# zgojcic/3D_multiview_reg

Measured on AMD Instinct MI355X. Metric: point-cloud pairs/s (feat+match+filter+SVD), 3DMatch 20k-pt, 1/2/4/8 GPU, higher is better.
Workload: dtype f32 (bf16x3 MFMA operands); 1 GPU; one synthetic 3DMatch-scale scene per GPU (configs[2]): 30 fragments x ~20393 voxels (0.025 m) -> FCGF -> rand 5000 samples -> soft feature-NN for all 435 pairs -> OANet (128ch, 500 clusters, 2 blocks) -> weighted Procrustes -> all-gather of (R,t,conf); sampler=rand, fragments_per_gpu=30, pairs_per_gpu=435, samples=5000, voxels_mean=20393, math=f32eq, oanet_point_layout=chunk-major, spconv_presplit_planes=False, spatial_map_order=False, library=d32607a7c7e03829, parallelism=dp1 (one scene per rank, RCCL all-gather of records)

## Files before the change

### 3d_multiview_reg_amd/csrc/gemm.hip

```cpp
#include <atomic>
#include <type_traits>
#include <utility>

#include "common.hpp"
#include "knobs.hpp"
#include "gemm.hpp"
#include "mfma_bf16.hpp"
#include "prof.hpp"

#ifndef GEMM_EARLY
#define GEMM_EARLY 0
#endif

#ifndef GEMM_TRACE
#define GEMM_TRACE 0
#endif

namespace mvr {

#if GEMM_TRACE
__device__ unsigned long long g_gemm_trace[8];
#define TSTAMP(slot)                                                   \
  do {                                                                 \
    unsigned long long t_;                                             \
// ... 1017 lines not shown
#pragma unroll
      for (int j = 0; j < 2; ++j) {
        const int r = wn * 64 + j * 32 + l32;
        const int o = r * C2_BK + 8 * (cc ^ ((r >> 2) & 3));
        fb[j].h = *reinterpret_cast<const bf16x8*>(Bs + o);
        fb[j].m = *reinterpret_cast<const bf16x8*>(Bs + C2_BPL + o);
        fb[j].l = *reinterpret_cast<const bf16x8*>(Bs + 2 * C2_BPL + o);
      }
      if (st == 0) store_a(SET, gn, so);
#pragma unroll
      for (int ii = 0; ii < 2; ++ii)
#pragma unroll
        for (int j = 0; j < 2; ++j) acc[ii][j] = bx::mfma6(fa[ii], fb[j], acc[ii][j]);
      if (st == 0) {
        issue_a(SET, min(gs + 3, S - 1));
        __builtin_amdgcn_sched_group_barrier(0x100, 16, 0);
#pragma unroll
        for (int u = 0; u < 24; ++u) {
          __builtin_amdgcn_sched_group_barrier(0x008, 1, 0);
          __builtin_amdgcn_sched_group_barrier(0x002, 4, 0);
          if (u == C2_AISSUE) __builtin_amdgcn_sched_group_barrier(0x020, 2, 0);
          if (u == 20) __builtin_amdgcn_sched_group_barrier(0x200, 3, 0);
        }
        __builtin_amdgcn_sched_barrier(0);
        TSTAMP(3);
      }
    }
    TSTAMP(4);
    if (ks == nks - 1) {
      const int t = slot + (gs / nks) * G;
      const int b = t / ntn, tn = t % ntn;
      const int n0 = tn * C2_BN, nb0 = n0 + wn * 64;
      const int nw = min(max(N - nb0, 0), 64);
      const float rnw = nw > 0 ? 1.f / (float)nw : 0.f;
      bool cok[2][4], sok[2];
      float bn[2][4];
#pragma unroll
      for (int j = 0; j < 2; ++j) {
        const int gn = nb0 + j * 32 + 4 * p8;
        sok[j] = gn < N4;
#pragma unroll
        for (int u = 0; u < 4; ++u) {
          cok[j][u] = gn + u < N;
          bn[j][u] = cok[j][u] ? g.bias[gn + u] : 0.f;
        }
      }
      float* Cb = g.C + (int64_t)b * g.sCb;
      if (!C2_RPRE) {
        const float* Rb = g.R + (int64_t)b * g.sRb;
#pragma unroll
        for (int ii = 0; ii < 2; ++ii)
#pragma unroll
          for (int q = 0; q < 4; ++q) {
            const int gm = wm * 64 + ii * 32 + 8 * q + 4 * kh + t4;
#pragma unroll
            for (int j = 0; j < 2; ++j) {
              const int gnc = min(nb0 + j * 32 + 4 * p8, N4 - 4);
              w[ii][j][q] = *reinterpret_cast<const float4*>(Rb + (int64_t)gm * g.ldc + gnc);
            }
          }
      }
#pragma unroll
      for (int ii = 0; ii < 2; ++ii) {
#pragma unroll
        for (int q = 0; q < 4; ++q) {
          const int gm = wm * 64 + ii * 32 + 8 * q + 4 * kh + t4;
#pragma unroll
          for (int j = 0; j < 2; ++j) {
            float a0 = acc[ii][j][4 * q], a1 = acc[ii][j][4 * q + 1], a2 = acc[ii][j][4 * q + 2],
                  a3 = acc[ii][j][4 * q + 3];
            quad_transpose(a0, a1, a2, a3, h1, h2);
            const float4 x = make_float4(a0 + bn[j][0] + w[ii][j][q].x, a1 + bn[j][1] + w[ii][j][q].y,
                                         a2 + bn[j][2] + w[ii][j][q].z, a3 + bn[j][3] + w[ii][j][q].w);
            w[ii][j][q] = x;
            if (sok[j]) *reinterpret_cast<float4*>(Cb + (int64_t)gm * g.ldc + nb0 + j * 32 + 4 * p8) = x;
          }
        }
        float s1[4], s2[4];
#pragma unroll
        for (int q = 0; q < 4; ++q) {
          s1[q] = 0.f;
#pragma unroll
          for (int j = 0; j < 2; ++j)
#pragma unroll
            for (int u = 0; u < 4; ++u) s1[q] += cok[j][u] ? f4(w[ii][j][q], u) : 0.f;
          s1[q] = sum8_p8(s1[q]);
        }
#pragma unroll
        for (int q = 0; q < 4; ++q) {
          const float mu = s1[q] * rnw;
          s2[q] = 0.f;
#pragma unroll
          for (int j = 0; j < 2; ++j)
#pragma unroll
            for (int u = 0; u < 4; ++u) {
              const float d = cok[j][u] ? f4(w[ii][j][q], u) - mu : 0.f;
              s2[q] = fmaf(d, d, s2[q]);
            }
          s2[q] = sum8_p8(s2[q]);
        }
        if (p8 == 0) {
#pragma unroll
          for (int q = 0; q < 4; ++q)
            red[wn * 128 + wm * 64 + ii * 32 + 8 * q + 4 * kh + t4] = make_float2(s1[q], s2[q]);
        }
      }
      lds_barrier();
      if (tid < 256) {
        const int half = tid >> 7, row = tid & 127;
        const int n0h = n0 + 128 * half;
        if (n0h < N) {
          const float2 x = red[(2 * half) * 128 + row], c = red[(2 * half + 1) * 128 + row];
          const int na = min(N - n0h, 64), nb = min(max(N - n0h - 64, 0), 64);
          float2 o = x;
          if (nb > 0) {
            const float d = c.x / (float)nb - x.x / (float)na;
            o = make_float2(x.x + c.x, x.y + c.y + d * d * ((float)na * (float)nb / (float)(na + nb)));
          }
          g.stats[((int64_t)b * ntn128 + 2 * tn + half) * g.st_ld + g.st_off + row] = o;
        }
      }
#pragma unroll
      for (int ii = 0; ii < 2; ++ii)
#pragma unroll
        for (int j = 0; j < 2; ++j)
#pragma unroll
          for (int r = 0; r < 16; ++r) acc[ii][j][r] = 0.f;
    }
    TSTAMP(5);
    if (ks != nks - 1) asm volatile("s_waitcnt vmcnt(2)" ::: "memory");
    else asm volatile("s_waitcnt vmcnt(0)" ::: "memory");
  };
  for (int gs = 0; gs < S; gs += 2) {
    stage(I1{}, gs);
    if (gs + 1 < S) stage(I0{}, gs + 1);
  }
  asm volatile("s_waitcnt vmcnt(0)" ::: "memory");
#if GEMM_TRACE
  TSTAMP(7);
  if (lane == 0)
    for (int q = 0; q < 8; ++q) atomicAdd(&g_gemm_trace[q], tr[q]);
#endif
}


static bool oaf_conv2_covers(const GemmArgs& g) {
  return g.wimg && g.M == 128 && g.pro == PRO_A_K && g.bkc == 1 && g.sBb == 0 && g.bias_mode == BIAS_N &&
         g.stats_mode == ST_ROW && g.has_res && !g.no_store && !g.head_w && !g.xin && g.K % 4 == 0 &&
         g.K > C2_BK && g.K <= C2_KMAX &&
         g.wimg_bytes >= oaf_conv2_image_bytes(g.N, g.K) && (reinterpret_cast<uintptr_t>(g.wimg) & 15) == 0 &&
         (int64_t)c2_nks(g.K) * c2_npad(g.N) * C2_BK * 2 * 3 < ((int64_t)1 << 31);
}

static int launch_oaf_conv2(const GemmArgs& g, hipStream_t s) {
  const int Npad = c2_npad(g.N), nks = c2_nks(g.K);
  const int64_t nthr = (int64_t)nks * Npad * 4;
  hipLaunchKernelGGL(oaf_w_image_kernel, dim3((unsigned)((nthr + 255) / 256)), dim3(256), 0, s, g.B, g.N, g.K, g.ldb,
                     Npad, nks, g.wimg);
  MVR_CHECK_LAUNCH();
  const long long tiles = (long long)(Npad / C2_BN) * g.batch;
  const unsigned wgs = (unsigned)(tiles < GPU_CUS ? tiles : GPU_CUS);
  hipLaunchKernelGGL(oaf_conv2_kernel, dim3(wgs), dim3(C2_THREADS), 0, s, g, (const uint16_t*)g.wimg);
  MVR_CHECK_LAUNCH();
  return MVR_OK;
}

#ifndef GEMM_F16_DEFAULT
#define GEMM_F16_DEFAULT 0
#endif
int g_gemm_h = GEMM_F16_DEFAULT;

template <int PRO, int BKC, int BIAS, int STATS, int RES>
static void launch_t(const KArgs& ka0, long long tiles, hipStream_t s) {
  KArgs ka = ka0;
  const unsigned wgs = (unsigned)(tiles < ka.persist ? tiles : ka.persist);
  const GemmArgs& g = ka.g;
  const bool alias = g.C && (g.C == g.A || g.C == g.B || (g.has_res && g.C == g.R));
  if (g_gemm_h && g.flag && !alias) {
    ka.range = g.flag;
    ka.epoch = 1;
    hipLaunchKernelGGL((gemm_kernel<MATH_F16X2, PRO, BKC, BIAS, STATS, RES>), dim3(wgs), dim3(256), 0, s, ka);
    ka.guard = ka.range;
    ka.range = nullptr;
  }
  hipLaunchKernelGGL((gemm_kernel<MATH_BF16X3, PRO, BKC, BIAS, STATS, RES>), dim3(wgs), dim3(256), 0, s, ka);
}

static inline bool al16(const void* p) { return (reinterpret_cast<uintptr_t>(p) & 15) == 0; }

static int launch_gemm_impl(const GemmArgs& g, hipStream_t s, bool conv2) {
  if (g.M <= 0 || g.N <= 0 || g.batch <= 0) return MVR_OK;
  if (!g.A || !g.B || (!g.C && !g.no_store) || g.K <= 0) return MVR_EINVAL;
  if (g.no_store && !g.head_w && (g.stats_mode != ST_ROW || g.has_res)) return MVR_EINVAL;
  if (g.pro != PRO_NONE && !g.psc) return MVR_EINVAL;
  if ((g.pro == PRO_A_K || g.pro == PRO_B_K) && !g.psh) return MVR_EINVAL;
  if (g.stats_mode != ST_NONE && !g.stats) return MVR_EINVAL;
  if (g.bias_mode != BIAS_NONE && !g.bias) return MVR_EINVAL;
  if (g.has_res && !g.R) return MVR_EINVAL;
  if (g.math != MATH_BF16X3) return MVR_EINVAL;
  const int64_t K4 = round4(g.K), N4 = round4(g.N);
  const bool cm = g.bcs || g.ccs || (g.has_res && (g.rcs || (g.ldr && g.ldr != g.ldc)));
  const int64_t ldr = g.ldr ? g.ldr : g.ldc;
  bool ok = al16(g.A) && al16(g.B) && al16(g.C) && g.lda % 4 == 0 && g.ldb % 4 == 0 && g.ldc % 4 == 0 &&
            g.sAb % 4 == 0 && g.sBb % 4 == 0 && g.sCb % 4 == 0 && g.lda >= K4 && g.ldc >= (g.ccs ? 32 : N4) &&
            g.ldb >= (g.bkc ? K4 : (g.bcs ? 32 : N4));
  if (g.bcs) ok = ok && !g.bkc && g.ldb == 32 && g.bcs % 4 == 0 && g.bcs >= 32LL * g.K;
  if (g.ccs) ok = ok && g.ldc == 32 && g.ccs % 4 == 0 && g.ccs >= 32LL * g.M;
  if (g.has_res) {
    ok = ok && al16(g.R) && g.sRb % 4 == 0;
    if (g.xin != 2)
      ok = ok && ldr % 4 == 0 && (g.rcs ? ldr == 32 && g.rcs % 4 == 0 && g.rcs >= 32LL * g.M : ldr >= N4);
  }
  if (cm && !pconv_covers(g)) return MVR_EINVAL;
  if (g.pro == PRO_A_K || g.pro == PRO_B_K)
    ok = ok && al16(g.psc) && al16(g.psh) && g.sPb % 4 == 0 && g.K % 4 == 0 && g.K <= KV_MAX;
  if (g.pro == PRO_B_SMX) ok = ok && al16(g.psc) && g.sPb % 4 == 0 && g.pld % 4 == 0 && g.pld >= N4;
  if (!ok) return MVR_EINVAL;
  KArgs ka{};
  ka.g = g;
  ka.persist = 2 * GPU_CUS;
  ka.m_fast = (g.sAb == 0 && gemm_mtiles(g.M) > 1) ? 1 : 0;
  const long long tiles = (long long)gemm_ntiles(g.N) * gemm_mtiles(g.M) * g.batch;
  if (tiles > 0x7fffffffLL) return MVR_EINVAL;
  const double fl = 2.0 * g.M * g.N * (double)g.K * g.batch;
  double by = 4.0 * ((double)g.M * g.K * (g.sAb ? g.batch : 1) + (double)g.K * g.N * (g.sBb ? g.batch : 1) +
                     (double)g.M * g.N * g.batch * ((g.has_res ? 2 : 1) - (g.no_store ? 1 : 0)));
  if (g.xin) {
    if (!pconv_covers(g)) return MVR_EINVAL;
    by = 4.0 * ((double)g.M * g.K + (double)g.N * g.batch * (g.xin == 1 ? g.xci + g.M : g.K + g.xci + g.M));
  }
  ProfScope prof(g.prof_kind, fl, by, s);
  if (pconv_covers(g)) return launch_pconv(g, s);
  if (conv2 && oaf_conv2_covers(g)) return launch_oaf_conv2(g, s);
  if (g.head_w) return MVR_EINVAL;
#define MVR_CASE(P, BKC_, BI, ST, RS)                                                                     \
  if (g.pro == P && g.bkc == BKC_ && g.bias_mode == BI && g.stats_mode == ST && (g.has_res != 0) == RS) { \
    launch_t<P, BKC_, BI, ST, RS>(ka, tiles, s);                                                        \
    MVR_CHECK_LAUNCH();                                                                                  \
    return MVR_OK;                                                                                       \
  }
  MVR_CASE(PRO_NONE, 0, BIAS_M, ST_ROW, 0)
  MVR_CASE(PRO_NONE, 0, BIAS_M, ST_NONE, 0)
  MVR_CASE(PRO_B_K, 0, BIAS_M, ST_ROW, 0)
  MVR_CASE(PRO_B_K, 0, BIAS_M, ST_NONE, 0)
  MVR_CASE(PRO_B_K, 0, BIAS_M, ST_COL, 0)
  MVR_CASE(PRO_B_K, 0, BIAS_M, ST_ROW, 1)
  MVR_CASE(PRO_B_K, 0, BIAS_M, ST_ROWSMX, 0)
  MVR_CASE(PRO_B_K, 0, BIAS_M, ST_COLSMX, 0)
  MVR_CASE(PRO_B_SMX, 1, BIAS_NONE, ST_ROW, 0)
  MVR_CASE(PRO_B_SMX, 0, BIAS_NONE, ST_ROW, 0)
  MVR_CASE(PRO_A_K, 1, BIAS_N, ST_ROW, 1)
  MVR_CASE(PRO_NONE, 0, BIAS_NONE, ST_NONE, 0)
  MVR_CASE(PRO_NONE, 1, BIAS_NONE, ST_NONE, 0)
#undef MVR_CASE
  return MVR_EINVAL;
}

int launch_gemm(const GemmArgs& g, hipStream_t s) { return launch_gemm_impl(g, s, !g_force[FORCE_GENERIC_GEMM]); }

}

extern "C" int mvr_gemm_f32(int M, int N, int K, int batch, const float* A, int64_t sAb, int64_t lda, const float* B,
                            int64_t sBb, int64_t ldb, int b_kcontig, float* C, int64_t sCb, int64_t ldc,
                            const float* R, int64_t sRb, const float* bias, int bias_mode, const float* psc,
                            const float* psh, int64_t sPb, int64_t pld, int pro, float* stats, int64_t st_ld,
                            int st_off, int stats_mode, int math, int32_t* range_flag, hipStream_t stream) {
  mvr::GemmArgs g{};
  if (range_flag && math == mvr::MATH_BF16X3 && (mvr::g_gemm_h || mvr::g_pconv_h)) {
    if (hipMemsetAsync(range_flag, 0, sizeof(int32_t), stream) != hipSuccess) return MVR_ELAUNCH;
    g.flag = range_flag;
  }
  g.math = math;
  g.M = M; g.N = N; g.K = K; g.batch = batch;
  g.A = A; g.sAb = sAb; g.lda = lda;
  g.B = B; g.sBb = sBb; g.ldb = ldb; g.bkc = b_kcontig;
  g.C = C; g.sCb = sCb; g.ldc = ldc;
  g.R = R; g.sRb = sRb; g.has_res = R != nullptr;
  g.bias = bias; g.bias_mode = bias_mode;
  g.psc = psc; g.psh = psh; g.sPb = sPb; g.pld = pld; g.pro = pro;
  g.stats = reinterpret_cast<float2*>(stats); g.st_ld = st_ld; g.st_off = st_off; g.stats_mode = stats_mode;
  return mvr::launch_gemm(g, stream);
}

#if GEMM_TRACE
extern "C" int mvr_gemm_trace(unsigned long long* out, int reset) {
  if (hipMemcpyFromSymbol(out, HIP_SYMBOL(mvr::g_gemm_trace), sizeof(unsigned long long) * 8) != hipSuccess) return -1;
  if (reset) {
    unsigned long long z[8] = {0, 0, 0, 0, 0, 0, 0, 0};
    if (hipMemcpyToSymbol(HIP_SYMBOL(mvr::g_gemm_trace), z, sizeof(z)) != hipSuccess) return -1;
  }
  return 0;
}
#endif

extern "C" int mvr_oaf_conv2_f32(int M, int N, int K, int batch, const float* A, int64_t sAb, int64_t lda,
                                 const float* W, int64_t ldw, float* C, int64_t sCb, int64_t ldc, const float* R,
                                 int64_t sRb, const float* bias, const float* psc, const float* psh, int64_t sPb,
                                 float* stats, int64_t st_ld, void* img, int64_t img_bytes, hipStream_t stream) {
  mvr::GemmArgs g{};
  g.math = mvr::MATH_BF16X3;
  g.M = M; g.N = N; g.K = K; g.batch = batch;
  g.A = A; g.sAb = sAb; g.lda = lda;
  g.B = W; g.sBb = 0; g.ldb = ldw; g.bkc = 1;
  g.C = C; g.sCb = sCb; g.ldc = ldc;
  g.R = R; g.sRb = sRb; g.has_res = 1;
  g.bias = bias; g.bias_mode = mvr::BIAS_N;
  g.psc = psc; g.psh = psh; g.sPb = sPb; g.pro = mvr::PRO_A_K;
  g.stats = reinterpret_cast<float2*>(stats); g.st_ld = st_ld; g.stats_mode = mvr::ST_ROW;
  g.wimg = static_cast<uint16_t*>(img); g.wimg_bytes = img_bytes;
  if (M != 128 || K % 4 || N < 0 || batch < 0) return MVR_EINVAL;
  if (N == 0 || batch == 0) return MVR_OK;
  if (!R || !bias || !psc || !psh || !stats || !img) return MVR_EINVAL;
// ... 8 lines not shown
```

### 3d_multiview_reg_amd/csrc/gemm.hpp

```cpp
#pragma once
#include "knobs.hpp"
#include <hip/hip_runtime.h>
#include <stdint.h>

#include "mvreg.h"

namespace mvr {

enum Pro : int {
  PRO_NONE = 0,
  PRO_A_K = 1,
  PRO_B_K = 2,
  PRO_B_SMX = 3,
};
enum Bias : int { BIAS_NONE = 0, BIAS_M = 1, BIAS_N = 2 };
enum Stats : int {
  ST_NONE = 0,
  ST_ROW = 1,
  ST_ROWSMX = 2,
  ST_COLSMX = 3,
  ST_COL = 4,
};

enum Math : int { MATH_BF16X3 = 1, MATH_F16X2 = 2 };

constexpr int GEMM_BM = 128, GEMM_BN = 128, GEMM_BK = 32;

struct GemmArgs {
  int M, N, K, batch;
  const float* A; int64_t sAb; int64_t lda;
  const float* B; int64_t sBb; int64_t ldb; int bkc;
  float* C; int64_t sCb; int64_t ldc;
  const float* R; int64_t sRb;
  const float* bias;
  const float* psc; const float* psh; int64_t sPb;
  int64_t pld;
  float2* stats; int64_t st_ld; int st_off;
  int pro, bias_mode, stats_mode, has_res;
  int prof_kind;
  int math;
  int no_store;
  const float* head_w; const float* head_bp; float* logits; float* scores; int32_t* pos;
  int xin; int xci; const float* xw; const float* xb;
  int64_t xld;
  int* flag;
  int* fin_cnt; float fin_eps; mvr_bn_p fin_bn; float* fin_sc; float* fin_sh; int64_t fin_ld;
  float fin_eps2; mvr_bn_p fin_bn2; float* fin_sc2; float* fin_sh2;
  int fin_train; float2* fin_mv; int* fin_done;
  uint16_t* wimg; int64_t wimg_bytes;
  int64_t bcs, ccs, rcs, ldr;
};

int launch_gemm(const GemmArgs& g, hipStream_t stream);

bool pconv_covers(const GemmArgs& g);
int launch_pconv(const GemmArgs& g, hipStream_t stream);

int oan_diff_pool_cm(const float* x, int64_t x_pstride, int64_t x_ld, int64_t x_cs, const float* sc, const float* sh,
                     int64_t s_pstride, const float* weight, const float* bias, int P, int channels, int N, int clusters,
                     float* out, int64_t out_pstride, int64_t out_ld, float* stats, int64_t st_ld, int st_off,
                     void* workspace, size_t workspace_bytes, hipStream_t stream);
int oan_diff_unpool_cm(const float* x_up, int64_t x_pstride, int64_t x_ld, int64_t x_cs, const float* sc,
                       const float* sh, int64_t s_pstride, const float* weight, const float* bias, const float* x_down,
                       int64_t xd_pstride, int64_t xd_ld, int P, int channels, int N, int clusters, float* out,
                       int64_t out_pstride, int64_t out_ld, int64_t out_cs, float* stats, int64_t st_ld, int st_off,
                       void* workspace, size_t workspace_bytes, hipStream_t stream);

int64_t oaf_conv2_image_bytes(int N, int K);

inline int gemm_ntiles(int N){ return (N + GEMM_BN - 1) / GEMM_BN; }
inline int gemm_mtiles(int M) { return (M + GEMM_BM - 1) / GEMM_BM; }
inline int64_t round4(int64_t x) { return (x + 3) & ~(int64_t)3; }
inline int64_t round32(int64_t x) { return (x + 31) & ~(int64_t)31; }

}
```

### 3d_multiview_reg_amd/csrc/knobs.hip

```cpp
#include "common.hpp"
#include "knobs.hpp"
#include "mvreg.h"

namespace mvr {
int g_force[FORCE_COUNT] = {};
}

extern "C" int mvr_set_math(int mode) {
  using namespace mvr;
  const int prev = g_spconv_h ? 1 : 0;
  const int h = mode == 1 ? 1 : 0;
  g_gemm_h = g_pconv_h = g_attn_h = g_spconv_h = h;
  if (g_feat_nn_fast) g_feat_nn_fast = h ? 2 : 1;
  return prev;
}

extern "C" int mvr_debug_force(int what, int value) {
  using namespace mvr;
  if (what == FORCE_FEAT_NN_ONLINE) {
    const int prev = g_feat_nn_fast ? 0 : 1;
    g_feat_nn_fast = value ? 0 : (g_spconv_h ? 2 : 1);
    return prev;
  }
  if (what < 0 || what >= FORCE_COUNT) return MVR_EINVAL;
  const int prev = g_force[what];
  g_force[what] = value ? 1 : 0;
  return prev;
}
```

### 3d_multiview_reg_amd/csrc/knobs.hpp

```cpp
#pragma once

namespace mvr {

constexpr int GPU_CUS = 256;

extern int g_gemm_h;
extern int g_pconv_h;
extern int g_attn_h;
extern int g_spconv_h;
extern int g_feat_nn_fast;

enum ForcePath : int {
  FORCE_FEAT_NN_ONLINE = 0,
  FORCE_GENERIC_GEMM = 1,
  FORCE_UNFUSED_ATTN = 2,
  FORCE_NO_CONV1_FOLD = 3,
  FORCE_POOL_NOSPLIT = 4,
  FORCE_UNPOOL8 = 5,
  FORCE_ROW_LAYOUT = 6,
  FORCE_COUNT = 7
};
extern int g_force[FORCE_COUNT];

}
```

### 3d_multiview_reg_amd/csrc/oan_attn.hip

```cpp
#include <algorithm>
#include <functional>
#include <vector>

#include "common.hpp"
#include "gemm.hpp"
#include "knobs.hpp"
#include "mfma_bf16.hpp"
#include "prof.hpp"
#include "mvreg.h"

namespace mvr {

using namespace bx;

constexpr int AC = 128;
constexpr int AKB = 32;
constexpr int AQ = 256;
constexpr int ATHREADS = 512;
constexpr int ATL = AQ + 4;
constexpr int PLANE = AC * AKB * 2;
constexpr int IMG = 3 * PLANE;
constexpr int STAGE_B = 2 * IMG;
constexpr int MAX_CLUSTERS = 1024;
constexpr int WROW = 272;
// ... 982 lines not shown
static double pool_makespan(int64_t full, int64_t parts, int k, int cus) {
  std::vector<double> slot((size_t)cus, 0.0);
  std::make_heap(slot.begin(), slot.end(), std::greater<double>());
  auto put = [&](double d) {
    std::pop_heap(slot.begin(), slot.end(), std::greater<double>());
    slot.back() += d;
    std::push_heap(slot.begin(), slot.end(), std::greater<double>());
  };
  for (int64_t i = 0; i < full; ++i) put(1.0);
  for (int64_t i = 0; i < parts; ++i) put(1.0 / k);
  return *std::max_element(slot.begin(), slot.end());
}
static PoolSplit pool_splits(int P, int nqb, int N) {
  const int nkb = (N + AKB - 1) / AKB;
  if (!POOL_TAIL) return nkb >= 16 ? PoolSplit{2, 0} : PoolSplit{1, (P + 7) / 8};
  int dev = 0, cus = 0;
  if (hipGetDevice(&dev) != hipSuccess ||
      hipDeviceGetAttribute(&cus, hipDeviceAttributeMultiprocessorCount, dev) != hipSuccess || cus <= 0)
    cus = 256;
  const int G = (P + 7) / 8;
  const int64_t per = 8LL * nqb;
  PoolSplit best{1, G};
  double tbest = pool_makespan(per * G, 0, 1, cus);
  int64_t slabs_best = 0;
  for (int k = 2; k <= 4; k *= 2) {
    if (nkb < 8 * k) break;
    const int gfill = (int)(((per * G) / cus) * cus / per);
    const int cands[3] = {0, gfill, G};
    for (int g0 : cands) {
      if (g0 >= G) continue;
      const int64_t parts = per * k * (G - g0);
      const double t = pool_makespan(per * g0, parts, k, cus);
      if (t < tbest - 1e-9 || (t < tbest + 1e-9 && parts < slabs_best)) {
        tbest = t;
        best = PoolSplit{k, g0};
        slabs_best = parts;
      }
    }
  }
  return best;
}

static size_t pool_ws_bytes(int P, int clusters, int nks) {
  const size_t slots = (size_t)P * ((clusters + AQ - 1) / AQ);
  return (nks > 1 ? slots * ((size_t)nks * PSLAB * 4 + 4) : 0) + 512;
}


extern "C" size_t mvr_oan_diff_pool_workspace_bytes(int P, int channels, int clusters) {
  if (P <= 0 || channels != AC || clusters <= 0 || clusters > MAX_CLUSTERS) return 0;
  return pool_ws_bytes(P, clusters, 4);
}

extern "C" int mvr_oan_diff_pool_ws(const float* x, int64_t x_pstride, int64_t x_ld, const float* sc,
                                    const float* sh, int64_t s_pstride, const float* weight, const float* bias, int P,
                                    int channels, int N, int clusters, float* out, int64_t out_pstride, int64_t out_ld,
                                    float* stats, int64_t st_ld, int st_off, void* workspace, size_t workspace_bytes,
                                    hipStream_t stream);

extern "C" int mvr_oan_diff_pool(const float* x, int64_t x_pstride, int64_t x_ld, const float* sc, const float* sh,
                                 int64_t s_pstride, const float* weight, const float* bias, int P, int channels, int N,
                                 int clusters, float* out, int64_t out_pstride, int64_t out_ld, float* stats,
                                 int64_t st_ld, int st_off, hipStream_t stream) {
  return mvr_oan_diff_pool_ws(x, x_pstride, x_ld, sc, sh, s_pstride, weight, bias, P, channels, N, clusters, out,
                              out_pstride, out_ld, stats, st_ld, st_off, nullptr, 0, stream);
}

extern "C" int mvr_oan_diff_pool_ws(const float* x, int64_t x_pstride, int64_t x_ld, const float* sc,
                                    const float* sh, int64_t s_pstride, const float* weight, const float* bias, int P,
                                    int channels, int N, int clusters, float* out, int64_t out_pstride, int64_t out_ld,
                                    float* stats, int64_t st_ld, int st_off, void* workspace, size_t workspace_bytes,
                                    hipStream_t stream) {
  return mvr::oan_diff_pool_cm(x, x_pstride, x_ld, 32, sc, sh, s_pstride, weight, bias, P, channels, N, clusters, out,
                               out_pstride, out_ld, stats, st_ld, st_off, workspace, workspace_bytes, stream);
}

int mvr::oan_diff_pool_cm(const float* x, int64_t x_pstride, int64_t x_ld, int64_t x_cs, const float* sc,
                          const float* sh, int64_t s_pstride, const float* weight, const float* bias, int P,
                          int channels, int N, int clusters, float* out, int64_t out_pstride, int64_t out_ld,
                          float* stats, int64_t st_ld, int st_off, void* workspace, size_t workspace_bytes,
                          hipStream_t stream) {
  if (P < 0 || N <= 0 || channels != AC || clusters <= 0 || clusters > MAX_CLUSTERS) return MVR_EINVAL;
  if (P == 0) return MVR_OK;
  if (!x || !sc || !sh || !weight || !out) return MVR_EINVAL;
  const bool xcm = x_cs != 32;
  if ((xcm ? (x_ld != 32 || (x_cs & 3) || x_cs < 32 * AC) : x_ld < round_up4(N)) || (x_ld & 3) || (x_pstride & 3) ||
      !al16(x) || !al16(weight) || !al16(out) || out_ld < round_up4(clusters) || (out_ld & 3) || (out_pstride & 3) ||
      (stats && (st_ld < channels + st_off)))
    return MVR_EINVAL;
  if ((xcm ? (int64_t)((N + 31) / 32) * x_cs : (int64_t)AC * x_ld) * 4 >= ((int64_t)1 << 31)) return MVR_EINVAL;
  if (P == 0) return MVR_OK;
  PoolArgs a{};
  a.X = x; a.xps = x_pstride; a.xld = x_ld; a.xcs = x_cs;
  a.sc = sc; a.sh = sh; a.sps = s_pstride;
  a.W = weight; a.bias = bias;
  a.P = P; a.N = N; a.Kc = clusters; a.nqb = (clusters + AQ - 1) / AQ;
  a.out = out; a.ops = out_pstride; a.old = out_ld;
  a.stats = reinterpret_cast<float2*>(stats); a.st_ld = st_ld; a.st_off = st_off;
  a.nks = 1;
  const size_t slots = (size_t)P * a.nqb;
  int* range = nullptr;
  if (workspace) {
    if (!al16(workspace) || workspace_bytes < pool_ws_bytes(P, clusters, 4)) return MVR_EINVAL;
    const PoolSplit ps = pool_splits(P, a.nqb, N);
    const int k = ps.nks;
    if (k > 1) {
      a.nks = k;
      a.g0 = ps.g0;
      a.part = reinterpret_cast<float*>(workspace);
      a.cnt = reinterpret_cast<int*>(reinterpret_cast<char*>(workspace) + slots * (size_t)k * PSLAB * 4);
    }
    if (g_attn_h)
      range = reinterpret_cast<int*>(reinterpret_cast<char*>(workspace) +
                                     (a.nks > 1 ? slots * ((size_t)a.nks * PSLAB * 4 + 4) : 0));
  }
  if (a.nks > 1 || range) {
    void* z = a.nks > 1 ? (void*)a.cnt : (void*)range;
    const size_t zb = (a.nks > 1 ? slots * sizeof(int) : 0) + (range ? sizeof(int) : 0);
    if (hipMemsetAsync(z, 0, zb, stream) != hipSuccess) return MVR_ELAUNCH;
  }
  const double fl = 4.0 * AC * clusters * (double)N * P;
  const double by = 4.0 * AC * ((double)N + clusters) * P;
  ProfScope prof(PK_POOL, fl, by, stream);
  const int G = (P + 7) / 8;
  const int grid = a.nks > 1 ? 8 * a.nqb * (a.g0 + a.nks * (G - a.g0)) : G * 8 * a.nqb;
  if (range) {
    a.range = range;
    hipLaunchKernelGGL(oan_pool_kernel<1>, dim3(grid), dim3(ATHREADS), 0, stream, a);
    MVR_CHECK_LAUNCH();
    a.range = nullptr;
    a.guard = range;
  }
  hipLaunchKernelGGL(oan_pool_kernel<0>, dim3(grid), dim3(ATHREADS), 0, stream, a);
  MVR_CHECK_LAUNCH();
  return MVR_OK;
}

extern "C" int mvr_oan_diff_unpool(const float* x_up, int64_t x_pstride, int64_t x_ld, const float* sc,
                                   const float* sh, int64_t s_pstride, const float* weight, const float* bias,
                                   const float* x_down, int64_t xd_pstride, int64_t xd_ld, int P, int channels,
                                   int N, int clusters, float* out, int64_t out_pstride, int64_t out_ld, float* stats,
                                   int64_t st_ld, int st_off, void* workspace, size_t workspace_bytes,
                                   hipStream_t stream) {
  return mvr::oan_diff_unpool_cm(x_up, x_pstride, x_ld, 32, sc, sh, s_pstride, weight, bias, x_down, xd_pstride,
                                 xd_ld, P, channels, N, clusters, out, out_pstride, out_ld, 32, stats, st_ld, st_off,
                                 workspace, workspace_bytes, stream);
}

int mvr::oan_diff_unpool_cm(const float* x_up, int64_t x_pstride, int64_t x_ld, int64_t x_cs, const float* sc,
                            const float* sh, int64_t s_pstride, const float* weight, const float* bias,
                            const float* x_down, int64_t xd_pstride, int64_t xd_ld, int P, int channels, int N,
                            int clusters, float* out, int64_t out_pstride, int64_t out_ld, int64_t out_cs,
                            float* stats, int64_t st_ld, int st_off, void* workspace, size_t workspace_bytes,
                            hipStream_t stream) {
  if (P < 0 || N <= 0 || channels != AC || clusters <= 0 || clusters > MAX_CLUSTERS) return MVR_EINVAL;
  if (P == 0) return MVR_OK;
  if (!x_up || !sc || !sh || !weight || !x_down || !out || !workspace) return MVR_EINVAL;
  auto bad_layout = [&](int64_t ld, int64_t cs) {
    return cs != 32 ? (ld != 32 || (cs & 3) || cs < 32 * AC) : ld < round_up4(N);
  };
  if (bad_layout(x_ld, x_cs) || (x_ld & 3) || (x_pstride & 3) || xd_ld < clusters || bad_layout(out_ld, out_cs) ||
      (out_ld & 3) || (out_pstride & 3) || !al16(out) || !al16(workspace) || (stats && (st_ld < channels + st_off)))
    return MVR_EINVAL;
  if (P == 0) return MVR_OK;
  if (workspace_bytes < mvr_oan_diff_unpool_workspace_bytes(P, channels, clusters)) return MVR_EINVAL;
  const int nkb = (clusters + AKB - 1) / AKB;
  char* wimg = reinterpret_cast<char*>(workspace);
  char* dimg = wimg + (size_t)nkb * WIMG;
  float2* bs = reinterpret_cast<float2*>(dimg + (size_t)P * nkb * IMG);
  int* range = reinterpret_cast<int*>(bs + (size_t)nkb * AKB);
  const double fl = 4.0 * AC * clusters * (double)N * P;
  const double by = 4.0 * AC * (2.0 * N + clusters) * P;
  ProfScope prof(PK_UNPOOL, fl, by, stream);
  UnpoolArgs a{};
  a.X = x_up; a.xps = x_pstride; a.xld = x_ld; a.xcs = x_cs;
  a.sc = sc; a.sh = sh; a.sps = s_pstride;
  a.wimg = wimg; a.bias = bias; a.bs = bs; a.dimg = dimg;
  a.P = P; a.N = N; a.Kc = clusters; a.nkb = nkb; a.nqb = (N + AQ - 1) / AQ;
  a.out = out; a.ops = out_pstride; a.old = out_ld; a.ocs = out_cs;
  a.stats = reinterpret_cast<float2*>(stats); a.st_ld = st_ld; a.st_off = st_off;
  const int64_t nx = (int64_t)P * nkb * 1024;
  const dim3 gw((nkb * 512 + 255) / 256), gx((unsigned)((nx + 255) / 256));
  if (!g_force[FORCE_UNPOOL8] && clusters <= 512) {
    a.nqb = (N + U4Q - 1) / U4Q;
    const int grid = ((P + 7) / 8) * 8 * a.nqb;
    const int* guard = nullptr;
    if (g_attn_h) {
      if (hipMemsetAsync(range, 0, sizeof(int), stream) != hipSuccess) return MVR_ELAUNCH;
      hipLaunchKernelGGL(split_w_kernel<1>, gw, dim3(256), 0, stream, weight, bias, clusters, nkb, wimg, bs, range,
                         nullptr);
      MVR_CHECK_LAUNCH();
      hipLaunchKernelGGL(split_xd16_kernel, dim3((unsigned)(((int64_t)P * AC * 64 + 255) / 256)), dim3(256), 0, stream,
                         x_down, xd_pstride, xd_ld, P, clusters, nkb, dimg, range);
      MVR_CHECK_LAUNCH();
      a.range = range;
      hipLaunchKernelGGL(oan_unpool4_kernel<1>, dim3(grid), dim3(U4T), 0, stream, a);
      MVR_CHECK_LAUNCH();
      a.range = nullptr;
      a.guard = guard = range;
    }
    hipLaunchKernelGGL(split_w_kernel<0>, gw, dim3(256), 0, stream, weight, bias, clusters, nkb, wimg, bs, nullptr,
                       guard);
    MVR_CHECK_LAUNCH();
    hipLaunchKernelGGL(split_xd_kernel, gx, dim3(256), 0, stream, x_down, xd_pstride, xd_ld, P, clusters, nkb, dimg,
                       guard);
    MVR_CHECK_LAUNCH();
    hipLaunchKernelGGL(oan_unpool4_kernel<0>, dim3(grid), dim3(U4T), 0, stream, a);
  } else {
    hipLaunchKernelGGL(split_w_kernel<0>, gw, dim3(256), 0, stream, weight, bias, clusters, nkb, wimg, bs, nullptr,
                       nullptr);
    MVR_CHECK_LAUNCH();
    hipLaunchKernelGGL(split_xd_kernel, gx, dim3(256), 0, stream, x_down, xd_pstride, xd_ld, P, clusters, nkb, dimg,
                       nullptr);
    MVR_CHECK_LAUNCH();
    const int grid = ((P + 7) / 8) * 8 * a.nqb;
    hipLaunchKernelGGL(oan_unpool_kernel, dim3(grid), dim3(ATHREADS), 0, stream, a);
  }
  MVR_CHECK_LAUNCH();
  return MVR_OK;
}

extern "C" int mvr_attn_reruns(int reset) {
  int v = 0;
  if (hipDeviceSynchronize() != hipSuccess || hipMemcpyFromSymbol(&v, HIP_SYMBOL(g_attn_reruns), sizeof(int)) != hipSuccess)
    return -1;
  if (reset) {
    const int z = 0;
    if (hipMemcpyToSymbol(HIP_SYMBOL(g_attn_reruns), &z, sizeof(int)) != hipSuccess) return -1;
  }
  return v;
}
```

### 3d_multiview_reg_amd/csrc/oanet.hip

```cpp
#include <math.h>
#include <string.h>

#include <algorithm>

#include "common.hpp"
#include "gemm.hpp"
#include "prof.hpp"
#include "mvreg.h"

namespace mvr {

__global__ void in_finalize_kernel(const float2* __restrict__ st, int64_t st_ld, int st_off, int tw0, int csplit,
                                   int tw1, int C, int L, float eps_in, mvr_bn_p bn, int train, float* sc, float* sh,
                                   int64_t out_ld, float2* mv) {
  extern __shared__ double red[];
  const int G = blockDim.y, nb = blockDim.x, lt = threadIdx.x, tg = threadIdx.y;
  const int c = blockIdx.x * nb + lt;
  const int p = blockIdx.y;
  const bool ok = c < C;
  const int cc = ok ? c : 0;
  const int tw = cc < csplit ? tw0 : tw1;
  const int T = (L + tw - 1) / tw;
  const float2* sp = st + (int64_t)p * T * st_ld + st_off + cc;
  double tot = 0.0;
// ... 211 lines not shown

static unsigned long long* g_dbg = nullptr;
static int g_dbg_cap = 0, g_dbg_n = 0;

__global__ void dbg_hash_kernel(const float* __restrict__ p, int rows, int L, int64_t ps, int64_t ld, int64_t cs,
                                int64_t total, unsigned long long* out) {
  unsigned long long acc = 0;
  for (int64_t i = (int64_t)blockIdx.x * blockDim.x + threadIdx.x; i < total; i += (int64_t)gridDim.x * blockDim.x) {
    const int64_t n = i % L, r = (i / L) % rows, b = i / ((int64_t)L * rows);
    acc += (unsigned long long)__float_as_uint(p[b * ps + r * ld + (n >> 5) * cs + (n & 31)]) *
           (unsigned long long)(2 * i + 1);
  }
  for (int o = 32; o > 0; o >>= 1) acc += __shfl_xor(acc, o, 64);
  if ((threadIdx.x & 63) == 0) atomicAdd(out, acc);
}

static void dbg_hash(const float* p, int P, int rows, int L, int64_t ps, int64_t ld, hipStream_t s, int64_t cs = 0) {
  if (!g_dbg || g_dbg_n >= g_dbg_cap) return;
  hipLaunchKernelGGL(dbg_hash_kernel, dim3(1024), dim3(256), 0, s, p, rows, L, ps, ld, cs ? cs : 32,
                     (int64_t)P * rows * L, g_dbg + g_dbg_n++);
}

static void* g_dump = nullptr;
static size_t g_dump_bytes = 0;
static int g_dump_stage = -1;
static void dbg_dump(const void* p, size_t bytes, hipStream_t s) {
  if (g_dump && g_dbg && g_dbg_n - 1 == g_dump_stage)
    (void)hipMemcpyAsync(g_dump, p, bytes < g_dump_bytes ? bytes : g_dump_bytes, hipMemcpyDeviceToDevice, s);
}

static int g_last_layout = -1;
extern "C" int mvr_oan_last_layout(void) { return g_last_layout; }

extern "C" int mvr_debug_stage_dump(int stage, void* dst, size_t bytes) {
  g_dump = dst;
  g_dump_bytes = bytes;
  g_dump_stage = stage;
  return MVR_OK;
}

extern "C" int mvr_debug_stage_hash(unsigned long long* buf, int cap) {
  g_dbg = buf;
  g_dbg_cap = buf ? cap : 0;
  g_dbg_n = 0;
  return MVR_OK;
}

struct Act {
  float* p;
  int64_t ps;
  int64_t ld;
  int C, L;
  float2* st;
  int64_t st_ld;
  int st_off;
  int tw0 = 128;
  int csplit = 1 << 30;
  int tw1 = 128;
  int64_t cs = 0;
};

struct Ws {
  char* base;
  size_t off, cap;
  template <typename T>
  T* take(size_t n) {
    off = (off + 255) & ~(size_t)255;
    T* r = reinterpret_cast<T*>(base + off);
    off += n * sizeof(T);
    return r;
  }
};

struct Plan {
  int P, N, C, Kc, Cin;
  int64_t Np, Kp, Cinp;
  bool fused;
  bool cm = false;
  char* uimg;
  size_t uimg_bytes;
  size_t bytes;
  float *X11, *XA, *T1, *E, *XD, *O1, *O2, *sc, *sh, *scK, *shK, *fac, *W1, *W8;
  float *sc2, *sh2;
  float *scU, *shU;
  int* fcnt;
  float2 *st11, *stA, *stT, *stD, *stO, *smx, *mv, *stcol;
  int* flags;
  uint16_t* w2img;
  int64_t w2img_bytes;
};

constexpr int FLAG_SLOTS = 128;
constexpr int FIN_SLOTS = 32;

struct FoldReq {
  float eps;
  mvr_bn_p bn;
  float eps2 = 0.f;
  mvr_bn_p bn2{};
  float* sc2 = nullptr;
  float* sh2 = nullptr;
};

Plan plan(int C, int Kc, int Cin, int P, int N, void* base) {
  Plan pl{};
  pl.P = P; pl.N = N; pl.C = C; pl.Kc = Kc; pl.Cin = Cin;
  pl.Np = round32(N); pl.Kp = round32(Kc); pl.Cinp = round4(Cin);
  pl.fused = !g_force[FORCE_UNFUSED_ATTN] && mvr_oan_diff_unpool_workspace_bytes(P, C, Kc) > 0;
  const int TS = gemm_ntiles(N);
  Ws w{reinterpret_cast<char*>(base), 0, 0};
  const size_t PN = (size_t)P * pl.Np, PK = (size_t)P * pl.Kp;
  const int TN = gemm_ntiles(N), TK = gemm_ntiles(Kc), MK = gemm_mtiles(Kc), MC = gemm_mtiles(C);
  pl.X11 = w.take<float>(PN * 2 * C);
  pl.XA = w.take<float>(PN * C);
  pl.T1 = w.take<float>(PN * C);
  pl.E = pl.fused ? nullptr : w.take<float>(PN * Kc);
  pl.XD = w.take<float>(PK * C);
  pl.O1 = w.take<float>(PK * C);
  pl.O2 = w.take<float>(PK * C);
  pl.sc = w.take<float>((size_t)P * 2 * C);
  pl.sh = w.take<float>((size_t)P * 2 * C);
  pl.sc2 = w.take<float>((size_t)P * 2 * C);
  pl.sh2 = w.take<float>((size_t)P * 2 * C);
  pl.scU = w.take<float>((size_t)P * C);
  pl.shU = w.take<float>((size_t)P * C);
  pl.fcnt = w.take<int>((size_t)FIN_SLOTS * P);
  pl.scK = w.take<float>((size_t)P * pl.Kp);
  pl.shK = w.take<float>((size_t)P * pl.Kp);
  size_t nf = (size_t)P * TN * pl.Kp;
  if ((size_t)P * MK * pl.Np > nf) nf = (size_t)P * MK * pl.Np;
  pl.fac = pl.fused ? nullptr : w.take<float>(nf);
  pl.W1 = w.take<float>((size_t)C * pl.Cinp);
  pl.W8 = w.take<float>((size_t)C * 8);
  pl.st11 = w.take<float2>((size_t)P * TS * 2 * C);
  pl.stA = w.take<float2>((size_t)P * TS * C);
  pl.stT = w.take<float2>((size_t)P * TN * C);
  pl.stD = w.take<float2>((size_t)P * TK * C);
  pl.stO = w.take<float2>((size_t)P * TK * C);
  size_t smx = (size_t)P * TN * Kc;
  if ((size_t)P * MK * N > smx) smx = (size_t)P * MK * N;
  pl.smx = pl.fused ? nullptr : w.take<float2>(smx);
  pl.uimg_bytes = pl.fused ? std::max(mvr_oan_diff_unpool_workspace_bytes(P, C, Kc),
                                      mvr_oan_diff_pool_workspace_bytes(P, C, Kc)) : 0;
  pl.uimg = pl.fused ? w.take<char>(pl.uimg_bytes) : nullptr;
  pl.mv = w.take<float2>((size_t)P * 2 * C);
  pl.stcol = w.take<float2>((size_t)P * MC * Kc);
  pl.flags = w.take<int>(FLAG_SLOTS);
  pl.w2img_bytes = oaf_conv2_image_bytes(Kc, Kc);
  pl.w2img = w.take<uint16_t>((size_t)pl.w2img_bytes / 2);
  pl.bytes = w.off + 256;
  return pl;
}

struct Ctx {
  const Plan& pl;
  hipStream_t s;
  int train;
  int bn_group;
  int ngroups() const { return (pl.P + bn_group - 1) / bn_group; }
  bool f16;
  int err = 0;
  int nflag = 0;
  int nfin = 0;
  int fcur = 0;
  float* sc() const { return fcur ? pl.sc2 : pl.sc; }
  float* sh() const { return fcur ? pl.sh2 : pl.sh; }
  int* flag() { return f16 && nflag < FLAG_SLOTS ? pl.flags + nflag++ : nullptr; }
  void chk(int e) {
    if (e && !err) err = e;
  }
  void chk_launch() {
    if (hipGetLastError() != hipSuccess && !err) err = MVR_ELAUNCH;
  }

  Act pts(float* p, int C, int rows, float2* st, int64_t st_ld, int st_off = 0) const {
    Act a{p, (int64_t)rows * pl.Np, pl.cm ? 32 : pl.Np, C, pl.N, st, st_ld, st_off};
    a.cs = pl.cm ? 32LL * rows : 0;
    return a;
  }

  void finalize_in(const Act& a, float eps, const mvr_bn_p& bn, float* sc = nullptr, float* sh = nullptr) {
    if (!sc) { sc = this->sc(); sh = this->sh(); }
    const int bs = a.C >= 256 ? 256 : (a.C + 63) & ~63;
    const int G = 1024 / bs < 4 ? 1024 / bs : 4;
    dim3 grid((a.C + bs - 1) / bs, pl.P);
    hipLaunchKernelGGL(in_finalize_kernel, grid, dim3(bs, G), sizeof(double) * bs * G, s, a.st, a.st_ld, a.st_off,
                       a.tw0, a.csplit, a.tw1, a.C, a.L, eps, bn, train, sc, sh, (int64_t)a.C, pl.mv);
    chk_launch();
    if (train) {
      hipLaunchKernelGGL(in_bn_train_kernel, dim3((a.C + 255) / 256, ngroups()), dim3(256), 0, s, pl.mv, pl.P,
                         bn_group, a.C, eps, bn, sc, sh, (int64_t)a.C);
      chk_launch();
    }
  }

  const mvr_conv_p* head = nullptr;
  bool head_only = false;
  float* h_logits = nullptr;
  float* h_scores = nullptr;
  int32_t* h_pos = nullptr;

  void bn_train_from_mv(int C, float eps, const mvr_bn_p& bn, float* sc, float* sh) {
    hipLaunchKernelGGL(in_bn_train_kernel, dim3((C + 255) / 256, ngroups()), dim3(256), 0, s, pl.mv, pl.P, bn_group, C,
                       eps, bn, sc, sh, (int64_t)C);
    chk_launch();
  }

  bool conv(const mvr_conv_p& cv, const Act& in, bool pro, const Act& out, const Act* res, int stats_mode,
            const float* w_padded = nullptr, bool no_store = false, const FoldReq* fold = nullptr,
            const float* pro_sc = nullptr, const float* pro_sh = nullptr) {
    GemmArgs g{};
    int done = 0;
    if (fold) fuse(g, *fold, &done);
    if (head) {
      g.head_w = head->weight; g.head_bp = head->bias;
      g.logits = h_logits; g.scores = h_scores; g.pos = h_pos;
    }
    g.no_store = no_store ? 1 : 0;
    g.math = MATH_BF16X3;
    g.M = out.C; g.N = in.L; g.K = in.C; g.batch = pl.P;
    g.A = w_padded ? w_padded : cv.weight; g.sAb = 0; g.lda = w_padded ? round4(in.C) : in.C;
    g.B = in.p; g.sBb = in.ps; g.ldb = in.ld; g.bkc = 0; g.bcs = in.cs;
    g.C = out.p; g.sCb = out.ps; g.ldc = out.ld; g.ccs = out.cs;
    if (res) { g.R = res->p; g.sRb = res->ps; g.has_res = 1; g.ldr = res->ld; g.rcs = res->cs; }
    g.bias = cv.bias; g.bias_mode = cv.bias ? BIAS_M : BIAS_NONE;
    if (pro) { g.pro = PRO_B_K; g.psc = pro_sc ? pro_sc : sc(); g.psh = pro_sh ? pro_sh : sh(); g.sPb = in.C; }
    g.stats_mode = stats_mode;
    g.stats = out.st; g.st_ld = out.st_ld; g.st_off = out.st_off;
    g.prof_kind = (in.L == pl.Kc && out.L == pl.Kc) ? PK_OAFILTER : (out.C == pl.Kc ? PK_EMBED : PK_CONV_PTS);
    g.flag = flag();
    chk(launch_gemm(g, s));
    return fused(g, fold, done, out.C);
  }

  void fuse(GemmArgs& g, const FoldReq& f, int* done) {
    if (!OAN_FUSED_FIN || nfin >= FIN_SLOTS) return;
    g.fin_cnt = pl.fcnt + (size_t)nfin * pl.P;
    g.fin_eps = f.eps; g.fin_bn = f.bn;
    g.fin_sc = fcur ? pl.sc : pl.sc2; g.fin_sh = fcur ? pl.sh : pl.sh2; g.fin_ld = 128;
    g.fin_eps2 = f.eps2; g.fin_bn2 = f.bn2; g.fin_sc2 = f.sc2; g.fin_sh2 = f.sh2;
    g.fin_train = train; g.fin_mv = pl.mv;
    g.fin_done = done;
  }
  bool fused(const GemmArgs& g, const FoldReq* f, int done, int C) {
    if (!f || !g.fin_cnt) return false;
    ++nfin;
    if (!done) return false;
    fcur ^= 1;
    if (train) {
      bn_train_from_mv(C, f->eps, f->bn, sc(), sh());
      if (f->sc2) bn_train_from_mv(C, f->eps2, f->bn2, f->sc2, f->sh2);
    }
    return true;
  }

  bool pointcn(const mvr_pointcn_p& pc, const Act& x, Act& y, const FoldReq* next = nullptr, bool x_folded = false) {
    if (!x_folded) finalize_in(x, 1e-5f, pc.bn1);
    Act t = pts(pl.T1, y.C, y.C, pl.stT, y.C);
    const bool sc = pc.shortcut.weight != nullptr;
    y.tw0 = 128;
    y.csplit = 1 << 30;
    const mvr_conv_p* hd = head;
    head = nullptr;
    dbg_hash(this->sc(), pl.P, 1, x.C, x.C, 0, s);
    dbg_hash(this->sh(), pl.P, 1, x.C, x.C, 0, s);
    if (sc) conv(pc.shortcut, x, false, y, nullptr, ST_NONE);
    const FoldReq f5{1e-5f, pc.bn5};
    const bool tf = conv(pc.conv3, x, true, t, nullptr, ST_ROW, nullptr, false, &f5);
    const int TNn = (pl.N + 127) / 128;
    dbg_hash(reinterpret_cast<const float*>(pl.stT), pl.P, 1, TNn * y.C * 2, (int64_t)TNn * y.C * 2, 0, s);
    if (!tf) finalize_in(t, 1e-5f, pc.bn5);
    dbg_hash(this->sc(), pl.P, 1, y.C, y.C, 0, s);
    dbg_hash(this->sh(), pl.P, 1, y.C, y.C, 0, s);
    head = hd;
    const bool yf = conv(pc.conv7, t, true, y, sc ? &y : &x, hd ? ST_NONE : ST_ROW, nullptr, hd && head_only,
                         hd ? nullptr : next);
    head = nullptr;
    if (!hd) {
      dbg_hash(y.p, pl.P, y.C, pl.N, y.ps, y.ld, s, y.cs);
      dbg_hash(reinterpret_cast<const float*>(y.st + y.st_off), pl.P * TNn, 1, 2 * y.C, y.st_ld * 2, 0, s);
      dbg_dump(y.st, (size_t)pl.P * TNn * y.st_ld * sizeof(float2), s);
    }
    return yf;
  }

  bool oafilter(const mvr_oafilter_p& f, const Act& xd, const FoldReq* next = nullptr, bool x_folded = false) {
    const int C = pl.C, Kc = pl.Kc;
    const int64_t Kp = pl.Kp;
    if (!x_folded) finalize_in(xd, 1e-3f, f.bn1);
    Act o1{pl.O1, (int64_t)C * Kp, Kp, C, Kc, pl.stcol, Kc, 0};
    conv(f.conv1, xd, true, o1, nullptr, train ? ST_COL : ST_NONE);
    if (train) {
      hipLaunchKernelGGL(bn_col_train_kernel, dim3((Kc + 255) / 256, ngroups()), dim3(256), 0, s, pl.stcol, pl.P,
                         bn_group, gemm_mtiles(C), Kc, C, f.bn2, pl.scK, pl.shK, Kp);
    } else {
      hipLaunchKernelGGL(bn_fold_eval_kernel, dim3((Kc + 255) / 256), dim3(256), 0, s, f.bn2, Kc, pl.scK, pl.shK);
    }
    chk_launch();
    Act o2{pl.O2, (int64_t)C * Kp, Kp, C, Kc, pl.stO, C, 0};
    GemmArgs g{};
    g.math = MATH_BF16X3;
    g.M = C; g.N = Kc; g.K = Kc; g.batch = pl.P;
    g.A = pl.O1; g.sAb = (int64_t)C * Kp; g.lda = Kp;
    g.B = f.conv2.weight; g.sBb = 0; g.ldb = Kc; g.bkc = 1;
    g.C = o2.p; g.sCb = o2.ps; g.ldc = Kp;
    g.R = pl.O1; g.sRb = (int64_t)C * Kp; g.has_res = 1;
    g.bias = f.conv2.bias; g.bias_mode = BIAS_N;
    g.pro = PRO_A_K; g.psc = pl.scK; g.psh = pl.shK; g.sPb = train ? Kp : 0;
    g.stats_mode = ST_ROW; g.stats = o2.st; g.st_ld = C; g.st_off = 0;
    g.prof_kind = PK_OAFILTER;
    g.flag = flag();
    g.wimg = pl.w2img; g.wimg_bytes = pl.w2img_bytes;
    chk(launch_gemm(g, s));
    finalize_in(o2, 1e-3f, f.bn3);
    return conv(f.conv3, o2, true, xd, &xd, ST_ROW, nullptr, false, next);
  }

  void smx_factors(int T, int L, int64_t ld) {
    dim3 grid((unsigned)((ld + 255) / 256), pl.P);
    hipLaunchKernelGGL(smx_factor_kernel, grid, dim3(256), 0, s, pl.smx, T, L, ld, pl.fac);
    chk_launch();
  }
};

}
}

using namespace mvr;


extern "C" size_t mvr_oan_block_workspace_bytes(int channels, int clusters, int in_channels, int P, int N) {
  return plan(channels, clusters, in_channels, P, N, nullptr).bytes;
}

extern "C" int mvr_oan_block_forward(const mvr_oan_block_p* blk, const float* input, int64_t in_pstride, int64_t ld,
                                     const float* xs, int64_t xs_pstride, int64_t xs_nstride, int P, int N,
                                     int bn_train, float* logits, float* scores, float* R, float* t, float* res,
                                     float* latent, float* res_row, float* score_row, int64_t row_pstride,
                                     int32_t* guard_pos, int32_t* status, int guard_group, void* workspace,
                                     size_t workspace_bytes, hipStream_t s) {
  if (P < 0 || N < 0) return MVR_EINVAL;
  if (P == 0) return MVR_OK;
  if (!blk || !input || !xs || !logits || !scores || !R || !t || !res || !guard_pos || !workspace) return MVR_EINVAL;
  const int C = blk->channels, Kc = blk->clusters, H = blk->half_layers, Cin = blk->in_channels;
  if (P <= 0 || N <= 0 || C <= 0 || Kc <= 0 || H <= 0 || H > MVR_OAN_MAX_HALF || Cin <= 0) return MVR_EINVAL;
  if (C % 4 || ld < round4(N) || ld % 4 || in_pstride % 4 || (reinterpret_cast<uintptr_t>(input) & 15))
    return MVR_EINVAL;
  if (!blk->l1_2[0].shortcut.weight) return MVR_EINVAL;
  Plan pl = plan(C, Kc, Cin, P, N, workspace);
  if (workspace_bytes < pl.bytes) return MVR_EINVAL;
  Ctx cx{pl, s, bn_train ? 1 : 0, bn_train > 1 ? std::min(bn_train, P) : P, g_gemm_h || g_pconv_h};
  if (cx.f16 && hipMemsetAsync(pl.flags, 0, sizeof(int) * FLAG_SLOTS, s) != hipSuccess) return MVR_ELAUNCH;
  if (OAN_FUSED_FIN && hipMemsetAsync(pl.fcnt, 0, sizeof(int) * FIN_SLOTS * P, s) != hipSuccess)
    return MVR_ELAUNCH;
  const int64_t Np = pl.Np, Kp = pl.Kp;
  const int64_t CN = (int64_t)C * Np;
  const int TN = gemm_ntiles(N);

  const float* w1 = nullptr;
  if (Cin % 4) {
    const int n = (int)(C * pl.Cinp);
    hipLaunchKernelGGL(pad_cols_kernel, dim3((n + 255) / 256), dim3(256), 0, s, blk->conv1.weight, C, Cin,
                       (int)pl.Cinp, pl.W1);
    cx.chk_launch();
    w1 = pl.W1;
  }
  Act in{const_cast<float*>(input), in_pstride, ld, Cin, N, nullptr, 0, 0};
  GemmArgs f3{};
  f3.math = MATH_BF16X3; f3.M = C; f3.N = N; f3.K = C; f3.batch = P;
  f3.A = blk->l1_1[0].conv3.weight; f3.lda = C;
  f3.B = input; f3.sBb = in_pstride; f3.ldb = ld;
  f3.C = pl.T1; f3.sCb = CN; f3.ldc = Np;
  f3.bias = blk->l1_1[0].conv3.bias; f3.bias_mode = f3.bias ? BIAS_M : BIAS_NONE;
  f3.pro = PRO_B_K; f3.sPb = C;
  f3.stats_mode = ST_ROW; f3.stats = pl.stT; f3.st_ld = C; f3.st_off = 0;
  f3.xin = 1; f3.xci = Cin; f3.xw = pl.W8; f3.xb = blk->conv1.bias; f3.xld = ld;
  f3.prof_kind = PK_CONV_PTS;
  const bool fold1 = !g_force[FORCE_NO_CONV1_FOLD] && Cin <= 8 && C == 128 && !blk->l1_1[0].shortcut.weight &&
                     pconv_covers(f3);
  auto pconv_takes = [&](int K, int pro, int res, int st) {
    GemmArgs q{};
    q.math = MATH_BF16X3; q.M = C; q.N = N; q.K = K; q.batch = P; q.bias_mode = BIAS_M;
    q.pro = pro ? PRO_B_K : PRO_NONE; q.has_res = res; q.stats_mode = st ? ST_ROW : ST_NONE;
    return pconv_covers(q);
  };
  pl.cm = OAN_CHUNK_MAJOR && fold1 && pl.fused && !g_force[FORCE_ROW_LAYOUT] && pconv_takes(C, 1, 1, 1) && pconv_takes(C, 1, 0, 1) &&
          pconv_takes(2 * C, 1, 0, 1) && pconv_takes(2 * C, 0, 0, 0);
  g_last_layout = pl.cm ? 1 : 0;
  Act xa = cx.pts(pl.XA, C, C, pl.stA, C);
  Act x11top = cx.pts(pl.X11, C, 2 * C, pl.st11, 2 * C);
  const int64_t x11cs = x11top.cs ? x11top.cs : 32;
  f3.ldc = xa.ld; f3.ccs = xa.cs;
  FoldReq fx11{1e-3f, blk->down_bn};
  fx11.eps2 = 1e-3f; fx11.bn2 = blk->up_bn; fx11.sc2 = pl.scU; fx11.sh2 = pl.shU;
  const FoldReq fnext1{1e-5f, H > 1 ? blk->l1_1[1].bn1 : mvr_bn_p{}};
  bool yfold = false;
  if (fold1) {
    const int n8 = C * 8;
    hipLaunchKernelGGL(pad_cols_kernel, dim3((n8 + 255) / 256), dim3(256), 0, s, blk->conv1.weight, C, Cin, 8, pl.W8);
    hipLaunchKernelGGL(xin_stats_kernel, dim3((TN + 3) / 4, P), dim3(256), 0, s, input, in_pstride, ld, Cin, N, TN,
                       pl.W8, blk->conv1.bias, pl.stA);
    cx.chk_launch();
    dbg_hash(reinterpret_cast<const float*>(pl.stA), P, 1, TN * C * 2, (int64_t)TN * C * 2, 0, s);
    cx.finalize_in(xa, 1e-5f, blk->l1_1[0].bn1);
    dbg_hash(cx.sc(), P, 1, C, C, 0, s);
    dbg_hash(cx.sh(), P, 1, C, C, 0, s);
    f3.psc = cx.sc(); f3.psh = cx.sh();
    f3.flag = cx.flag();
    const FoldReq f5{1e-5f, blk->l1_1[0].bn5};
    int f3done = 0;
    cx.fuse(f3, f5, &f3done);
    cx.chk(launch_gemm(f3, s));
    Act t = cx.pts(pl.T1, C, C, pl.stT, C);
    dbg_hash(reinterpret_cast<const float*>(pl.stT), P, 1, TN * C * 2, (int64_t)TN * C * 2, 0, s);
    if (!cx.fused(f3, &f5, f3done, C)) cx.finalize_in(t, 1e-5f, blk->l1_1[0].bn5);
    dbg_hash(cx.sc(), P, 1, C, C, 0, s);
    dbg_hash(cx.sh(), P, 1, C, C, 0, s);
    Act& y = (H == 1) ? x11top : xa;
    GemmArgs f7{};
    f7.math = MATH_BF16X3; f7.M = C; f7.N = N; f7.K = C; f7.batch = P;
    f7.A = blk->l1_1[0].conv7.weight; f7.lda = C;
    f7.B = pl.T1; f7.sBb = CN; f7.ldb = t.ld; f7.bcs = t.cs;
    f7.C = y.p; f7.sCb = y.ps; f7.ldc = y.ld; f7.ccs = y.cs;
    f7.R = input; f7.sRb = in_pstride; f7.has_res = 1;
    f7.bias = blk->l1_1[0].conv7.bias; f7.bias_mode = f7.bias ? BIAS_M : BIAS_NONE;
    f7.pro = PRO_B_K; f7.psc = cx.sc(); f7.psh = cx.sh(); f7.sPb = C;
    f7.stats_mode = ST_ROW; f7.stats = y.st; f7.st_ld = y.st_ld; f7.st_off = y.st_off;
    f7.xin = 2; f7.xci = Cin; f7.xw = pl.W8; f7.xb = blk->conv1.bias; f7.xld = ld;
    f7.prof_kind = PK_CONV_PTS;
    f7.flag = cx.flag();
    int f7done = 0;
    const FoldReq* n7 = (H == 1) ? &fx11 : &fnext1;
    cx.fuse(f7, *n7, &f7done);
    cx.chk(launch_gemm(f7, s));
    yfold = cx.fused(f7, n7, f7done, C);
    dbg_hash(pl.T1, P, C, N, CN, t.ld, s, t.cs);
    dbg_hash(y.p, P, C, N, y.ps, y.ld, s, y.cs);
  } else {
    cx.conv(blk->conv1, in, false, xa, nullptr, ST_ROW, w1);
  }
  for (int i = fold1 ? 1 : 0; i < H; ++i) {
    Act& yo = (i == H - 1) ? x11top : xa;
    const FoldReq fn{1e-5f, i + 1 < H ? blk->l1_1[i + 1].bn1 : mvr_bn_p{}};
    yfold = cx.pointcn(blk->l1_1[i], xa, yo, i == H - 1 ? &fx11 : &fn, yfold);
    dbg_hash(pl.T1, P, C, N, CN, xa.ld, s, xa.cs);
    dbg_hash(yo.p, P, C, N, yo.ps, yo.ld, s, yo.cs);
  }
  const bool up_folded = yfold;

  if (!yfold) cx.finalize_in(x11top, 1e-3f, blk->down_bn);
  Act xd{pl.XD, (int64_t)C * Kp, Kp, C, Kc, pl.stD, C, 0};
  if (pl.fused) {
    cx.chk(oan_diff_pool_cm(pl.X11, 2 * CN, x11top.ld, x11cs, cx.sc(), cx.sh(), C, blk->down_conv.weight,
                            blk->down_conv.bias, P, C, N, Kc, pl.XD, (int64_t)C * Kp, Kp, reinterpret_cast<float*>(pl.stD),
                            C, 0, !g_force[FORCE_POOL_NOSPLIT] ? pl.uimg : nullptr, pl.uimg_bytes, s));
  } else {
    Act e{pl.E, (int64_t)Kc * Np, Np, Kc, N, pl.smx, Kc, 0};
    cx.conv(blk->down_conv, x11top, true, e, nullptr, ST_ROWSMX);
    cx.smx_factors(TN, Kc, Kp);
    GemmArgs g{};
    g.math = MATH_BF16X3;
    g.M = C; g.N = Kc; g.K = N; g.batch = P;
    g.A = pl.X11; g.sAb = 2 * CN; g.lda = Np;
    g.B = pl.E; g.sBb = (int64_t)Kc * Np; g.ldb = Np; g.bkc = 1;
    g.C = pl.XD; g.sCb = (int64_t)C * Kp; g.ldc = Kp;
    g.pro = PRO_B_SMX; g.psc = pl.fac; g.sPb = (int64_t)TN * Kp; g.pld = Kp;
    g.stats_mode = ST_ROW; g.stats = pl.stD; g.st_ld = C; g.st_off = 0;
    g.prof_kind = PK_POOL;
    g.flag = cx.flag();
    cx.chk(launch_gemm(g, s));
  }
  dbg_hash(pl.XD, P, C, Kc, (int64_t)C * Kp, Kp, s);
  bool xdfold = false;
  for (int i = 0; i < H; ++i) {
    const FoldReq fn{1e-3f, i + 1 < H ? blk->l2[i + 1].bn1 : mvr_bn_p{}};
    xdfold = cx.oafilter(blk->l2[i], xd, i + 1 < H ? &fn : nullptr, xdfold);
    dbg_hash(pl.XD, P, C, Kc, (int64_t)C * Kp, Kp, s);
  }

  if (!up_folded) cx.finalize_in(x11top, 1e-3f, blk->up_bn, pl.scU, pl.shU);
  if (pl.fused) {
    cx.chk(oan_diff_unpool_cm(pl.X11, 2 * CN, x11top.ld, x11cs, pl.scU, pl.shU, C, blk->up_conv.weight,
                              blk->up_conv.bias, pl.XD, (int64_t)C * Kp, Kp, P, C, N, Kc, pl.X11 + C * x11top.ld, 2 * CN,
                              x11top.ld, x11cs, reinterpret_cast<float*>(pl.st11), 2 * C, C, pl.uimg, pl.uimg_bytes, s));
  } else {
    Act e2{pl.E, (int64_t)Kc * Np, Np, Kc, N, pl.smx, N, 0};
    cx.conv(blk->up_conv, x11top, true, e2, nullptr, ST_COLSMX, nullptr, false, nullptr, pl.scU, pl.shU);
    const int MK = gemm_mtiles(Kc);
    cx.smx_factors(MK, N, Np);
    GemmArgs g{};
    g.math = MATH_BF16X3;
    g.M = C; g.N = N; g.K = Kc; g.batch = P;
    g.A = pl.XD; g.sAb = (int64_t)C * Kp; g.lda = Kp;
    g.B = pl.E; g.sBb = (int64_t)Kc * Np; g.ldb = Np; g.bkc = 0;
    g.C = pl.X11 + CN; g.sCb = 2 * CN; g.ldc = Np;
    g.pro = PRO_B_SMX; g.psc = pl.fac; g.sPb = (int64_t)MK * Np; g.pld = Np;
    g.stats_mode = ST_ROW; g.stats = pl.st11; g.st_ld = 2 * C; g.st_off = C;
    g.prof_kind = PK_UNPOOL;
    g.flag = cx.flag();
    cx.chk(launch_gemm(g, s));
  }
  dbg_hash(pl.X11 + C * x11top.ld, P, C, N, 2 * CN, x11top.ld, s, x11top.cs);
  Act x11 = cx.pts(pl.X11, 2 * C, 2 * C, pl.st11, 2 * C);
  x11.tw0 = x11top.tw0;
  x11.csplit = C;
  x11.tw1 = 128;
  Act outI = cx.pts(pl.XA, C, C, pl.stA, C);
  Act outL{latent, (int64_t)C * ld, ld, C, N, pl.stA, C, 0};
  if (hipMemsetAsync(guard_pos, 0, sizeof(int32_t) * P, s) != hipSuccess) return MVR_ELAUNCH;
  GemmArgs probe{};
  probe.math = MATH_BF16X3; probe.M = C; probe.N = N; probe.K = C; probe.batch = P; probe.pro = PRO_B_K;
  probe.has_res = 1; probe.bias_mode = BIAS_M; probe.head_w = blk->output.weight;
  probe.no_store = latent ? 0 : 1;
  const bool fuse_head = pconv_covers(probe);
  bool ofold = false;
  for (int i = 0; i < H; ++i) {
    if (fuse_head && i == H - 1) {
      cx.head = &blk->output;
      cx.head_only = latent == nullptr;
      cx.h_logits = logits; cx.h_scores = scores; cx.h_pos = guard_pos;
    }
    const FoldReq fn{1e-5f, i + 1 < H ? blk->l1_2[i + 1].bn1 : mvr_bn_p{}};
    Act& yo = (latent && i == H - 1) ? outL : outI;
    ofold = cx.pointcn(blk->l1_2[i], i == 0 ? x11 : outI, yo, i + 1 < H ? &fn : nullptr, i > 0 && ofold);
    dbg_hash(pl.T1, P, C, N, CN, outI.ld, s, outI.cs);
    if (latent || i < H - 1) dbg_hash(yo.p, P, C, N, yo.ps, yo.ld, s, yo.cs);
  }
  const Act& out = latent ? outL : outI;
  dbg_hash(logits, P, 1, N, N, N, s);
  if (!fuse_head) {
    hipLaunchKernelGGL(head_kernel, dim3((N + 255) / 256, P), dim3(256), 0, s, out.p, out.ps, out.ld,
                       out.cs ? out.cs : (int64_t)32, C, N,
                       blk->output.weight, blk->output.bias, logits, scores, guard_pos);
    cx.chk_launch();
  }
  if (cx.err) return cx.err;
  if (guard_group < 0) return hipGetLastError() == hipSuccess ? MVR_OK : MVR_ELAUNCH;
  int e3 = mvr_procrustes(xs, xs + 3, xs_pstride, xs_nstride, scores, N, guard_pos, nullptr, 0, P, N, 1, 1e-7f, R,
                          t, res, N, res_row, row_pstride, status, guard_group, s);
  if (e3) return e3;
  if (score_row) {
    if (hipMemcpy2DAsync(score_row, row_pstride * sizeof(float), scores, N * sizeof(float), N * sizeof(float), P,
                         hipMemcpyDeviceToDevice, s) != hipSuccess)
      return MVR_ELAUNCH;
  }
  return hipGetLastError() == hipSuccess ? MVR_OK : MVR_ELAUNCH;
}
```

### 3d_multiview_reg_amd/csrc/sparse.hip

```cpp

#include <algorithm>

#include "common.hpp"
#include "mfma_bf16.hpp"
#include "prof.hpp"
#include "radix.hpp"
#include "sparse.hpp"

namespace mvr {

__device__ __forceinline__ uint64_t mix64(uint64_t x) {
  x ^= x >> 33;
  x *= 0xff51afd7ed558ccdULL;
  x ^= x >> 33;
  x *= 0xc4ceb9fe1a85ec53ULL;
  x ^= x >> 33;
  return x;
}

__device__ __forceinline__ uint64_t pack_key(int b, int x, int y, int z) {
  return ((uint64_t)(uint32_t)b << 51) | ((uint64_t)((uint32_t)(x + KEY_BIAS) & KEY_MASK) << 34) |
         ((uint64_t)((uint32_t)(y + KEY_BIAS) & KEY_MASK) << 17) | (uint64_t)((uint32_t)(z + KEY_BIAS) & KEY_MASK);
}

// ... 335 lines not shown
    return;
  }
  const int t = h.hdr[0];
  if (t < -1 || t > 15) return;
  const int dx = k % 3 - 1, dy = (k / 3) % 3 - 1, dz = k / 9 - 1;
  const int4 c = oc[o];
  const int qx = c.y + dx * step, qy = c.z + dy * step, qz = c.w + dz * step;
  if (t >= 0 && ((qx | qy | qz) & ((1 << t) - 1)) != 0) return;
  const int64_t i = hash_find(h, pack_key(c.x, qx, qy, qz), t);
  if (i < 0) return;
  nbr[o * 27 + k] = (int32_t)i;
  nbr[i * 27 + (26 - k)] = (int32_t)o;
}

__global__ void kernel_map_transpose_kernel(const int32_t* __restrict__ src, int64_t Ms, int K, int32_t* __restrict__ dst,
                                            int64_t Md) {
  const int64_t e = (int64_t)blockIdx.x * blockDim.x + threadIdx.x;
  if (e >= Ms * K) return;
  const int32_t i = src[e];
  if (i < 0 || i >= Md) return;
  const int64_t o = e / K;
  const int k = (int)(e - o * K);
  dst[(int64_t)i * K + k] = (int32_t)o;
}

struct BrickView {
  HashView h;
  int32_t* count;
  int32_t* rows;
  int4* bcoord;
};

__device__ __forceinline__ int brick_cell(int x, int y, int z) { return (x & 3) | ((y & 3) << 2) | ((z & 3) << 4); }

__global__ void brick_insert_kernel(const int4* __restrict__ c, int64_t M, HashView h, int t) {
  const int64_t i = (int64_t)blockIdx.x * blockDim.x + threadIdx.x;
  if (i < M) {
    const int4 v = c[i];
    hash_insert_min(h, pack_key(v.x, v.y >> (t + 2), v.z >> (t + 2), v.w >> (t + 2)), (int32_t)i);
  }
}

__global__ __launch_bounds__(256) void brick_ids_kernel(const int4* __restrict__ c, int64_t M, HashView h,
                                                        int32_t* count, int32_t* slot_of, int4* bcoord, int t) {
  __shared__ int wcnt[4];
  __shared__ int wbase;
  const int64_t i = (int64_t)blockIdx.x * blockDim.x + threadIdx.x;
  int64_t sl = -1;
  bool rep = false;
  int4 v = make_int4(0, 0, 0, 0);
  if (i < M) {
    v = c[i];
    sl = hash_slot(h, pack_key(v.x, v.y >> (t + 2), v.z >> (t + 2), v.w >> (t + 2)));
    rep = sl >= 0 && h.vals[sl] == (int32_t)i;
    slot_of[i] = (int32_t)sl;
  }
  const unsigned long long m = __ballot(rep);
  const int lane = threadIdx.x & 63, wv = threadIdx.x >> 6;
  if (lane == 0) wcnt[wv] = __popcll(m);
  __syncthreads();
  if (threadIdx.x == 0) {
    const int tot = wcnt[0] + wcnt[1] + wcnt[2] + wcnt[3];
    wbase = tot ? atomicAdd(count, tot) : 0;
  }
  __syncthreads();
  int base = wbase;
  for (int w = 0; w < wv; ++w) base += wcnt[w];
  if (rep) {
    const int id = base + __popcll(m & ((1ULL << lane) - 1));
    h.vals[sl] = id;
    bcoord[id] = make_int4(v.x, v.y >> (t + 2), v.z >> (t + 2), v.w >> (t + 2));
  }
}

__global__ void brick_rows_init_kernel(int32_t* rows, const int32_t* __restrict__ count) {
  const int64_t n = (int64_t)count[0] * 16;
  int4* r = reinterpret_cast<int4*>(rows);
  for (int64_t i = (int64_t)blockIdx.x * blockDim.x + threadIdx.x; i < n; i += (int64_t)gridDim.x * blockDim.x)
    r[i] = make_int4(-1, -1, -1, -1);
}

__global__ void brick_fill_kernel(const int4* __restrict__ c, int64_t M, HashView h, const int32_t* __restrict__ slot_of,
                                  int32_t* rows, int t) {
  const int64_t i = (int64_t)blockIdx.x * blockDim.x + threadIdx.x;
  if (i >= M) return;
  const int4 v = c[i];
  const int sl = slot_of[i];
  if (sl < 0) return;
  rows[(int64_t)h.vals[sl] * 64 + brick_cell(v.y >> t, v.z >> t, v.w >> t)] = (int32_t)i;
}

template <int CO>
__global__ __launch_bounds__(256) void spconv_c1_kernel(const int4* __restrict__ oc, int64_t Mo, BrickView bv,
                                                        const float* __restrict__ feat, int ks, int step,
                                                        const float* __restrict__ W, mvr_bn_p bn, float bn_eps,
                                                        int relu, float* __restrict__ out, int64_t ldout) {
  extern __shared__ float sW[];
  constexpr int WLD = CO + 1;
  const int K = ks * ks * ks;
  for (int e = threadIdx.x; e < K * CO; e += blockDim.x) sW[(e / CO) * WLD + e % CO] = W[e];
  __syncthreads();
  const int64_t o = (int64_t)blockIdx.x * blockDim.x + threadIdx.x;
  if (o >= Mo) return;
  float acc[CO];
#pragma unroll
  for (int c = 0; c < CO; ++c) acc[c] = 0.f;
  const int4 cc = oc[o];
  const int r = ks / 2;
  const int x = cc.y / step, y = cc.z / step, z = cc.w / step;
  for (int bz = (z - r) >> 2; bz <= (z + r) >> 2; ++bz)
    for (int by = (y - r) >> 2; by <= (y + r) >> 2; ++by)
      for (int bx = (x - r) >> 2; bx <= (x + r) >> 2; ++bx) {
        const int64_t sl = hash_slot(bv.h, pack_key(cc.x, bx, by, bz));
        if (sl < 0) continue;
        const int32_t* br = bv.rows + (int64_t)bv.h.vals[sl] * 64;
        const int x0 = max(x - r, 4 * bx), x1 = min(x + r, 4 * bx + 3);
        const int y0 = max(y - r, 4 * by), y1 = min(y + r, 4 * by + 3);
        const int z0 = max(z - r, 4 * bz), z1 = min(z + r, 4 * bz + 3);
        for (int cz = z0; cz <= z1; ++cz)
          for (int cy = y0; cy <= y1; ++cy)
            for (int cx = x0; cx <= x1; ++cx) {
              const int row = br[brick_cell(cx, cy, cz)];
              if (row < 0) continue;
              const float f = feat[row];
              const float* w = sW + ((cx - x + r) + ks * (cy - y + r) + ks * ks * (cz - z + r)) * WLD;
#pragma unroll
              for (int c = 0; c < CO; ++c) acc[c] = fmaf(f, w[c], acc[c]);
            }
      }
#pragma unroll
  for (int c = 0; c < CO; ++c) {
    float v = acc[c];
    if (bn.gamma) {
      const float sc = bn.gamma[c] / sqrtf(bn.var[c] + bn_eps);
      v = (v - bn.mean[c]) * sc + bn.beta[c];
    }
    if (relu) v = fmaxf(v, 0.f);
    out[o * ldout + c] = v;
  }
}

constexpr int C1_KSZ = 7, C1_K = 343, C1_NS = 22;
constexpr int C1_G = 10;
constexpr int C1_WAVES = 8;
constexpr int C1_GRID = 1024;

struct C1Smem {
  bx::bf16x8 wf[C1_NS][3][64];
  short off[C1_NS * 16];
  float grid[C1_WAVES][C1_GRID];
  float sc[32], sh[32];
};

__global__ __launch_bounds__(512) void spconv_c1_brick_kernel(BrickView bv, const float* __restrict__ feat,
                                                              const float* __restrict__ W, mvr_bn_p bn,
                                                              float bn_eps, int relu, float* __restrict__ out,
                                                              int64_t ldout, uint16_t* __restrict__ outp) {
  using namespace bx;
  __shared__ __attribute__((aligned(16))) C1Smem sm;
  const int tid = threadIdx.x, lane = tid & 63, l32 = lane & 31, hh = lane >> 5;
  const int w = tid >> 6;
  for (int e = tid; e < C1_NS * 64; e += blockDim.x) {
    const int s = e >> 6, ln = e & 63, k0 = 16 * s + 8 * (ln >> 5), c = ln & 31;
    float v[8];
#pragma unroll
    for (int i = 0; i < 8; ++i) v[i] = k0 + i < C1_K ? W[(k0 + i) * 32 + c] : 0.f;
    Frag f;
    split8(v, f.h, f.m, f.l);
    sm.wf[s][0][ln] = f.h;
    sm.wf[s][1][ln] = f.m;
    sm.wf[s][2][ln] = f.l;
  }
  for (int k = tid; k < C1_NS * 16; k += blockDim.x)
    sm.off[k] = (short)(k < C1_K ? k % C1_KSZ + C1_G * ((k / C1_KSZ) % C1_KSZ) + C1_G * C1_G * (k / (C1_KSZ * C1_KSZ))
                                 : 0);
  if (tid < 32) {
    float sc = 1.f, sh = 0.f;
    if (bn.gamma) {
      sc = bn.gamma[tid] / sqrtf(bn.var[tid] + bn_eps);
      sh = bn.beta[tid] - bn.mean[tid] * sc;
    }
    sm.sc[tid] = sc;
    sm.sh[tid] = sh;
  }
  __syncthreads();
  const float csc = sm.sc[l32], csh = sm.sh[l32];
  const int base0 = (l32 & 3) + C1_G * ((l32 >> 2) & 3) + C1_G * C1_G * (l32 >> 4);
  const int base1 = base0 + 2 * C1_G * C1_G;
  float* g = sm.grid[w];
  const int nb = *bv.count;
  typedef short s16x8 __attribute__((ext_vector_type(8)));
  for (int b = blockIdx.x * C1_WAVES + w; b < nb; b += gridDim.x * C1_WAVES) {
    const int4 bc = bv.bcoord[b];
    int nid = -1;
    if (lane < 27) {
      const int64_t sl =
          hash_slot(bv.h, pack_key(bc.x, bc.y + lane % 3 - 1, bc.z + (lane / 3) % 3 - 1, bc.w + lane / 9 - 1));
      nid = sl >= 0 ? bv.h.vals[sl] : -1;
    }
    int rw[16];
#pragma unroll
    for (int i = 0; i < 16; ++i) {
      const int gi = lane + 64 * i;
      const int ux = gi % C1_G + 1, uy = (gi / C1_G) % C1_G + 1, uz = gi / (C1_G * C1_G) + 1;
      const int id = __shfl(nid, (ux >> 2) + 3 * (uy >> 2) + 9 * min(uz >> 2, 2), 64);
      rw[i] = (gi < C1_G * C1_G * C1_G && id >= 0) ? bv.rows[(int64_t)id * 64 + brick_cell(ux, uy, uz)] : -1;
    }
    float fv[16];
#pragma unroll
    for (int i = 0; i < 16; ++i) fv[i] = rw[i] >= 0 ? feat[rw[i]] : 0.f;
    const int myrow = bv.rows[(int64_t)b * 64 + lane];
    asm volatile("s_waitcnt lgkmcnt(0)" ::: "memory");
#pragma unroll
    for (int i = 0; i < 16; ++i) g[lane + 64 * i] = fv[i];
    asm volatile("s_waitcnt lgkmcnt(0)" ::: "memory");
    floatx16 acc0, acc1;
#pragma unroll
    for (int r = 0; r < 16; ++r) acc0[r] = acc1[r] = 0.f;
#pragma unroll 2
    for (int s = 0; s < C1_NS; ++s) {
      const s16x8 o = *reinterpret_cast<const s16x8*>(&sm.off[16 * s + 8 * hh]);
      Frag wf;
      wf.h = sm.wf[s][0][lane];
      wf.m = sm.wf[s][1][lane];
      wf.l = sm.wf[s][2][lane];
      float v0[8], v1[8];
#pragma unroll
      for (int i = 0; i < 8; ++i) {
        v0[i] = g[base0 + o[i]];
        v1[i] = g[base1 + o[i]];
      }
      Frag a0, a1;
      split8(v0, a0.h, a0.m, a0.l);
      split8(v1, a1.h, a1.m, a1.l);
      acc0 = mfma6(a0, wf, acc0);
      acc1 = mfma6(a1, wf, acc1);
    }
#pragma unroll
    for (int q = 0; q < 16; ++q) {
      const int r = (q & 3) + 8 * (q >> 2) + 4 * hh;
      const int r0 = __shfl(myrow, r, 64), r1 = __shfl(myrow, 32 + r, 64);
      float v0 = fmaf(acc0[q], csc, csh), v1 = fmaf(acc1[q], csc, csh);
      if (relu) {
        v0 = fmaxf(v0, 0.f);
        v1 = fmaxf(v1, 0.f);
      }
      if (r0 >= 0) out[(int64_t)r0 * ldout + l32] = v0;
      if (r1 >= 0) out[(int64_t)r1 * ldout + l32] = v1;
      if (outp) {
        if (r0 >= 0) store_planes(outp + (int64_t)r0 * 3 * ldout + l32, ldout, v0);
        if (r1 >= 0) store_planes(outp + (int64_t)r1 * 3 * ldout + l32, ldout, v1);
      }
    }
  }
}

__global__ void l2norm_rows_kernel(float* x, int64_t M, int C, int64_t ld) {
  const int64_t o = (int64_t)blockIdx.x * blockDim.x + threadIdx.x;
  if (o >= M) return;
  float* r = x + o * ld;
  float s = 0.f;
  for (int c = 0; c < C; ++c) s = fmaf(r[c], r[c], s);
  const float inv = 1.f / sqrtf(s);
  for (int c = 0; c < C; ++c) r[c] *= inv;
}

__global__ void l2norm_rows32_kernel(float* x, int64_t M, int64_t ld) {
  const int64_t o = ((int64_t)blockIdx.x * blockDim.x + threadIdx.x) >> 3;
  const int part = threadIdx.x & 7;
  const bool ok = o < M;
  float4* r = reinterpret_cast<float4*>(x + (ok ? o : 0) * ld) + part;
  float4 v = ok ? *r : make_float4(0.f, 0.f, 0.f, 0.f);
  float s = v.x * v.x + v.y * v.y + v.z * v.z + v.w * v.w;
  s += __shfl_xor(s, 1, 64);
  s += __shfl_xor(s, 2, 64);
  s += __shfl_xor(s, 4, 64);
  const float inv = 1.f / sqrtf(s);
  if (ok) *r = make_float4(v.x * inv, v.y * inv, v.z * inv, v.w * inv);
}

static inline uint64_t next_pow2(uint64_t v) {
  uint64_t p = 1024;
  while (p < v) p <<= 1;
  return p;
}

size_t hash_table_bytes(int64_t M) { return 16 + next_pow2((uint64_t)(2 * (M > 0 ? M : 1))) * 12; }

HashView hash_view(void* table, size_t bytes) {
  HashView h{};
  if (bytes < 16 + 1024 * 12) return h;
  uint64_t cap = 1024;
  while (16 + cap * 2 * 12 <= bytes) cap <<= 1;
  char* base = reinterpret_cast<char*>(table);
  h.cap = cap;
  h.keys = reinterpret_cast<uint64_t*>(base + 16);
  h.vals = reinterpret_cast<int32_t*>(base + 16 + cap * 8);
  h.hdr = reinterpret_cast<int32_t*>(base);
  return h;
}

static inline unsigned nblk(int64_t n, int b = 256) { return (unsigned)((n + b - 1) / b); }

struct DedupWs {
  uint64_t* keys; int4* cc; int32_t* flags; int32_t* pos; int32_t* bsum; void* table; size_t table_bytes;
};

static size_t dedup_scan_bytes(int64_t n) { return scan_ws_bytes(n > 0 ? n : 1); }
static size_t dedup_ws_bytes(int64_t n, int64_t keys = -1) {
  return (size_t)n * (8 + 16 + 4 + 4) + dedup_scan_bytes(n) + hash_table_bytes(keys < 0 ? n : keys) + 8 * 256;
}

static DedupWs dedup_ws(void* ws, int64_t n, int64_t keys = -1) {
  char* p = reinterpret_cast<char*>(ws);
  auto take = [&](size_t b) { p = reinterpret_cast<char*>(((uintptr_t)p + 255) & ~(uintptr_t)255); char* r = p; p += b; return r; };
  DedupWs d{};
  d.keys = reinterpret_cast<uint64_t*>(take((size_t)n * 8));
  d.cc = reinterpret_cast<int4*>(take((size_t)n * 16));
  d.flags = reinterpret_cast<int32_t*>(take((size_t)n * 4));
  d.pos = reinterpret_cast<int32_t*>(take((size_t)n * 4));
  d.bsum = reinterpret_cast<int32_t*>(take(dedup_scan_bytes(n)));
  d.table_bytes = hash_table_bytes(keys < 0 ? n : keys);
  d.table = take(d.table_bytes);
  return d;
}

static int dedup_run(const DedupWs& d, int64_t n, int4* coords_out, int64_t* sel_out, int64_t* counts, int B,
                     hipStream_t s, int* overflow = nullptr) {
  HashView h = hash_view(d.table, d.table_bytes);
  hipLaunchKernelGGL(hash_clear_kernel, dim3(nblk((int64_t)h.cap)), dim3(256), 0, s, h);
  if (overflow)
    hipLaunchKernelGGL(insert_min_bounded_kernel, dim3(nblk(n)), dim3(256), 0, s, d.keys, n, h, overflow);
  else
    hipLaunchKernelGGL(insert_min_kernel, dim3(nblk(n)), dim3(256), 0, s, d.keys, n, h);
  if (hipMemsetAsync(d.flags, 0, sizeof(int32_t) * (size_t)n, s) != hipSuccess) return MVR_ELAUNCH;
  hipLaunchKernelGGL(slot_flag_kernel, dim3(nblk((int64_t)h.cap)), dim3(256), 0, s, h, d.flags);
  if (hipMemsetAsync(counts, 0, sizeof(int64_t) * (1 + B), s) != hipSuccess) return MVR_ELAUNCH;
  const int rc = excl_scan_i32(d.flags, d.pos, n, d.bsum, dedup_scan_bytes(n), s);
  if (rc != MVR_OK) return rc;
  hipLaunchKernelGGL(compact_kernel, dim3(nblk(n)), dim3(256), 0, s, d.flags, d.pos, n, d.cc, coords_out, sel_out,
                     counts);
  const int cb = (int)std::min<int64_t>(nblk(n), 512);
  hipLaunchKernelGGL(batch_count_kernel, dim3(cb), dim3(256), sizeof(int) * B, s, coords_out, B, counts);
  MVR_CHECK_LAUNCH();
  return MVR_OK;
}

__device__ __forceinline__ uint32_t spread3(uint32_t v) {
  v &= 255u;
  v = (v | (v << 16)) & 0x030000FFu;
  v = (v | (v << 8)) & 0x0300F00Fu;
  v = (v | (v << 4)) & 0x030C30C3u;
  v = (v | (v << 2)) & 0x09249249u;
  return v;
}

constexpr int ORDER_MAX_MAPS = 16;
struct OrderMaps {
  const int32_t* nbr[ORDER_MAX_MAPS];
  const int4* coords[ORDER_MAX_MAPS];
  int step[ORDER_MAX_MAPS];
  int64_t start[ORDER_MAX_MAPS + 1];
  int n, K;
  int jshift;
};
__global__ __launch_bounds__(256) void order_keys_kernel(OrderMaps m, uint64_t* __restrict__ keys,
                                                         int32_t* __restrict__ vals) {
  __shared__ int32_t snb[4][64 * 27];
  const int64_t i = (int64_t)blockIdx.x * blockDim.x + threadIdx.x;
  const int lane = threadIdx.x & 63, w = threadIdx.x >> 6;
  const int64_t total = m.start[m.n];
  const int64_t iw = i - lane;
  int j = 0;
  const int64_t ic = i < total ? i : total - 1;
  while (ic >= m.start[j + 1]) ++j;
  const int jf = __shfl(j, 0, 64), jl = __shfl(j, (int)min<int64_t>(63, total - 1 - iw), 64);
  const bool staged = iw < total && jf == jl && m.nbr[jf] != nullptr;
  if (staged) {
    const int64_t nrow = min<int64_t>(64, total - iw);
    const int32_t* src = m.nbr[jf] + (iw - m.start[jf]) * m.K;
    for (int e = lane; e < nrow * m.K; e += 64) snb[w][e] = src[e];
  }
  __syncthreads();
  if (i >= total) return;
  const int64_t o = i - m.start[j];
  uint32_t mask = 0;
  if (m.nbr[j]) {
    const int32_t* row = staged ? &snb[w][lane * m.K] : m.nbr[j] + o * m.K;
    for (int k = 0; k < m.K; ++k) mask |= (row[k] >= 0 ? 1u : 0u) << k;
  }
  uint32_t lo = 0;
  if (m.coords[j]) {
    const int4 c = m.coords[j][o];
    const int st = m.step[j];
    lo = ((uint32_t)c.x & 127u) << 25 | spread3((uint32_t)(c.y / st)) << 2 | spread3((uint32_t)(c.z / st)) << 1 |
         spread3((uint32_t)(c.w / st));
  }
  keys[i] = (uint64_t)j << m.jshift | (uint64_t)mask << 32 | lo;
  vals[i] = (int32_t)o;
}

}

using namespace mvr;

extern "C" size_t mvr_hash_table_bytes(int64_t M) { return hash_table_bytes(M); }

// ... 61 lines not shown
}

extern "C" size_t mvr_coords_downsample_workspace_bytes(int64_t M) { return dedup_ws_bytes(M); }

extern "C" int mvr_coords_downsample(const int32_t* coords, int64_t M, int B, int stride_out, void* ws,
                                     size_t ws_bytes, int32_t* coords_out, int64_t* counts_out, hipStream_t s) {
  if (M < 0 || B <= 0 || B > MAX_BATCH || stride_out <= 0 || !counts_out) return MVR_EINVAL;
  if (M == 0) return hipMemsetAsync(counts_out, 0, sizeof(int64_t) * (1 + B), s) == hipSuccess ? MVR_OK : MVR_ELAUNCH;
  if (!coords || !ws || !coords_out || ws_bytes < dedup_ws_bytes(M)) return MVR_EINVAL;
  ProfScope prof(PK_SPARSE_MISC, 0.0, (double)M * 40.0, s);
  DedupWs d = dedup_ws(ws, M);
  hipLaunchKernelGGL(coarse_keys_kernel, dim3(nblk(M)), dim3(256), 0, s, reinterpret_cast<const int4*>(coords), M,
                     stride_out, d.keys, d.cc);
  return dedup_run(d, M, reinterpret_cast<int4*>(coords_out), nullptr, counts_out, B, s);
}

static int hash_build(const int32_t* coords, int64_t M, int t, void* table, size_t table_bytes, hipStream_t s) {
  if (M < 0 || !table || (M > 0 && !coords)) return MVR_EINVAL;
  if (table_bytes < hash_table_bytes(M)) return MVR_EINVAL;
  HashView h = hash_view(table, table_bytes);
  ProfScope prof(PK_SPARSE_MISC, 0.0, (double)h.cap * 12 + M * 28.0, s);
  hipLaunchKernelGGL(hash_clear_kernel, dim3(nblk((int64_t)h.cap)), dim3(256), 0, s, h, t);
  if (M > 0)
    hipLaunchKernelGGL(build_table_kernel, dim3(nblk(M)), dim3(256), 0, s, reinterpret_cast<const int4*>(coords), M,
                       h, t);
  MVR_CHECK_LAUNCH();
  return MVR_OK;
}

extern "C" int mvr_hash_build(const int32_t* coords, int64_t M, void* table, size_t table_bytes, hipStream_t s) {
  return hash_build(coords, M, -1, table, table_bytes, s);
}

extern "C" int mvr_hash_build_lattice(const int32_t* coords, int64_t M, int stride, void* table, size_t table_bytes,
                                      hipStream_t s) {
  if (stride <= 0 || (stride & (stride - 1)) || stride > (1 << 15)) return MVR_EINVAL;
  return hash_build(coords, M, __builtin_ctz((unsigned)stride), table, table_bytes, s);
}

extern "C" int mvr_kernel_map_x(const int32_t* out_coords, int64_t Mout, const void* in_table, size_t in_table_bytes,
                                int ksize, int step, int transposed, int32_t* nbr, const int32_t* row_order,
                                hipStream_t s) {
  if (Mout < 0 || ksize <= 0 || (ksize & 1) == 0 || step <= 0) return MVR_EINVAL;
  if (Mout == 0) return MVR_OK;
  if (!out_coords || !in_table || !nbr) return MVR_EINVAL;
  HashView h = hash_view(const_cast<void*>(in_table), in_table_bytes);
  if (!h.cap) return MVR_EINVAL;
  const int64_t tot = Mout * (int64_t)ksize * ksize * ksize;
  ProfScope prof(PK_SPARSE_MISC, 0.0, (double)tot * 4.0, s);
  hipLaunchKernelGGL(kernel_map_kernel, dim3(nblk(tot)), dim3(256), 0, s, reinterpret_cast<const int4*>(out_coords),
                     Mout, h, ksize, step, transposed ? -1 : 1, nbr, row_order);
  MVR_CHECK_LAUNCH();
  return MVR_OK;
}

extern "C" int mvr_kernel_map_sym(const int32_t* coords, int64_t M, const void* table, size_t table_bytes, int step,
                                  int32_t* nbr, hipStream_t s) {
  if (M < 0 || step <= 0) return MVR_EINVAL;
  if (M == 0) return MVR_OK;
  if (!coords || !table || !nbr) return MVR_EINVAL;
  HashView h = hash_view(const_cast<void*>(table), table_bytes);
  if (!h.cap) return MVR_EINVAL;
  ProfScope prof(PK_SPARSE_MISC, 0.0, (double)M * 27 * 4.0, s);
  if (hipMemsetAsync(nbr, 0xFF, sizeof(int32_t) * 27 * (size_t)M, s) != hipSuccess) return MVR_ELAUNCH;
  hipLaunchKernelGGL(kernel_map_sym_kernel, dim3(nblk(M * 14)), dim3(256), 0, s, reinterpret_cast<const int4*>(coords), M,
                     h, step, nbr);
  MVR_CHECK_LAUNCH();
  return MVR_OK;
}

extern "C" int mvr_kernel_map_transpose(const int32_t* src, int64_t Ms, int K, int32_t* dst, int64_t Md, hipStream_t s) {
  if (Ms < 0 || Md < 0 || K <= 0 || K > 343) return MVR_EINVAL;
  if (Md == 0) return MVR_OK;
  if (!dst || (Ms > 0 && !src)) return MVR_EINVAL;
  ProfScope prof(PK_SPARSE_MISC, 0.0, (double)(Ms + Md) * K * 4.0, s);
  if (hipMemsetAsync(dst, 0xFF, sizeof(int32_t) * (size_t)K * (size_t)Md, s) != hipSuccess) return MVR_ELAUNCH;
  if (Ms > 0)
    hipLaunchKernelGGL(kernel_map_transpose_kernel, dim3(nblk(Ms * K)), dim3(256), 0, s, src, Ms, K, dst, Md);
  MVR_CHECK_LAUNCH();
  return MVR_OK;
}

extern "C" int mvr_kernel_map(const int32_t* out_coords, int64_t Mout, const void* in_table, size_t in_table_bytes,
                              int ksize, int step, int transposed, int32_t* nbr, hipStream_t s) {
  return mvr_kernel_map_x(out_coords, Mout, in_table, in_table_bytes, ksize, step, transposed, nbr, nullptr, s);
}

static size_t brick_slot_of_bytes(int64_t M) { return ((size_t)(M > 0 ? M : 1) * 4 + 15) & ~(size_t)15; }
static size_t brick_map_bytes(int64_t M) {
  const uint64_t cap = next_pow2((uint64_t)(2 * (M > 0 ? M : 1)));
  const size_t m = (size_t)(M > 0 ? M : 1);
  return 16 + cap * 12 + m * 64 * 4 + brick_slot_of_bytes(M) + m * 16;
}
static BrickView brick_view(void* ws, int64_t M) {
  BrickView v{};
  const uint64_t cap = next_pow2((uint64_t)(2 * (M > 0 ? M : 1)));
  const size_t m = (size_t)(M > 0 ? M : 1);
  char* base = reinterpret_cast<char*>(ws);
  v.count = reinterpret_cast<int32_t*>(base);
  v.h.cap = cap;
  v.h.keys = reinterpret_cast<uint64_t*>(base + 16);
  v.h.vals = reinterpret_cast<int32_t*>(base + 16 + cap * 8);
  v.rows = reinterpret_cast<int32_t*>(base + 16 + cap * 12);
  v.bcoord = reinterpret_cast<int4*>(base + 16 + cap * 12 + m * 64 * 4 + brick_slot_of_bytes(M));
  return v;
}

extern "C" size_t mvr_brick_map_bytes(int64_t M) { return brick_map_bytes(M); }

extern "C" int mvr_brick_map_build_stride(const int32_t* coords, int64_t M, int stride, void* ws, size_t ws_bytes,
                                          hipStream_t s) {
  if (M < 0 || !ws || ws_bytes < brick_map_bytes(M) || stride <= 0 || (stride & (stride - 1)) || stride > (1 << 12) ||
      (M > 0 && !coords))
    return MVR_EINVAL;
  const int t = __builtin_ctz((unsigned)stride);
  BrickView v = brick_view(ws, M);
  int32_t* slot_of = v.rows + (M > 0 ? M : 1) * 64;
  ProfScope prof(PK_SPARSE_MISC, 0.0, (double)v.h.cap * 12 + M * 40.0, s);
  if (hipMemsetAsync(v.count, 0, 16, s) != hipSuccess) return MVR_ELAUNCH;
  hipLaunchKernelGGL(hash_clear_kernel, dim3(nblk((int64_t)v.h.cap)), dim3(256), 0, s, v.h, -1);
  if (M > 0) {
    const int4* c = reinterpret_cast<const int4*>(coords);
    hipLaunchKernelGGL(brick_insert_kernel, dim3(nblk(M)), dim3(256), 0, s, c, M, v.h, t);
    hipLaunchKernelGGL(brick_ids_kernel, dim3(nblk(M)), dim3(256), 0, s, c, M, v.h, v.count, slot_of, v.bcoord, t);
    hipLaunchKernelGGL(brick_rows_init_kernel, dim3((unsigned)std::min<int64_t>(1024, nblk(M * 16))), dim3(256), 0, s,
                       v.rows, v.count);
    hipLaunchKernelGGL(brick_fill_kernel, dim3(nblk(M)), dim3(256), 0, s, c, M, v.h, slot_of, v.rows, t);
  }
  MVR_CHECK_LAUNCH();
  return MVR_OK;
}

extern "C" int mvr_brick_map_build(const int32_t* coords, int64_t M, void* ws, size_t ws_bytes, hipStream_t s) {
  return mvr_brick_map_build_stride(coords, M, 1, ws, ws_bytes, s);
}

extern "C" int mvr_spconv_c1_x(const int32_t* out_coords, int64_t Mout, const void* in_bricks, int64_t Min,
                               size_t in_bricks_bytes, const float* feat, int ksize, int step, const float* W, int Cout,
                               mvr_bn_p bn, float bn_eps, int relu, float* out, int64_t ldout, uint16_t* out_planes,
                               hipStream_t s) {
  if (Mout < 0 || (ksize & 1) == 0 || step <= 0 || Min < 0) return MVR_EINVAL;
  if (Mout == 0 && (out_coords || Min == 0)) return MVR_OK;
  if (!in_bricks || !feat || !W || !out) return MVR_EINVAL;
  if (out_planes && (out_coords || (reinterpret_cast<uintptr_t>(out_planes) & 1))) return MVR_EINVAL;
  if (Cout != 32) return MVR_EINVAL;
  if (in_bricks_bytes < brick_map_bytes(Min)) return MVR_EINVAL;
  if (!out_coords) {
    if (Mout != Min || step != 1 || ksize != C1_KSZ || ldout < 32) return MVR_EINVAL;
    if (Mout == 0) return MVR_OK;
    BrickView v = brick_view(const_cast<void*>(in_bricks), Min);
    ProfScope prof(PK_SPCONV, 2.0 * Mout * C1_K * Cout, (double)Mout * (16 + Cout * 4), s);
    const int grid = (int)std::min<int64_t>(256, (Mout + 63) / 64);
    hipLaunchKernelGGL(spconv_c1_brick_kernel, dim3(grid), dim3(512), 0, s, v, feat, W, bn, bn_eps, relu, out,
                       ldout, out_planes);
    MVR_CHECK_LAUNCH();
    return MVR_OK;
  }
  if (Mout == 0) return MVR_OK;
  BrickView v = brick_view(const_cast<void*>(in_bricks), Min);
  const int K = ksize * ksize * ksize;
  const size_t lds = (size_t)K * (Cout + 1) * sizeof(float);
  if (lds > 160 * 1024) return MVR_EINVAL;
  ProfScope prof(PK_SPCONV, 2.0 * Mout * K * Cout, (double)Mout * (16 + Cout * 4), s);
  hipLaunchKernelGGL(spconv_c1_kernel<32>, dim3(nblk(Mout)), dim3(256), lds, s,
                     reinterpret_cast<const int4*>(out_coords), Mout, v, feat, ksize, step, W, bn, bn_eps, relu, out,
                     ldout);
  MVR_CHECK_LAUNCH();
  return MVR_OK;
}

extern "C" int mvr_spconv_c1(const int32_t* out_coords, int64_t Mout, const void* in_bricks, int64_t Min,
                             size_t in_bricks_bytes, const float* feat, int ksize, int step, const float* W, int Cout,
                             mvr_bn_p bn, float bn_eps, int relu, float* out, int64_t ldout, hipStream_t s) {
  return mvr_spconv_c1_x(out_coords, Mout, in_bricks, Min, in_bricks_bytes, feat, ksize, step, W, Cout, bn, bn_eps,
                         relu, out, ldout, nullptr, s);
}

extern "C" int mvr_l2norm_rows(float* x, int64_t M, int C, int64_t ld, hipStream_t s) {
  if (M < 0 || C <= 0 || ld < C) return MVR_EINVAL;
  if (M == 0) return MVR_OK;
  if (!x) return MVR_EINVAL;
  if (C == 32 && ld % 4 == 0 && (reinterpret_cast<uintptr_t>(x) & 15) == 0)
    hipLaunchKernelGGL(l2norm_rows32_kernel, dim3((unsigned)((M * 8 + 255) / 256)), dim3(256), 0, s, x, M, ld);
  else
    hipLaunchKernelGGL(l2norm_rows_kernel, dim3(nblk(M)), dim3(256), 0, s, x, M, C, ld);
  MVR_CHECK_LAUNCH();
  return MVR_OK;
}

extern "C" size_t mvr_kernel_map_orders_bytes(int64_t total) { return radix_ws_bytes(total); }

extern "C" int mvr_kernel_map_orders(int n_maps, const int32_t* const* nbr, const int32_t* const* out_coords,
                                     const int* steps, const int64_t* Mo, int K, int32_t* perm_out, void* ws,
                                     size_t ws_bytes, hipStream_t s) {
  if (n_maps <= 0 || n_maps > ORDER_MAX_MAPS || !Mo || K < 0 || K > 27) return MVR_EINVAL;
  if ((!nbr) != (K == 0) || (!nbr && !out_coords)) return MVR_EINVAL;
  OrderMaps m{};
  m.n = n_maps;
  m.K = K;
  m.jshift = nbr ? 59 : 32;
  m.start[0] = 0;
  for (int j = 0; j < n_maps; ++j) {
    const int32_t* c = out_coords ? out_coords[j] : nullptr;
    if (Mo[j] < 0 || (Mo[j] > 0 && nbr && !nbr[j]) || (c && (!steps || steps[j] <= 0)) || (!nbr && Mo[j] > 0 && !c))
      return MVR_EINVAL;
    m.nbr[j] = nbr ? nbr[j] : nullptr;
    m.coords[j] = reinterpret_cast<const int4*>(c);
    m.step[j] = c ? steps[j] : 1;
    m.start[j + 1] = m.start[j] + Mo[j];
  }
  const int64_t total = m.start[n_maps];
  if (total > (int64_t)(1 << 30) - 1) return MVR_EINVAL;
  if (total == 0) return MVR_OK;
  if (!perm_out || !ws || ws_bytes < radix_ws_bytes(total)) return MVR_EINVAL;
  ProfScope prof(PK_SPARSE_MISC, 0.0, (double)total * (4.0 * K + 16 + 8 * 24 + 4), s);
  RadixWs w = radix_ws(ws, total);
  hipLaunchKernelGGL(order_keys_kernel, dim3(nblk(total)), dim3(256), 0, s, m, w.ka, w.va);
  int bits = 32 + K;
  if (n_maps > 1) bits = m.jshift + (32 - __builtin_clz((unsigned)(n_maps - 1)));
  return radix_sort(w, bits, perm_out, s);
}

extern "C" size_t mvr_kernel_map_order_bytes(int64_t Mo) { return radix_ws_bytes(Mo); }

extern "C" int mvr_kernel_map_order(const int32_t* nbr, const int32_t* out_coords, int step, int64_t Mo, int K,
                                    int32_t* perm, void* ws, size_t ws_bytes, hipStream_t s) {
  if (Mo < 0 || K <= 0 || K > 27 || (out_coords && step <= 0)) return MVR_EINVAL;
  if (Mo == 0) return MVR_OK;
  if (!nbr || !perm) return MVR_EINVAL;
  return mvr_kernel_map_orders(1, &nbr, &out_coords, &step, &Mo, K, perm, ws, ws_bytes, s);
}
```

### 3d_multiview_reg_amd/lib/_native.py

```python
import ctypes
import os

import torch

_PKG = os.path.dirname(os.path.dirname(os.path.abspath(__file__)))
LIB_PATH = os.environ.get("MVR_LIB") or os.path.join(_PKG, "libmvreg_hip.so")
_lib = None

c_i64 = ctypes.c_int64
c_int = ctypes.c_int
c_float = ctypes.c_float
c_vp = ctypes.c_void_p
c_size = ctypes.c_size_t


class ConvP(ctypes.Structure):
    _fields_ = [("weight", c_vp), ("bias", c_vp)]


class BnP(ctypes.Structure):
    _fields_ = [("gamma", c_vp), ("beta", c_vp), ("mean", c_vp), ("var", c_vp)]


class PointCNP(ctypes.Structure):
    _fields_ = [("bn1", BnP), ("conv3", ConvP), ("bn5", BnP), ("conv7", ConvP), ("shortcut", ConvP)]


class OAFilterP(ctypes.Structure):
    _fields_ = [("bn1", BnP), ("conv1", ConvP), ("bn2", BnP), ("conv2", ConvP), ("bn3", BnP), ("conv3", ConvP)]


MAX_HALF = 8


class OanBlockP(ctypes.Structure):
    _fields_ = [("in_channels", c_int), ("channels", c_int), ("clusters", c_int), ("half_layers", c_int),
                ("conv1", ConvP), ("l1_1", PointCNP * MAX_HALF), ("down_bn", BnP), ("down_conv", ConvP),
                ("l2", OAFilterP * MAX_HALF), ("up_bn", BnP), ("up_conv", ConvP), ("l1_2", PointCNP * MAX_HALF),
                ("output", ConvP)]


_SIGS = {
    "mvr_procrustes": (c_int, [c_vp, c_vp, c_i64, c_i64, c_vp, c_i64, c_vp, c_vp, c_i64, c_int, c_int, c_int, c_float,
                               c_vp, c_vp, c_vp, c_i64, c_vp, c_i64, c_vp, c_int, c_vp]),
    "mvr_procrustes_f64": (c_int, [c_vp, c_vp, c_i64, c_i64, c_vp, c_i64, c_vp, c_vp, c_i64, c_int, c_int, c_int,
                                   ctypes.c_double, c_vp, c_vp, c_vp, c_i64, c_vp, c_i64, c_vp, c_int, c_vp]),
    "mvr_ransac_workspace_bytes": (c_size, [c_int, c_int]),
    "mvr_ransac": (c_int, [c_vp, c_vp, c_i64, c_vp, c_int, c_int, c_int, ctypes.c_double, ctypes.c_uint64, c_vp, c_vp,
                           c_vp, c_vp, c_vp, c_vp, c_size, c_vp]),
    "mvr_sync_workspace_bytes": (c_size, [c_int, c_int, c_int]),
    "mvr_sync_poses": (c_int, [c_vp, c_vp, c_vp, c_vp, c_i64, c_vp, c_vp, c_int, c_int, c_int, c_int, c_int,
                               ctypes.c_double, ctypes.c_double, c_vp, c_vp, c_i64, c_vp, c_vp, c_vp, c_vp, c_vp, c_vp,
                               c_size, c_vp]),
    "mvr_gemm_f32": (c_int, [c_int, c_int, c_int, c_int, c_vp, c_i64, c_i64, c_vp, c_i64, c_i64, c_int, c_vp, c_i64,
                             c_i64, c_vp, c_i64, c_vp, c_int, c_vp, c_vp, c_i64, c_i64, c_int, c_vp, c_i64, c_int,
                             c_int, c_int, c_vp, c_vp]),
    "mvr_oaf_conv2_f32": (c_int, [c_int, c_int, c_int, c_int, c_vp, c_i64, c_i64, c_vp, c_i64, c_vp, c_i64, c_i64,
                                  c_vp, c_i64, c_vp, c_vp, c_vp, c_i64, c_vp, c_i64, c_vp, c_i64, c_vp]),
    "mvr_oaf_conv2_image_bytes": (c_size, [c_int, c_int]),
    "mvr_oan_block_workspace_bytes": (c_size, [c_int, c_int, c_int, c_int, c_int]),
    "mvr_set_math": (c_int, [c_int]),
    "mvr_debug_force": (c_int, [c_int, c_int]),
    "mvr_attn_reruns": (c_int, [c_int]),
    "mvr_debug_stage_hash": (c_int, [c_vp, c_int]),
    "mvr_debug_stage_dump": (c_int, [c_int, c_vp, c_size]),
    "mvr_oan_diff_pool": (c_int, [c_vp, c_i64, c_i64, c_vp, c_vp, c_i64, c_vp, c_vp, c_int, c_int, c_int, c_int,
                                  c_vp, c_i64, c_i64, c_vp, c_i64, c_int, c_vp]),
    "mvr_oan_diff_pool_ws": (c_int, [c_vp, c_i64, c_i64, c_vp, c_vp, c_i64, c_vp, c_vp, c_int, c_int, c_int, c_int,
                                  c_vp, c_i64, c_i64, c_vp, c_i64, c_int, c_vp, c_size, c_vp]),
    "mvr_oan_diff_pool_workspace_bytes": (c_size, [c_int, c_int, c_int]),
    "mvr_oan_diff_unpool_workspace_bytes": (c_size, [c_int, c_int, c_int]),
    "mvr_oan_diff_unpool": (c_int, [c_vp, c_i64, c_i64, c_vp, c_vp, c_i64, c_vp, c_vp, c_vp, c_i64, c_i64, c_int,
                                    c_int, c_int, c_int, c_vp, c_i64, c_i64, c_vp, c_i64, c_int, c_vp, c_size, c_vp]),
    "mvr_oan_block_forward": (c_int, [ctypes.POINTER(OanBlockP), c_vp, c_i64, c_i64, c_vp, c_i64, c_i64, c_int, c_int, c_int,
                                      c_vp, c_vp, c_vp, c_vp, c_vp, c_vp, c_vp, c_vp, c_i64, c_vp, c_vp, c_int, c_vp,
                                      c_size, c_vp]),
    "mvr_feat_nn": (c_int, [c_vp, c_i64, c_vp, c_i64, c_vp, c_i64, c_vp, c_i64, c_vp, c_int, c_int, c_int, c_int,
                            c_float, c_int, c_vp, c_i64, c_i64, c_vp, c_vp]),
    "mvr_feat_nn_gumbel": (c_int, [c_vp, c_i64, c_vp, c_i64, c_vp, c_i64, c_vp, c_i64, c_vp, c_int, c_int, c_int,
                                   c_int, c_float, c_int, ctypes.c_uint64, c_vp, c_i64, c_i64, c_vp, c_vp]),
    "mvr_feat_nn_workspace_bytes": (c_size, [c_int, c_int]),
    "mvr_feat_nn_ws": (c_int, [c_vp, c_i64, c_vp, c_i64, c_vp, c_i64, c_vp, c_i64, c_vp, c_int, c_int, c_int, c_int,
                               c_float, c_int, c_vp, c_i64, c_i64, c_vp, c_int, c_vp, c_size, c_vp]),
    "mvr_gather_rows": (c_int, [c_vp, c_int, c_vp, c_int, c_vp, c_vp]),
    "mvr_sample_rand_mt19937": (c_int, [c_vp, c_vp, c_vp, c_int, c_int, c_vp, c_vp]),
    "mvr_feat_knn2": (c_int, [c_vp, c_i64, c_vp, c_i64, c_vp, c_int, c_int, c_int, c_int, c_vp, c_vp, c_vp]),
    "mvr_fps": (c_int, [c_vp, c_vp, c_vp, c_int, c_int, c_vp, c_vp]),
    "mvr_knn1": (c_int, [c_vp, c_i64, c_i64, c_vp, c_i64, c_i64, c_int, c_int, c_int, c_vp, c_vp, c_vp]),
    "mvr_mutuals": (c_int, [c_vp, c_i64, c_i64, c_vp, c_i64, c_i64, c_vp, c_i64, c_i64, c_vp, c_i64, c_i64, c_int,
                            c_int, c_float, c_vp, c_vp, c_vp]),
    "mvr_voxel_centroids_workspace_bytes": (c_size, [c_i64]),
    "mvr_voxel_centroids": (c_int, [c_vp, c_vp, c_int, c_i64, ctypes.c_double, c_vp, c_size, c_vp, c_vp, c_vp]),
    "mvr_radius_index_bytes": (c_size, [c_i64]),
    "mvr_radius_index_build": (c_int, [c_vp, c_vp, c_int, c_i64, ctypes.c_double, c_vp, c_size, c_vp]),
    "mvr_radius_overlap_count": (c_int, [c_vp, c_size, c_vp, c_vp, c_int, c_i64, c_vp, c_vp, c_int, c_i64,
                                         ctypes.c_double, c_vp, c_vp]),
    "mvr_icp_refine": (c_int, [c_vp, c_size, c_vp, c_vp, c_int, c_i64, ctypes.c_double, c_vp, c_vp, c_int,
                               ctypes.c_double, c_int, ctypes.c_double, ctypes.c_double, c_vp, c_vp, c_vp, c_vp, c_vp,
                               c_vp, c_vp, c_vp]),
    "mvr_estimate_normals": (c_int, [c_vp, c_size, c_vp, c_vp, c_int, c_i64, ctypes.c_double, ctypes.c_double, c_vp,
                                     c_vp, c_vp, c_vp]),
    "mvr_icp_refine_plane": (c_int, [c_vp, c_size, c_vp, c_vp, c_vp, c_int, c_i64, ctypes.c_double, c_vp, c_vp, c_int,
                                     ctypes.c_double, c_int, ctypes.c_double, ctypes.c_double, c_vp, c_vp, c_vp, c_vp,
                                     c_vp, c_vp, c_vp, c_vp]),
    "mvr_icp_refine_generalized": (c_int, [c_vp, c_size, c_vp, c_vp, c_vp, c_int, c_i64, ctypes.c_double, c_vp, c_vp,
                                           c_int, ctypes.c_double, ctypes.c_double, c_int, ctypes.c_double,
                                           ctypes.c_double, c_vp, c_vp, c_vp, c_vp, c_vp, c_vp, c_vp, c_vp]),
    "mvr_pair_information": (c_int, [c_vp, c_size, c_vp, c_vp, c_int, c_i64, ctypes.c_double, c_vp, c_vp, c_int,
                                     ctypes.c_double, c_vp, c_vp, c_vp, c_vp, c_vp]),
    "mvr_compute_fpfh_workspace_bytes": (c_size, [c_i64]),
    "mvr_compute_fpfh": (c_int, [c_vp, c_size, c_vp, c_vp, c_vp, c_int, c_i64, ctypes.c_double, ctypes.c_double, c_vp,
                                 c_vp, c_vp, c_size, c_vp]),
    "mvr_feat_match": (c_int, [c_vp, c_int, c_vp, c_int, c_i64, c_vp, c_vp, c_int, c_i64, c_i64, c_vp, c_vp, c_vp]),
    "mvr_posegraph_workspace_bytes": (c_size, [c_int, c_int, c_int]),
    "mvr_posegraph_optimize": (c_int, [c_vp, c_vp, c_vp, c_vp, c_vp, c_i64, c_vp, c_vp, c_int, c_int, c_int, c_int,
                                       c_vp, c_vp, c_int, ctypes.c_double, ctypes.c_double, ctypes.c_double, c_vp,
                                       c_vp, c_i64, c_vp, c_vp, c_vp, c_vp, c_vp, c_vp, c_size, c_vp]),
    "mvr_fuse_scene_workspace_bytes": (c_size, [c_i64]),
    "mvr_fuse_scene": (c_int, [c_vp, c_vp, c_vp, c_int, c_i64, c_vp, c_vp, ctypes.c_double, c_vp, c_size, c_vp, c_vp,
                               c_vp, c_vp, c_vp, c_vp]),
    "mvr_hash_table_bytes": (c_size, [c_i64]),
    "mvr_voxelize_workspace_bytes": (c_size, [c_i64]),
    "mvr_voxelize_hint_workspace_bytes": (c_size, [c_i64, c_i64]),
    "mvr_voxelize_hint": (c_int, [c_vp, c_vp, c_int, c_i64, ctypes.c_double, c_i64, c_vp, c_size, c_vp, c_vp, c_vp,
                                  c_vp]),
    "mvr_voxelize": (c_int, [c_vp, c_vp, c_int, c_i64, ctypes.c_double, c_vp, c_size, c_vp, c_vp, c_vp, c_vp]),
    "mvr_voxelize_f64": (c_int, [c_vp, c_vp, c_int, c_i64, ctypes.c_double, c_vp, c_size, c_vp, c_vp, c_vp, c_vp]),
    "mvr_coords_downsample_workspace_bytes": (c_size, [c_i64]),
    "mvr_coords_downsample": (c_int, [c_vp, c_i64, c_int, c_int, c_vp, c_size, c_vp, c_vp, c_vp]),
    "mvr_hash_build": (c_int, [c_vp, c_i64, c_vp, c_size, c_vp]),
    "mvr_hash_build_lattice": (c_int, [c_vp, c_i64, c_int, c_vp, c_size, c_vp]),
    "mvr_kernel_map": (c_int, [c_vp, c_i64, c_vp, c_size, c_int, c_int, c_int, c_vp, c_vp]),
    "mvr_kernel_map_x": (c_int, [c_vp, c_i64, c_vp, c_size, c_int, c_int, c_int, c_vp, c_vp, c_vp]),
    "mvr_kernel_map_sym": (c_int, [c_vp, c_i64, c_vp, c_size, c_int, c_vp, c_vp]),
    "mvr_kernel_map_transpose": (c_int, [c_vp, c_i64, c_int, c_vp, c_i64, c_vp]),
    "mvr_kernel_map_order_bytes": (c_size, [c_i64]),
    "mvr_kernel_map_order": (c_int, [c_vp, c_vp, c_int, c_i64, c_int, c_vp, c_vp, c_size, c_vp]),
    "mvr_kernel_map_orders_bytes": (c_size, [c_i64]),
    "mvr_kernel_map_orders": (c_int, [c_int, c_vp, c_vp, c_vp, c_vp, c_int, c_vp, c_vp, c_size, c_vp]),
    "mvr_radix_sort_pairs_bytes": (c_size, [c_i64]),
    "mvr_radix_sort_pairs": (c_int, [c_vp, c_vp, c_i64, c_int, c_vp, c_vp, c_size, c_vp]),
    "mvr_spconv": (c_int, [c_vp, c_i64, c_int, c_vp, c_vp, c_int, c_i64, c_vp, c_int, c_vp, BnP, c_float, c_vp, c_i64,
                           c_int, c_vp, c_i64, c_vp, c_vp, c_vp]),
    "mvr_spconv_x": (c_int, [c_vp, c_i64, c_int, c_vp, c_vp, c_int, c_i64, c_vp, c_int, c_vp, BnP, c_float, c_vp,
                             c_i64, c_int, c_vp, c_i64, c_vp, c_vp, c_vp, c_vp, c_vp]),
    "mvr_spconv_c1_x": (c_int, [c_vp, c_i64, c_vp, c_i64, c_size, c_vp, c_int, c_int, c_vp, c_int, BnP, c_float,
                                c_int, c_vp, c_i64, c_vp, c_vp]),
    "mvr_spconv_wimage_bytes": (c_size, [c_int, c_int, c_int]),
    "mvr_spconv_wimage": (c_int, [c_vp, c_int, c_int, c_int, c_vp, c_size, c_vp]),
    "mvr_brick_map_bytes": (c_size, [c_i64]),
    "mvr_brick_map_build": (c_int, [c_vp, c_i64, c_vp, c_size, c_vp]),
    "mvr_brick_map_build_stride": (c_int, [c_vp, c_i64, c_int, c_vp, c_size, c_vp]),
    "mvr_spconv_c1": (c_int, [c_vp, c_i64, c_vp, c_i64, c_size, c_vp, c_int, c_int, c_vp, c_int, BnP, c_float, c_int,
                              c_vp, c_i64, c_vp]),
    "mvr_l2norm_rows": (c_int, [c_vp, c_i64, c_int, c_i64, c_vp]),
    "mvr_prof_set": (c_int, [c_int]),
    "mvr_prof_mask": (c_int, [ctypes.c_uint]),
    "mvr_prof_seq": (c_int, [c_vp, c_vp, c_int]),
    "mvr_prof_get": (c_int, [c_int, ctypes.POINTER(ctypes.c_double), ctypes.POINTER(ctypes.c_longlong),
                             ctypes.POINTER(ctypes.c_double), ctypes.POINTER(ctypes.c_double)]),
    "mvr_oan_last_layout": (c_int, []),
    "mvr_source_hash": (c_int, [ctypes.c_char_p, c_size]),
    "mvr_xs_to_channels": (c_int, [c_vp, c_i64, c_i64, c_int, c_int, c_int, c_vp, c_i64, c_i64, c_vp]),
}

EXPORTS = tuple(_SIGS)


def lib():
    global _lib
    if _lib is None:
        if not os.path.exists(LIB_PATH):
            raise RuntimeError("libmvreg_hip.so not found at %s — run __graft_entry__.build() "
                               "(there is no CPU fallback for the HIP path)" % LIB_PATH)
        L = ctypes.CDLL(LIB_PATH)
        for name, (res, args) in _SIGS.items():
            f = getattr(L, name)
            f.restype = res
            f.argtypes = args
        _lib = L
    return _lib


_hip_ok = False


def require_hip(t=None):
    global _hip_ok
    if not _hip_ok:
        if not torch.cuda.is_available():
            raise RuntimeError("mvreg HIP path: no HIP device available (no CPU fallback)")
        _hip_ok = True
    if t is not None and t.device.type != "cuda":
        raise RuntimeError("mvreg HIP path: tensor on %s, expected a HIP device" % t.device)


def stream():
    return c_vp(torch.cuda.current_stream().cuda_stream)


def ptr(t):
    if t is None:
        return None
    return c_vp(t.data_ptr())


def check(rc, name):
    if rc != 0:
        raise RuntimeError("%s failed with code %d" % (name, rc))


def source_hash():
    buf = ctypes.create_string_buffer(128)
    check(lib().mvr_source_hash(buf, len(buf)), "mvr_source_hash")
    return buf.value.decode()


PROF_KINDS = {"conv_pts": 0, "embed": 1, "pool": 2, "unpool": 3, "oafilter": 4, "small": 5, "procrustes": 6,
              "feat_nn": 7, "spconv": 8, "sparse_misc": 9, "pointcn": 10}


def prof_set(on):
    check(lib().mvr_prof_set(int(on)), "mvr_prof_set")


def prof_mask(kinds=None):
    m = 0xFFFFFFFF if kinds is None else sum(1 << (PROF_KINDS[k] if isinstance(k, str) else int(k)) for k in kinds)
    check(lib().mvr_prof_mask(m), "mvr_prof_mask")


def prof_seq():
    import numpy as np
    L = lib()
    n = L.mvr_prof_seq(None, None, 0)
    k = np.zeros(max(n, 1), np.int32)
    b = np.zeros(max(n, 1), np.float64)
    L.mvr_prof_seq(k.ctypes.data, b.ctypes.data, n)
    names = {v: s for s, v in PROF_KINDS.items()}
    return [(names.get(int(k[i]), str(int(k[i]))), float(b[i])) for i in range(n)]


def prof_get(kind):
    ms, n, fl, by = ctypes.c_double(), ctypes.c_longlong(), ctypes.c_double(), ctypes.c_double()
    k = PROF_KINDS[kind] if isinstance(kind, str) else int(kind)
    check(lib().mvr_prof_get(k, ctypes.byref(ms), ctypes.byref(n), ctypes.byref(fl), ctypes.byref(by)),
          "mvr_prof_get")
    return ms.value, n.value, fl.value, by.value


MATH_KERNELS = "pconv_math,attn_math,spconv_math,gemm_f16,feat_nn"
FORCE = {"feat_nn_online": 0, "generic_gemm": 1, "unfused_attn": 2, "no_conv1_fold": 3, "pool_nosplit": 4,
         "unpool8": 5, "row_layout": 6}


def math_state():
    L = lib()
    m = L.mvr_set_math(0)
    L.mvr_set_math(m)
    return m


def set_math(mode):
    L = lib()
    L.mvr_set_math({"f32eq": 0, "split16": 1}[mode])
    m = math_state()
    dtype = "f32 (bf16x3 MFMA operands)" if not m else "mixed: split-fp16 (22-bit) operands in " + MATH_KERNELS
    return {"mode": "split16" if m else "f32eq", "dtype": dtype, "knobs": {"split16": m}}


class force:

    def __init__(self, what, value=1):
        self.what, self.value = FORCE[what], int(value)

    def __enter__(self):
        self.prev = lib().mvr_debug_force(self.what, self.value)
        return self

    def __exit__(self, *a):
        lib().mvr_debug_force(self.what, self.prev)


_ws_cache = {}
_flag_cache = {}


def flag_word(device=None):
    idx = (device.index if device is not None and device.index is not None else torch.cuda.current_device())
    key = (idx, torch.cuda.current_stream(idx).cuda_stream)
    buf = _flag_cache.get(key)
    if buf is None:
        buf = torch.zeros(64, dtype=torch.int32, device=torch.device("cuda", idx))
        _flag_cache[key] = buf
    return buf


def workspace(nbytes, device):
    idx = device.index if device.index is not None else torch.cuda.current_device()
    key = (idx, torch.cuda.current_stream(idx).cuda_stream)
    buf = _ws_cache.get(key)
    if buf is None or buf.numel() < nbytes:
        buf = torch.empty(max(int(nbytes), 1), dtype=torch.uint8, device=device)
        _ws_cache[key] = buf
    if _WS_POISON:
        buf[:int(nbytes)].fill_(0x7F)
    return buf


_WS_POISON = os.environ.get("MVR_WS_POISON") == "1"
```

### 3d_multiview_reg_amd/lib/descriptor/fcgf.py

```python
import os

import torch
import torch.nn as nn

from lib import _native as N
from lib.sparse import SparseTensor


CONV1_BRICKS = os.environ.get("MVR_CONV1_BRICKS", "1") == "1"
PRESPLIT = os.environ.get("MVR_SPCONV_PRESPLIT", "0") == "1"


def _planes(M, ld, dev):
    return torch.empty(M, 3, ld, dtype=torch.int16, device=dev) if PRESPLIT else None


class _MEConv(nn.Module):

    def __init__(self, cin, cout, ksize, has_bias=False):
        super().__init__()
        self.kernel_size = ksize
        self.kernel = nn.Parameter(torch.empty(ksize ** 3, cin, cout))
        nn.init.kaiming_normal_(self.kernel.data.view(-1, cout), nonlinearity="relu")
        self.bias = nn.Parameter(torch.zeros(1, cout)) if has_bias else None
# ... 9 lines not shown
            self._wimg = torch.empty(nb, dtype=torch.uint8, device=k.device)
            N.check(N.lib().mvr_spconv_wimage(N.ptr(k.data), K, cin, cout, N.ptr(self._wimg), nb, N.stream()),
                    "mvr_spconv_wimage")
            self._wimg_key = key
        return self._wimg


class _MENorm(nn.Module):

    def __init__(self, c, momentum=0.05):
        super().__init__()
        self.bn = nn.BatchNorm1d(c, momentum=momentum)


class BasicBlockBN(nn.Module):

    def __init__(self, inplanes, planes, bn_momentum=0.1):
        super().__init__()
        self.conv1 = _MEConv(inplanes, planes, 3)
        self.norm1 = _MENorm(planes, bn_momentum)
        self.conv2 = _MEConv(planes, planes, 3)
        self.norm2 = _MENorm(planes, bn_momentum)


def _bn(norm):
    if norm is None:
        return N.BnP(None, None, None, None), 1e-5
    b = norm.bn
    return N.BnP(b.weight.data_ptr(), b.bias.data_ptr(), b.running_mean.data_ptr(), b.running_var.data_ptr()), b.eps


class FCGFNet(nn.Module):
    NORM_TYPE = "BN"
    BLOCK_NORM_TYPE = "BN"
    CHANNELS = [None, 32, 64, 128, 256]
    TR_CHANNELS = [None, 64, 64, 64, 128]

    def __init__(self, in_channels=1, out_channels=32, bn_momentum=0.05, normalize_feature=True,
                 conv1_kernel_size=7, D=3):
        super().__init__()
        C, T = self.CHANNELS, self.TR_CHANNELS
        self.D = D
        self.normalize_feature = normalize_feature
        self.conv1_kernel_size = conv1_kernel_size
        self.conv1 = _MEConv(in_channels, C[1], conv1_kernel_size)
        self.norm1 = _MENorm(C[1], bn_momentum)
        self.block1 = BasicBlockBN(C[1], C[1], bn_momentum)
        self.conv2 = _MEConv(C[1], C[2], 3)
        self.norm2 = _MENorm(C[2], bn_momentum)
        self.block2 = BasicBlockBN(C[2], C[2], bn_momentum)
        self.conv3 = _MEConv(C[2], C[3], 3)
        self.norm3 = _MENorm(C[3], bn_momentum)
        self.block3 = BasicBlockBN(C[3], C[3], bn_momentum)
        self.conv4 = _MEConv(C[3], C[4], 3)
        self.norm4 = _MENorm(C[4], bn_momentum)
        self.block4 = BasicBlockBN(C[4], C[4], bn_momentum)
        self.conv4_tr = _MEConv(C[4], T[4], 3)
        self.norm4_tr = _MENorm(T[4], bn_momentum)
        self.block4_tr = BasicBlockBN(T[4], T[4], bn_momentum)
        self.conv3_tr = _MEConv(C[3] + T[4], T[3], 3)
        self.norm3_tr = _MENorm(T[3], bn_momentum)
        self.block3_tr = BasicBlockBN(T[3], T[3], bn_momentum)
        self.conv2_tr = _MEConv(C[2] + T[3], T[2], 3)
        self.norm2_tr = _MENorm(T[2], bn_momentum)
        self.block2_tr = BasicBlockBN(T[2], T[2], bn_momentum)
        self.conv1_tr = _MEConv(C[1] + T[2], T[1], 1)
        self.final = _MEConv(T[1], out_channels, 1, has_bias=True)

    def _conv(self, x, ldx, conv, km, M, out, ldout, norm=None, res=None, ldres=0, relu=False, bias=None, xp=None,
              outp=None):
        bnp, eps = _bn(norm)
        K, cin, cout = conv.kernel.shape
        nbr, perm = km if km is not None else (None, None)
        wimg = conv.wimage()
        N.check(N.lib().mvr_spconv_x(N.ptr(x), ldx, cin, N.ptr(nbr), N.ptr(perm), K, M, N.ptr(conv.kernel), cout,
                                     N.ptr(bias), bnp, eps, N.ptr(res), ldres, int(relu), N.ptr(out), ldout,
                                     N.ptr(wimg), N.ptr(N.flag_word(x.device)), N.ptr(xp), N.ptr(outp), N.stream()),
                "mvr_spconv_x")
        return out

    def _block(self, blk, x, ldx, km, M, out, ldout, xp=None, outp=None):
        c = blk.conv1.kernel.shape[2]
        t = torch.empty(M, c, device=x.device)
        tp = _planes(M, c, x.device)
        self._conv(x, ldx, blk.conv1, km, M, t, c, blk.norm1, relu=True, xp=xp, outp=tp)
        self._conv(t, c, blk.conv2, km, M, out, ldout, blk.norm2, res=x, ldres=ldx, relu=True, xp=tp, outp=outp)
        return out

    def forward(self, x):
        N.require_hip()
        f32 = torch.float32
        if not all(t.is_cuda and t.dtype is f32 and t.is_contiguous()
                   for t in (*self.parameters(), *self.buffers()) if t.dtype.is_floating_point):
            raise RuntimeError("FCGFNet parameters must be contiguous float32 on a HIP device")
        if self.training:
            raise NotImplementedError("FCGFNet on the HIP path runs in eval mode (BatchNorm running statistics)")
        cm = x.coords_man
        cm.prepare_orders()

        def km(kind, s):
            return cm.kernel_map(kind, s), cm.kernel_map_order(kind, s)
        dev = x.F.device
        C, T = self.CHANNELS, self.TR_CHANNELS
        M = [cm.coords_at(s).shape[0] for s in (1, 2, 4, 8)]
        L = N.lib()
        feat = x.F.float().contiguous()
        if feat.shape[1] != 1:
            raise NotImplementedError("conv1 kernel supports in_channels=1 (all reference configs)")
        s1 = torch.empty(M[0], C[1], device=dev)
        bnp, eps = _bn(self.norm1)
        bricks = cm.brick_map(1)
        oc = None if (self.conv1_kernel_size == 7 and CONV1_BRICKS) else N.ptr(cm.coords_at(1))
        s1p = _planes(M[0], C[1], dev) if oc is None else None
        N.check(L.mvr_spconv_c1_x(oc, M[0], N.ptr(bricks), M[0], bricks.numel(), N.ptr(feat),
                                  self.conv1_kernel_size, 1, N.ptr(self.conv1.kernel), C[1], bnp, eps, 0, N.ptr(s1),
                                  C[1], N.ptr(s1p), N.stream()), "mvr_spconv_c1_x")
        cat1 = torch.empty(M[0], T[2] + C[1], device=dev)
        cat2 = torch.empty(M[1], T[3] + C[2], device=dev)
        cat3 = torch.empty(M[2], T[4] + C[3], device=dev)
        w1, w2, w3 = cat1.shape[1], cat2.shape[1], cat3.shape[1]
        cat1p, cat2p, cat3p = (_planes(M[i], w, dev) for i, w in ((0, w1), (1, w2), (2, w3)))
        skip1, skip2, skip3 = cat1[:, T[2]:], cat2[:, T[3]:], cat3[:, T[4]:]

        def sl(p, c0):
            return p[:, :, c0:] if p is not None else None
        skip1p, skip2p, skip3p = sl(cat1p, T[2]), sl(cat2p, T[3]), sl(cat3p, T[4])
        self._block(self.block1, s1, C[1], km("s1", 1), M[0], skip1, w1, s1p, skip1p)
        t2 = torch.empty(M[1], C[2], device=dev)
        t2p = _planes(M[1], C[2], dev)
        self._conv(skip1, w1, self.conv2, km("down", 1), M[1], t2, C[2], self.norm2, xp=skip1p, outp=t2p)
        self._block(self.block2, t2, C[2], km("s1", 2), M[1], skip2, w2, t2p, skip2p)
        t3 = torch.empty(M[2], C[3], device=dev)
        t3p = _planes(M[2], C[3], dev)
        self._conv(skip2, w2, self.conv3, km("down", 2), M[2], t3, C[3], self.norm3, xp=skip2p, outp=t3p)
        self._block(self.block3, t3, C[3], km("s1", 4), M[2], skip3, w3, t3p, skip3p)
        t4 = torch.empty(M[3], C[4], device=dev)
        t4p = _planes(M[3], C[4], dev)
        self._conv(skip3, w3, self.conv4, km("down", 4), M[3], t4, C[4], self.norm4, xp=skip3p, outp=t4p)
        s8 = torch.empty(M[3], C[4], device=dev)
        s8p = _planes(M[3], C[4], dev)
        self._block(self.block4, t4, C[4], km("s1", 8), M[3], s8, C[4], t4p, s8p)
        u = torch.empty(M[2], T[4], device=dev)
        up = _planes(M[2], T[4], dev)
        self._conv(s8, C[4], self.conv4_tr, km("up", 4), M[2], u, T[4], self.norm4_tr, xp=s8p, outp=up)
        self._block(self.block4_tr, u, T[4], km("s1", 4), M[2], cat3, w3, up, cat3p)
        u = torch.empty(M[1], T[3], device=dev)
        up = _planes(M[1], T[3], dev)
        self._conv(cat3, w3, self.conv3_tr, km("up", 2), M[1], u, T[3], self.norm3_tr, xp=cat3p, outp=up)
        self._block(self.block3_tr, u, T[3], km("s1", 2), M[1], cat2, w2, up, cat2p)
        u = torch.empty(M[0], T[2], device=dev)
        up = _planes(M[0], T[2], dev)
        self._conv(cat2, w2, self.conv2_tr, km("up", 1), M[0], u, T[2], self.norm2_tr, xp=cat2p, outp=up)
        self._block(self.block2_tr, u, T[2], km("s1", 1), M[0], cat1, w1, up, cat1p)
        h = torch.empty(M[0], T[1], device=dev)
        hp = _planes(M[0], T[1], dev)
        self._conv(cat1, w1, self.conv1_tr, None, M[0], h, T[1], relu=True, xp=cat1p, outp=hp)
        cout = self.final.kernel.shape[2]
        out = torch.empty(M[0], cout, device=dev)
        self._conv(h, T[1], self.final, None, M[0], out, cout, bias=self.final.bias, xp=hp)
        if self.normalize_feature:
            N.check(L.mvr_l2norm_rows(N.ptr(out), M[0], cout, cout, N.stream()), "mvr_l2norm_rows")
        return SparseTensor(out, coords_key=1, coords_manager=cm)
```

### 3d_multiview_reg_amd/lib/filtering/oanet.py

```python
import ctypes
import logging

import torch
import torch.nn as nn

from lib import _native as N


class _Slots(nn.Module):

    def __init__(self, slots):
        super().__init__()
        for k in sorted(slots, key=int):
            self.add_module(str(k), slots[k])

    def __getitem__(self, i):
        return self._modules[str(i)]

    def __len__(self):
        return len(self._modules)


class DeviceFlag:
    __slots__ = ("_t", "_v")

    def __init__(self, t):
        self._t, self._v = t, None

    @property
    def tensor(self):
        return self._t

    def __bool__(self):
        if self._v is None:
            self._v = bool(self._t.item())
        return self._v

    def __eq__(self, other):
        return bool(self) == other

    def __hash__(self):
        return hash(bool(self))

    def __repr__(self):
        return repr(bool(self))


def _bn(c):
    return nn.BatchNorm2d(c)


def _conv(cin, cout):
    return nn.Conv2d(cin, cout, kernel_size=1)


class PointCN(nn.Module):

    def __init__(self, channels, out_channels=None):
        super().__init__()
        out_channels = out_channels or channels
        self.shot_cut = _conv(channels, out_channels) if out_channels != channels else None
        self.conv = _Slots({1: _bn(channels), 3: _conv(channels, out_channels), 5: _bn(out_channels),
                            7: _conv(out_channels, out_channels)})


class OAFilter(nn.Module):

    def __init__(self, channels, points):
        super().__init__()
        self.conv1 = _Slots({1: _bn(channels), 3: _conv(channels, channels)})
        self.conv2 = _Slots({0: _bn(points), 2: _conv(points, points)})
        self.conv3 = _Slots({2: _bn(channels), 4: _conv(channels, channels)})


class _Pool(nn.Module):

    def __init__(self, channels, clusters):
        super().__init__()
        self.output_points = clusters
        self.conv = _Slots({1: _bn(channels), 3: _conv(channels, clusters)})


class OANBlock(nn.Module):

    def __init__(self, net_channels, input_channel, depth, clusters, normalize_w=True):
        super().__init__()
        self.layer_num = depth
        self.in_channels = input_channel
        self.channels = net_channels
        self.clusters = clusters
        half = depth // 2
        if half > N.MAX_HALF:
            raise ValueError("net_depth too large for the native block (max %d layers per stage)" % (2 * N.MAX_HALF))
        logging.info("OANET: channels:%d, layer_num:%d", net_channels, depth)
        self.conv1 = _conv(input_channel, net_channels)
        self.l1_1 = _Slots({i: PointCN(net_channels) for i in range(half)})
        self.down1 = _Pool(net_channels, clusters)
        self.l2 = _Slots({i: OAFilter(net_channels, clusters) for i in range(half)})
        self.up1 = _Pool(net_channels, clusters)
        self.l1_2 = _Slots({i: (PointCN(2 * net_channels, net_channels) if i == 0 else PointCN(net_channels))
                            for i in range(half)})
        self.output = _conv(net_channels, 1)

    @staticmethod
    def _cp(conv):
        if conv is None:
            return N.ConvP(None, None)
        return N.ConvP(conv.weight.data_ptr(), conv.bias.data_ptr() if conv.bias is not None else None)

    @staticmethod
    def _bp(bn):
        return N.BnP(bn.weight.data_ptr(), bn.bias.data_ptr(), bn.running_mean.data_ptr(), bn.running_var.data_ptr())

    def _pcn(self, m):
        c = m.conv
        return N.PointCNP(self._bp(c[1]), self._cp(c[3]), self._bp(c[5]), self._cp(c[7]), self._cp(m.shot_cut))

    def native_params(self):
        for t in list(self.parameters()) + list(self.buffers()):
            if t.dtype.is_floating_point:
                if t.dtype != torch.float32 or not t.is_contiguous() or t.device.type != "cuda":
                    raise RuntimeError("OANBlock parameters must be contiguous float32 on a HIP device")
        p = N.OanBlockP()
        p.in_channels, p.channels, p.clusters, p.half_layers = (self.in_channels, self.channels, self.clusters,
                                                                self.layer_num // 2)
        p.conv1 = self._cp(self.conv1)
        for i in range(self.layer_num // 2):
            p.l1_1[i] = self._pcn(self.l1_1[i])
            f = self.l2[i]
            p.l2[i] = N.OAFilterP(self._bp(f.conv1[1]), self._cp(f.conv1[3]), self._bp(f.conv2[0]),
                                  self._cp(f.conv2[2]), self._bp(f.conv3[2]), self._cp(f.conv3[4]))
            p.l1_2[i] = self._pcn(self.l1_2[i])
        p.down_bn, p.down_conv = self._bp(self.down1.conv[1]), self._cp(self.down1.conv[3])
        p.up_bn, p.up_conv = self._bp(self.up1.conv[1]), self._cp(self.up1.conv[3])
        p.output = self._cp(self.output)
        return p


class OANet(nn.Module):

    def __init__(self, cfg):
        super().__init__()
        self.iter_num = cfg["misc"]["iter_num"]
        depth_each_stage = cfg["misc"]["net_depth"] // (cfg["misc"]["iter_num"] + 1)
        self.side_channel = (cfg["data"]["use_mutuals"] == 2)
        C, K = cfg["misc"]["net_channel"], cfg["misc"]["clusters"]
        nrm = cfg["misc"]["normalize_weights"]
        self.reg_init = OANBlock(C, 6 + self.side_channel, depth_each_stage, K, nrm)
        self.reg_iter = _Slots({i: OANBlock(C, 8 + self.side_channel, depth_each_stage, K, nrm)
                                for i in range(self.iter_num)})
        self.device = torch.device("cuda" if (torch.cuda.is_available() and cfg["misc"]["use_gpu"]) else "cpu")
        self.guard_group = 0
        self.guard_sync = None
        self.bn_group = 0

    def forward(self, data):
        xs_in = data["xs"]
        assert xs_in.dim() == 4 and xs_in.shape[1] == 1
        N.require_hip()
        dev = self.reg_init.conv1.weight.device
        N.require_hip(self.reg_init.conv1.weight)
        xs = xs_in.to(dev, torch.float32)[:, 0].contiguous()
        P, Npts, Cxs = xs.shape
        ld = (Npts + 31) // 32 * 32
        if Cxs < 6:
            raise ValueError("xs must have at least 6 channels (x1 | x2)")
        L = N.lib()
        st = N.stream()
        rows = Cxs + 2
        inp = torch.zeros(P, rows, ld, device=dev, dtype=torch.float32)
        N.check(L.mvr_xs_to_channels(N.ptr(xs), Npts * Cxs, Cxs, Cxs, P, Npts, N.ptr(inp), rows * ld, ld, st),
                "mvr_xs_to_channels")
        blocks = [self.reg_init] + [self.reg_iter[i] for i in range(self.iter_num)]
        C = self.reg_init.channels
        ws_bytes = max(L.mvr_oan_block_workspace_bytes(C, self.reg_init.clusters, b.in_channels, P, Npts)
                       for b in blocks)
        ws = N.workspace(ws_bytes, dev)
        guard = torch.empty(P, dtype=torch.int32, device=dev)
        status = torch.zeros(len(blocks), P, dtype=torch.int32, device=dev)
        latent = torch.empty(P, C, ld, device=dev, dtype=torch.float32)
        out = {"logits": [], "scores": [], "rot_est": [], "trans_est": []}
        for bi, blk in enumerate(blocks):
            params = blk.native_params()
            logits = torch.empty(P, Npts, device=dev)
            scores = torch.empty(P, Npts, device=dev)
            R = torch.empty(P, 3, 3, device=dev)
            t = torch.empty(P, 3, 1, device=dev)
            res = torch.empty(P, Npts, device=dev)
            if N._WS_POISON:
                for x in (logits, scores, R, t, res, latent):
                    x.fill_(3.0e38)
            last = bi == len(blocks) - 1
            ext = self.guard_sync is not None
            res_row = None if last else N.ptr(inp[:, Cxs])
            score_row = None if last else N.ptr(inp[:, Cxs + 1])
            rc = L.mvr_oan_block_forward(
                ctypes.byref(params), N.ptr(inp), rows * ld, ld, N.ptr(xs), Npts * Cxs, Cxs, P, Npts,
                (int(self.bn_group) if self.bn_group > 1 else 1) if self.training else 0,
                N.ptr(logits), N.ptr(scores), N.ptr(R), N.ptr(t), N.ptr(res), N.ptr(latent) if last else None,
                res_row, score_row, rows * ld, N.ptr(guard), N.ptr(status[bi]), -1 if ext else int(self.guard_group),
                N.ptr(ws), ws.numel(), st)
            N.check(rc, "mvr_oan_block_forward")
            if ext:
                gp = self.guard_sync(guard)
                N.check(L.mvr_procrustes(N.ptr(xs), N.ptr(xs[..., 3:]), Npts * Cxs, Cxs, N.ptr(scores), Npts, N.ptr(gp),
                                         None, 0, P, Npts, 1, 1e-7, N.ptr(R), N.ptr(t), N.ptr(res), Npts,
                                         res_row, rows * ld, N.ptr(status[bi]), 0, st), "mvr_procrustes")
                if not last:
                    inp[:, Cxs + 1, :Npts].copy_(scores)
            if bi == 0 and not last:
                blk_in_ch = blocks[1].in_channels
                if blk_in_ch != rows:
                    raise ValueError("reg_iter input channels %d != %d" % (blk_in_ch, rows))
            for k, v in zip(("logits", "scores", "rot_est", "trans_est"), (logits, scores, R, t)):
                out[k].append(v)
        out["latent features"] = latent[:, :, :Npts].unsqueeze(3)
        out["gradient_flag"] = DeviceFlag(status.any())
        return out
```

### include/mvreg.h

```cpp
#ifndef MVREG_H
#define MVREG_H
#include <stddef.h>
#include <stdint.h>

#ifdef __cplusplus
extern "C" {
#endif

typedef struct ihipStream_t* mvr_stream_t;

#define MVR_OK 0
#define MVR_EINVAL -1
#define MVR_ELAUNCH -2

int mvr_procrustes(const float* x1, const float* x2, int64_t x_pstride, int64_t x_nstride, float* w,
                   int64_t w_pstride, const int32_t* guard_pos, float* w_copy, int64_t wc_pstride, int P, int N,
                   int normalize, float eps, float* R, float* t, float* res, int64_t res_pstride, float* res_copy,
                   int64_t rc_pstride, int32_t* status, int guard_group, mvr_stream_t stream);
int mvr_procrustes_f64(const double* x1, const double* x2, int64_t x_pstride, int64_t x_nstride, double* w,
                       int64_t w_pstride, const int32_t* guard_pos, double* w_copy, int64_t wc_pstride, int P, int N,
                       int normalize, double eps, double* R, double* t, double* res, int64_t res_pstride,
                       double* res_copy, int64_t rc_pstride, int32_t* status, int guard_group,
                       mvr_stream_t stream);

size_t mvr_ransac_workspace_bytes(int P, int iters);
int mvr_ransac(const double* x1, const double* x2, int64_t x_pstride, const int32_t* n, int P, int ransac_n,
               int iters, double max_dist, uint64_t seed, double* T, double* fitness, double* rmse,
               int32_t* best_iter, double* hyp_out, void* workspace, size_t workspace_bytes, mvr_stream_t stream);

#define MVR_SYNC_MAX_FRAGS 128
size_t mvr_sync_workspace_bytes(int S, int max_frags, int max_edges);
int mvr_sync_poses(const double* R_pair, const double* t_pair, const int32_t* ij, const double* w, int64_t e_sstride,
                   const int32_t* n_edges, const int32_t* n_frags, int S, int max_frags, int max_edges, int anchor,
                   int irls_iters, double c_rot, double c_trans, double* R, double* t, int64_t f_sstride,
                   int32_t* member, double* w_out, double* res_rot, double* res_trans, int32_t* status,
                   void* workspace, size_t workspace_bytes, mvr_stream_t stream);

int mvr_set_math(int mode);
int mvr_debug_force(int what, int value);

int mvr_gemm_f32(int M, int N, int K, int batch, const float* A, int64_t sAb, int64_t lda, const float* B,
                 int64_t sBb, int64_t ldb, int b_kcontig, float* C, int64_t sCb, int64_t ldc, const float* R,
                 int64_t sRb, const float* bias, int bias_mode, const float* psc, const float* psh, int64_t sPb,
                 int64_t pld, int pro, float* stats, int64_t st_ld, int st_off, int stats_mode, int math,
                 int32_t* range_flag, mvr_stream_t stream);
int mvr_oaf_conv2_f32(int M, int N, int K, int batch, const float* A, int64_t sAb, int64_t lda, const float* W,
                      int64_t ldw, float* C, int64_t sCb, int64_t ldc, const float* R, int64_t sRb, const float* bias,
                      const float* psc, const float* psh, int64_t sPb, float* stats, int64_t st_ld, void* img,
                      int64_t img_bytes, mvr_stream_t stream);
size_t mvr_oaf_conv2_image_bytes(int N, int K);

typedef struct { const float* weight; const float* bias; } mvr_conv_p;
typedef struct { const float* gamma; const float* beta; const float* mean; const float* var; } mvr_bn_p;
typedef struct { mvr_bn_p bn1; mvr_conv_p conv3; mvr_bn_p bn5; mvr_conv_p conv7; mvr_conv_p shortcut; } mvr_pointcn_p;
typedef struct {
  mvr_bn_p bn1; mvr_conv_p conv1;
  mvr_bn_p bn2; mvr_conv_p conv2;
  mvr_bn_p bn3; mvr_conv_p conv3;
} mvr_oafilter_p;

#define MVR_OAN_MAX_HALF 8
typedef struct {
  int in_channels;
  int channels;
  int clusters;
  int half_layers;
  mvr_conv_p conv1;
  mvr_pointcn_p l1_1[MVR_OAN_MAX_HALF];
  mvr_bn_p down_bn; mvr_conv_p down_conv;
  mvr_oafilter_p l2[MVR_OAN_MAX_HALF];
  mvr_bn_p up_bn; mvr_conv_p up_conv;
  mvr_pointcn_p l1_2[MVR_OAN_MAX_HALF];
  mvr_conv_p output;
} mvr_oan_block_p;

size_t mvr_oan_block_workspace_bytes(int channels, int clusters, int in_channels, int P, int N);

int mvr_attn_reruns(int reset);
int mvr_debug_stage_hash(unsigned long long* buf, int cap);
int mvr_debug_stage_dump(int stage, void* dst, size_t bytes);
int mvr_oan_last_layout(void);
int mvr_oan_block_forward(const mvr_oan_block_p* blk, const float* input, int64_t in_pstride, int64_t ld,
                          const float* xs, int64_t xs_pstride, int64_t xs_nstride, int P, int N, int bn_train,
                          float* logits,
                          float* scores, float* R, float* t, float* res, float* latent, float* res_row,
                          float* score_row, int64_t row_pstride, int32_t* guard_pos, int32_t* status, int guard_group,
                          void* workspace,
                          size_t workspace_bytes, mvr_stream_t stream);

int mvr_oan_diff_pool(const float* x, int64_t x_pstride, int64_t x_ld, const float* sc, const float* sh,
                      int64_t s_pstride, const float* weight, const float* bias, int P, int channels, int N,
                      int clusters, float* out, int64_t out_pstride, int64_t out_ld, float* stats, int64_t st_ld,
                      int st_off, mvr_stream_t stream);
size_t mvr_oan_diff_pool_workspace_bytes(int P, int channels, int clusters);
int mvr_oan_diff_pool_ws(const float* x, int64_t x_pstride, int64_t x_ld, const float* sc, const float* sh,
                         int64_t s_pstride, const float* weight, const float* bias, int P, int channels, int N,
                         int clusters, float* out, int64_t out_pstride, int64_t out_ld, float* stats, int64_t st_ld,
                         int st_off, void* workspace, size_t workspace_bytes, mvr_stream_t stream);

size_t mvr_oan_diff_unpool_workspace_bytes(int P, int channels, int clusters);
int mvr_oan_diff_unpool(const float* x_up, int64_t x_pstride, int64_t x_ld, const float* sc, const float* sh,
                        int64_t s_pstride, const float* weight, const float* bias, const float* x_down,
                        int64_t xd_pstride, int64_t xd_ld, int P, int channels, int N, int clusters, float* out,
                        int64_t out_pstride, int64_t out_ld, float* stats, int64_t st_ld, int st_off,
                        void* workspace, size_t workspace_bytes, mvr_stream_t stream);

int mvr_xs_to_channels(const float* xs, int64_t xs_pstride, int64_t xs_nstride, int C, int P, int N, float* out,
                       int64_t out_pstride, int64_t out_ld, mvr_stream_t stream);

size_t mvr_voxel_centroids_workspace_bytes(int64_t n);
int mvr_voxel_centroids(const float* xyz, const int64_t* frag_off, int B, int64_t n, double voxel, void* workspace,
                        size_t workspace_bytes, double* out_xyz, int64_t* out_off, mvr_stream_t stream);
size_t mvr_radius_index_bytes(int64_t M);
int mvr_radius_index_build(const double* xyz, const int64_t* off, int B, int64_t M, double r, void* index,
                           size_t bytes, mvr_stream_t stream);
int mvr_radius_overlap_count(const void* index, size_t bytes, const double* xyz, const int64_t* off, int B,
                             int64_t M, const int64_t* pairs, const double* T, int P, int64_t max_points, double r,
                             int32_t* counts, mvr_stream_t stream);

int mvr_icp_refine(const void* index, size_t index_bytes, const double* xyz, const int64_t* off, int B, int64_t M,
                   double r_index, const int64_t* pairs, const double* T0, int P, double max_dist, int max_iters,
                   double tol_fitness, double tol_rmse, double* T, double* fitness, double* rmse, int32_t* n_corr,
                   int32_t* iters, int32_t* status, double* trace, mvr_stream_t stream);

int mvr_estimate_normals(const void* index, size_t index_bytes, const double* xyz, const int64_t* off, int B,
                         int64_t M, double r_index, double radius, const double* viewpoints, double* normals,
                         int32_t* n_nbr, mvr_stream_t stream);

int mvr_icp_refine_plane(const void* index, size_t index_bytes, const double* xyz, const double* normals,
                         const int64_t* off, int B, int64_t M, double r_index, const int64_t* pairs, const double* T0,
                         int P, double max_dist, int max_iters, double tol_fitness, double tol_rmse, double* T,
                         double* fitness, double* rmse, int32_t* n_corr, int32_t* iters, int32_t* status,
                         double* trace, mvr_stream_t stream);

int mvr_icp_refine_generalized(const void* index, size_t index_bytes, const double* xyz, const double* normals,
                               const int64_t* off, int B, int64_t M, double r_index, const int64_t* pairs,
                               const double* T0, int P, double max_dist, double epsilon, int max_iters,
                               double tol_fitness, double tol_rmse, double* T, double* fitness, double* rmse,
                               int32_t* n_corr, int32_t* iters, int32_t* status, double* trace, mvr_stream_t stream);

int mvr_pair_information(const void* index, size_t index_bytes, const double* xyz, const int64_t* off, int B,
                         int64_t M, double r_index, const int64_t* pairs, const double* T, int P, double max_dist,
                         double* info, int32_t* n_corr, double* rmse, int32_t* status, mvr_stream_t stream);

size_t mvr_compute_fpfh_workspace_bytes(int64_t M);
int mvr_compute_fpfh(const void* index, size_t index_bytes, const double* xyz, const double* normals,
                     const int64_t* off, int B, int64_t M, double r_index, double radius, float* fpfh,
                     float* spfh_out, void* workspace, size_t workspace_bytes, mvr_stream_t stream);

int mvr_feat_match(const float* F, int C, const int64_t* off, int B, int64_t M, const int64_t* pairs,
                   const int64_t* qoff, int P, int64_t n_queries, int64_t max_q, int32_t* idx, float* dist2,
                   mvr_stream_t stream);

size_t mvr_posegraph_workspace_bytes(int S, int max_frags, int max_edges);
int mvr_posegraph_optimize(const double* R_pair, const double* t_pair, const int32_t* ij, const double* w,
                           const double* info, int64_t e_sstride, const int32_t* n_edges, const int32_t* n_frags,
                           int S, int max_frags, int max_edges, int anchor, const double* R0, const double* t0,
                           int max_iters, double lambda0, double tol_cost, double tol_step, double* R, double* t,
                           int64_t f_sstride, int32_t* member, double* cost, int32_t* iters, int32_t* status,
                           double* trace, void* workspace, size_t workspace_bytes, mvr_stream_t stream);

size_t mvr_fuse_scene_workspace_bytes(int64_t M);
int mvr_fuse_scene(const double* xyz, const double* normals, const int64_t* off, int B, int64_t M,
                   const double* poses, const uint8_t* member, double voxel, void* workspace, size_t workspace_bytes,
                   double* out_xyz, double* out_normals, int32_t* out_n_points, int32_t* out_n_frags,
                   int64_t* out_count, mvr_stream_t stream);

int mvr_fps(const float* xyz, const int64_t* offsets, const int64_t* offsets_host, int B, int m, int64_t* idx_out,
            mvr_stream_t stream);

int mvr_knn1(const float* pos1, int64_t p1_bstride, int64_t p1_rstride, const float* pos2, int64_t p2_bstride,
             int64_t p2_rstride, int B, int N, int M, float* dist_out, int64_t* idx_out, mvr_stream_t stream);

int mvr_mutuals(const float* x1, int64_t x1_bstride, int64_t x1_rstride, const float* x2, int64_t x2_bstride,
                int64_t x2_rstride, const float* x1m, int64_t x1m_bstride, int64_t x1m_rstride, const float* x2m,
                int64_t x2m_bstride, int64_t x2m_rstride, int B, int N, float thr2, float* flag_out, int64_t* idx_out,
                mvr_stream_t stream);

int mvr_feat_nn(const float* Fq, int64_t fq_fstride, const float* Ft, int64_t ft_fstride, const float* Xq,
                int64_t xq_fstride, const float* Xt, int64_t xt_fstride, const int64_t* pairs, int P, int Nq, int Mt,
                int C, float inv_tau2, int mode, float* out, int64_t out_pstride, int64_t out_nstride,
                int32_t* idx_out, mvr_stream_t stream);
size_t mvr_feat_nn_workspace_bytes(int n_frag, int Mt);
int mvr_feat_nn_ws(const float* Fq, int64_t fq_fstride, const float* Ft, int64_t ft_fstride, const float* Xq,
                   int64_t xq_fstride, const float* Xt, int64_t xt_fstride, const int64_t* pairs, int P, int Nq,
                   int Mt, int C, float inv_tau2, int mode, float* out, int64_t out_pstride, int64_t out_nstride,
                   int32_t* idx_out, int n_frag, void* workspace, size_t workspace_bytes, mvr_stream_t stream);

int mvr_feat_nn_gumbel(const float* Fq, int64_t fq_fstride, const float* Ft, int64_t ft_fstride, const float* Xq,
                       int64_t xq_fstride, const float* Xt, int64_t xt_fstride, const int64_t* pairs, int P, int Nq,
                       int Mt, int C, float inv_tau, int hard, uint64_t seed, float* out, int64_t out_pstride,
                       int64_t out_nstride, int32_t* idx_out, mvr_stream_t stream);

int mvr_feat_knn2(const float* Fq, int64_t fq_fstride, const float* Ft, int64_t ft_fstride, const int64_t* pairs,
                  int P, int Nq, int Mt, int C, int32_t* idx2_out, double* dist2_out, mvr_stream_t stream);

int mvr_gather_rows(const float* src, int C, const int64_t* idx, int n, float* dst, mvr_stream_t stream);

size_t mvr_hash_table_bytes(int64_t M);
size_t mvr_voxelize_workspace_bytes(int64_t n);
int mvr_voxelize(const float* xyz, const int64_t* frag_off, int B, int64_t n, double voxel, void* workspace,
                 size_t workspace_bytes, int32_t* coords_out, int64_t* sel_out, int64_t* counts_out,
                 mvr_stream_t stream);
int mvr_voxelize_f64(const double* xyz, const int64_t* frag_off, int B, int64_t n, double voxel, void* workspace,
                     size_t workspace_bytes, int32_t* coords_out, int64_t* sel_out, int64_t* counts_out,
                     mvr_stream_t stream);
size_t mvr_voxelize_hint_workspace_bytes(int64_t n, int64_t distinct_hint);
int mvr_voxelize_hint(const float* xyz, const int64_t* frag_off, int B, int64_t n, double voxel,
                      int64_t distinct_hint, void* ws, size_t ws_bytes, int32_t* coords_out, int64_t* sel_out,
                      int64_t* counts_out, mvr_stream_t stream);
size_t mvr_coords_downsample_workspace_bytes(int64_t M);
int mvr_coords_downsample(const int32_t* coords, int64_t M, int B, int stride_out, void* workspace,
                          size_t workspace_bytes, int32_t* coords_out, int64_t* counts_out, mvr_stream_t stream);
int mvr_hash_build(const int32_t* coords, int64_t M, void* table, size_t table_bytes, mvr_stream_t stream);
int mvr_hash_build_lattice(const int32_t* coords, int64_t M, int stride, void* table, size_t table_bytes,
                           mvr_stream_t stream);
int mvr_kernel_map(const int32_t* out_coords, int64_t Mout, const void* in_table, size_t in_table_bytes, int ksize,
                   int step, int transposed, int32_t* nbr, mvr_stream_t stream);
int mvr_kernel_map_x(const int32_t* out_coords, int64_t Mout, const void* in_table, size_t in_table_bytes, int ksize,
                     int step, int transposed, int32_t* nbr, const int32_t* row_order, mvr_stream_t stream);
int mvr_kernel_map_sym(const int32_t* coords, int64_t M, const void* table, size_t table_bytes, int step, int32_t* nbr,
                       mvr_stream_t stream);
int mvr_kernel_map_transpose(const int32_t* src, int64_t Ms, int K, int32_t* dst, int64_t Md, mvr_stream_t stream);
size_t mvr_kernel_map_order_bytes(int64_t Mout);
int mvr_kernel_map_order(const int32_t* nbr, const int32_t* out_coords, int step, int64_t Mout, int K, int32_t* perm,
                         void* workspace, size_t workspace_bytes, mvr_stream_t stream);
size_t mvr_kernel_map_orders_bytes(int64_t total);
int mvr_kernel_map_orders(int n_maps, const int32_t* const* nbr, const int32_t* const* out_coords, const int* steps,
                          const int64_t* Mo, int K, int32_t* perm_out, void* workspace, size_t workspace_bytes,
                          mvr_stream_t stream);
size_t mvr_radix_sort_pairs_bytes(int64_t n);
int mvr_radix_sort_pairs(const uint64_t* keys, const int32_t* vals, int64_t n, int bits, int32_t* vals_out,
                         void* workspace, size_t workspace_bytes, mvr_stream_t stream);
int mvr_spconv(const float* in, int64_t ldin, int Cin, const int32_t* nbr, const int32_t* perm, int K, int64_t Mout,
               const float* W, int Cout, const float* bias, mvr_bn_p bn, float bn_eps, const float* res,
               int64_t ldres, int relu, float* out, int64_t ldout, const void* wimg, int32_t* range_flag,
               mvr_stream_t stream);
int mvr_spconv_x(const float* in, int64_t ldin, int Cin, const int32_t* nbr, const int32_t* perm, int K, int64_t Mout,
                 const float* W, int Cout, const float* bias, mvr_bn_p bn, float bn_eps, const float* res,
                 int64_t ldres, int relu, float* out, int64_t ldout, const void* wimg, int32_t* range_flag,
                 const uint16_t* in_planes, uint16_t* out_planes, mvr_stream_t stream);
size_t mvr_spconv_wimage_bytes(int K, int Cin, int Cout);
int mvr_spconv_wimage(const float* W, int K, int Cin, int Cout, void* img, size_t bytes, mvr_stream_t stream);
size_t mvr_brick_map_bytes(int64_t M);
int mvr_brick_map_build(const int32_t* coords, int64_t M, void* workspace, size_t workspace_bytes,
                        mvr_stream_t stream);
int mvr_brick_map_build_stride(const int32_t* coords, int64_t M, int stride, void* workspace, size_t workspace_bytes,
                               mvr_stream_t stream);
int mvr_spconv_c1(const int32_t* out_coords, int64_t Mout, const void* in_bricks, int64_t Min, size_t in_bricks_bytes,
                  const float* feat, int ksize, int step, const float* W, int Cout, mvr_bn_p bn, float bn_eps,
                  int relu, float* out, int64_t ldout, mvr_stream_t stream);
int mvr_spconv_c1_x(const int32_t* out_coords, int64_t Mout, const void* in_bricks, int64_t Min,
                    size_t in_bricks_bytes, const float* feat, int ksize, int step, const float* W, int Cout,
                    mvr_bn_p bn, float bn_eps, int relu, float* out, int64_t ldout, uint16_t* out_planes,
                    mvr_stream_t stream);
int mvr_l2norm_rows(float* x, int64_t M, int C, int64_t ld, mvr_stream_t stream);

int mvr_sample_rand_mt19937(uint32_t* key, int32_t* pos, const int64_t* counts, int B, int tgt, int64_t* out,
                            int64_t* ws);

int mvr_prof_set(int on);
int mvr_prof_mask(unsigned mask);
int mvr_prof_get(int kind, double* ms, long long* launches, double* flops, double* bytes);
int mvr_prof_seq(int* kinds, double* bytes, int cap);
int mvr_source_hash(char* buf, size_t cap);

#ifdef __cplusplus
}
#endif
#endif
```

Baseline: 10950 pairs/s.

## Fuse FCGF head convs with L2 norm and cache prepared OANet weight images

Adds a fused FCGF head kernel that runs the 96->64 ReLU conv, the 64->32 conv with bias and the row L2 normalisation in one pass, keeping the hidden activations in shared memory. OANet inference now precomputes the weight images (conv2 split images, unpool split weights, folded BN) once per weight version and reuses them across calls, skipping the per-call split kernels. The diff also adds a conv1_fast switch and runtime opt switches. The risks are stale-cache correctness if weights change in place without a version bump, and a new hand-written MFMA path for the head.

Result: no change. 11010 pairs/s, median of 6 (+0.6%).

```diff
diff --git a/3d_multiview_reg_amd/csrc/fcgf_head.hip b/3d_multiview_reg_amd/csrc/fcgf_head.hip
--- /dev/null
+++ b/3d_multiview_reg_amd/csrc/fcgf_head.hip
@@ -0,0 +1,158 @@
+#include <algorithm>
+
+#include "common.hpp"
+#include "knobs.hpp"
+#include "mfma_bf16.hpp"
+#include "prof.hpp"
+
+namespace mvr {
+
+#ifndef FCGF_HEAD_DEFAULT
+#define FCGF_HEAD_DEFAULT 1
+#endif
+int g_fcgf_head = FCGF_HEAD_DEFAULT;
+
+namespace {
+
+using namespace bx;
+
+constexpr int FH_CIN = 96, FH_CH = 64, FH_CO = 32;
+constexpr int FH_BST = 40;
+constexpr int FH_CP = 128;
+constexpr int FH_WAVES = 8;
+constexpr int FH_HLD = 68;
+
+struct FhSmem {
+  uint16_t wa[FH_CIN / 32][3][FH_CH][FH_BST];
+  uint16_t wb[FH_CH / 32][3][FH_CO][FH_BST];
+  float hs[FH_WAVES][32 * FH_HLD];
+};
+
+__global__ __launch_bounds__(64 * FH_WAVES, 1) void fcgf_head_kernel(const float* __restrict__ x, int64_t ldx, int64_t M,
+                                                                     const uint16_t* __restrict__ wimg1,
+                                                                     const uint16_t* __restrict__ wimg2,
+                                                                     const float* __restrict__ bias2,
+                                                                     float* __restrict__ out, int64_t ldout) {
+  __shared__ __attribute__((aligned(16))) FhSmem sm;
+  const int tid = threadIdx.x, lane = tid & 63, l32 = lane & 31, h = lane >> 5;
+  const int w = __builtin_amdgcn_readfirstlane(tid >> 6);
+  {
+    constexpr int GA = FH_CH * FH_BST * 2 / 16, GB = FH_CO * FH_BST * 2 / 16;
+    const char* s1 = reinterpret_cast<const char*>(wimg1);
+    const char* s2 = reinterpret_cast<const char*>(wimg2);
+    for (int g = tid; g < (FH_CIN / 32) * 3 * GA; g += blockDim.x) {
+      const int blk = g / GA, r = g - blk * GA;
+      *reinterpret_cast<u32x4*>(reinterpret_cast<char*>(sm.wa) + g * 16) =
+          *reinterpret_cast<const u32x4*>(s1 + (int64_t)blk * FH_CP * FH_BST * 2 + r * 16);
+    }
+    for (int g = tid; g < (FH_CH / 32) * 3 * GB; g += blockDim.x) {
+      const int blk = g / GB, r = g - blk * GB;
+      *reinterpret_cast<u32x4*>(reinterpret_cast<char*>(sm.wb) + g * 16) =
+          *reinterpret_cast<const u32x4*>(s2 + (int64_t)blk * FH_CP * FH_BST * 2 + r * 16);
+    }
+  }
+  __syncthreads();
+  const float bias = bias2 ? bias2[l32] : 0.f;
+  float* hs = sm.hs[w];
+  const int64_t nslab = (M + 31) / 32;
+  auto load_rows = [&](int64_t slab, float4 (&r)[12]) {
+    const int64_t row = slab * 32 + l32 < M ? slab * 32 + l32 : M - 1;
+    const float* p = x + row * ldx + 8 * h;
+#pragma unroll
+    for (int s = 0; s < 3; ++s)
+#pragma unroll
+      for (int q = 0; q < 4; ++q) r[4 * s + q] = *reinterpret_cast<const float4*>(p + 32 * s + 16 * (q >> 1) + 4 * (q & 1));
+  };
+  auto frag = [&](const float4& x0, const float4& x1) {
+    const float v[8] = {x0.x, x0.y, x0.z, x0.w, x1.x, x1.y, x1.z, x1.w};
+    return split8t<0>(v);
+  };
+  const int64_t stride = (int64_t)gridDim.x * FH_WAVES;
+  int64_t slab = (int64_t)blockIdx.x * FH_WAVES + w;
+  float4 xr[12], xn[12];
+  if (slab < nslab) load_rows(slab, xr);
+  for (; slab < nslab; slab += stride) {
+    load_rows(slab + stride < nslab ? slab + stride : slab, xn);
+    floatx16 a0, a1;
+#pragma unroll
+    for (int r = 0; r < 16; ++r) a0[r] = a1[r] = 0.f;
+#pragma unroll
+    for (int s = 0; s < 3; ++s)
+#pragma unroll
+      for (int st = 0; st < 2; ++st) {
+        const FragT<0> fa = frag(xr[4 * s + 2 * st], xr[4 * s + 2 * st + 1]);
+        const FragT<0> f0 = ld_frag<0>(reinterpret_cast<const char*>(&sm.wa[s][0][l32][16 * st + 8 * h]), FH_CH * FH_BST * 2);
+        const FragT<0> f1 = ld_frag<0>(reinterpret_cast<const char*>(&sm.wa[s][0][32 + l32][16 * st + 8 * h]), FH_CH * FH_BST * 2);
+        a0 = mma<0>(fa, f0, a0);
+        a1 = mma<0>(fa, f1, a1);
+      }
+#pragma unroll
+    for (int r = 0; r < 16; ++r) {
+      const int row = (r & 3) + 8 * (r >> 2) + 4 * h;
+      float v0 = a0[r] + 0.f, v1 = a1[r] + 0.f;
+      v0 = fmaf(v0, 1.f, 0.f);
+      v1 = fmaf(v1, 1.f, 0.f);
+      hs[row * FH_HLD + l32] = fmaxf(v0, 0.f);
+      hs[row * FH_HLD + 32 + l32] = fmaxf(v1, 0.f);
+    }
+    asm volatile("s_waitcnt lgkmcnt(0)" ::: "memory");
+    floatx16 b;
+#pragma unroll
+    for (int r = 0; r < 16; ++r) b[r] = 0.f;
+#pragma unroll
+    for (int s = 0; s < 2; ++s)
+#pragma unroll
+      for (int st = 0; st < 2; ++st) {
+        const float* hp = hs + l32 * FH_HLD + 32 * s + 16 * st + 8 * h;
+        const FragT<0> fa = frag(*reinterpret_cast<const float4*>(hp), *reinterpret_cast<const float4*>(hp + 4));
+        const FragT<0> fb = ld_frag<0>(reinterpret_cast<const char*>(&sm.wb[s][0][l32][16 * st + 8 * h]), FH_CO * FH_BST * 2);
+        b = mma<0>(fa, fb, b);
+      }
+    asm volatile("s_waitcnt lgkmcnt(0)" ::: "memory");
+#pragma unroll
+    for (int r = 0; r < 16; ++r) {
+      float v = b[r] + bias;
+      v = fmaf(v, 1.f, 0.f);
+      hs[((r & 3) + 8 * (r >> 2) + 4 * h) * FH_HLD + l32] = v;
+    }
+    asm volatile("s_waitcnt lgkmcnt(0)" ::: "memory");
+#pragma unroll
+    for (int it = 0; it < 4; ++it) {
+      const int row = (lane >> 3) + 8 * it, part = lane & 7;
+      const float4 v = *reinterpret_cast<const float4*>(hs + row * FH_HLD + 4 * part);
+      float s = v.x * v.x + v.y * v.y + v.z * v.z + v.w * v.w;
+      s += __shfl_xor(s, 1, 64);
+      s += __shfl_xor(s, 2, 64);
+      s += __shfl_xor(s, 4, 64);
+      const float inv = 1.f / sqrtf(s);
+      const int64_t o = slab * 32 + row;
+      if (o < M) *reinterpret_cast<float4*>(out + o * ldout + 4 * part) = make_float4(v.x * inv, v.y * inv, v.z * inv, v.w * inv);
+    }
+    asm volatile("s_waitcnt lgkmcnt(0)" ::: "memory");
+#pragma unroll
+    for (int i = 0; i < 12; ++i) xr[i] = xn[i];
+  }
+}
+
+}
+}
+
+using namespace mvr;
+
+extern "C" int mvr_fcgf_head(const float* x, int64_t ldx, int64_t M, const void* wimg1, const void* wimg2,
+                             const float* bias2, float* out, int64_t ldout, hipStream_t s) {
+  if (M < 0 || ldx < FH_CIN || ldout < FH_CO || (ldx & 3) || (ldout & 3)) return MVR_EINVAL;
+  if (M == 0) return MVR_OK;
+  if (!x || !wimg1 || !wimg2 || !out) return MVR_EINVAL;
+  if ((reinterpret_cast<uintptr_t>(x) | reinterpret_cast<uintptr_t>(out) | reinterpret_cast<uintptr_t>(wimg1) |
+       reinterpret_cast<uintptr_t>(wimg2)) & 15)
+    return MVR_EINVAL;
+  ProfScope prof(PK_SPCONV, 2.0 * M * (FH_CIN * FH_CH + FH_CH * FH_CO), (double)M * (FH_CIN + FH_CO) * 4.0, s);
+  const int64_t nslab = (M + 31) / 32;
+  const int grid = (int)std::min<int64_t>(GPU_CUS, (nslab + FH_WAVES - 1) / FH_WAVES);
+  hipLaunchKernelGGL(fcgf_head_kernel, dim3(grid), dim3(64 * FH_WAVES), 0, s, x, ldx, M,
+                     reinterpret_cast<const uint16_t*>(wimg1), reinterpret_cast<const uint16_t*>(wimg2), bias2, out,
+                     ldout);
+  MVR_CHECK_LAUNCH();
+  return MVR_OK;
+}
diff --git a/3d_multiview_reg_amd/csrc/gemm.hip b/3d_multiview_reg_amd/csrc/gemm.hip
--- a/3d_multiview_reg_amd/csrc/gemm.hip
+++ b/3d_multiview_reg_amd/csrc/gemm.hip
@@ -1193,12 +1193,22 @@
          (int64_t)c2_nks(g.K) * c2_npad(g.N) * C2_BK * 2 * 3 < ((int64_t)1 << 31);
 }
 
+int oaf_conv2_wimage(const float* W, int N, int K, int64_t ldw, uint16_t* wimg, int64_t wimg_bytes, hipStream_t s) {
+  if (!W || !wimg || N <= 0 || K <= 0 || wimg_bytes < oaf_conv2_image_bytes(N, K)) return MVR_EINVAL;
+  const int Npad = c2_npad(N), nks = c2_nks(K);
+  const int64_t nthr = (int64_t)nks * Npad * 4;
+  hipLaunchKernelGGL(oaf_w_image_kernel, dim3((unsigned)((nthr + 255) / 256)), dim3(256), 0, s, W, N, K, ldw, Npad, nks,
+                     wimg);
+  MVR_CHECK_LAUNCH();
+  return MVR_OK;
+}
+
 static int launch_oaf_conv2(const GemmArgs& g, hipStream_t s) {
-  const int Npad = c2_npad(g.N), nks = c2_nks(g.K);
-  const int64_t nthr = (int64_t)nks * Npad * 4;
-  hipLaunchKernelGGL(oaf_w_image_kernel, dim3((unsigned)((nthr + 255) / 256)), dim3(256), 0, s, g.B, g.N, g.K, g.ldb,
-                     Npad, nks, g.wimg);
-  MVR_CHECK_LAUNCH();
+  const int Npad = c2_npad(g.N);
+  if (!g.wimg_ready) {
+    const int e = oaf_conv2_wimage(g.B, g.N, g.K, g.ldb, g.wimg, g.wimg_bytes, s);
+    if (e) return e;
+  }
   const long long tiles = (long long)(Npad / C2_BN) * g.batch;
   const unsigned wgs = (unsigned)(tiles < GPU_CUS ? tiles : GPU_CUS);
   hipLaunchKernelGGL(oaf_conv2_kernel, dim3(wgs), dim3(C2_THREADS), 0, s, g, (const uint16_t*)g.wimg);
diff --git a/3d_multiview_reg_amd/csrc/gemm.hpp b/3d_multiview_reg_amd/csrc/gemm.hpp
--- a/3d_multiview_reg_amd/csrc/gemm.hpp
+++ b/3d_multiview_reg_amd/csrc/gemm.hpp
@@ -48,6 +48,7 @@
   float fin_eps2; mvr_bn_p fin_bn2; float* fin_sc2; float* fin_sh2;
   int fin_train; float2* fin_mv; int* fin_done;
   uint16_t* wimg; int64_t wimg_bytes;
+  int wimg_ready;
   int64_t bcs, ccs, rcs, ldr;
 };
 
@@ -64,9 +65,12 @@
                        const float* sh, int64_t s_pstride, const float* weight, const float* bias, const float* x_down,
                        int64_t xd_pstride, int64_t xd_ld, int P, int channels, int N, int clusters, float* out,
                        int64_t out_pstride, int64_t out_ld, int64_t out_cs, float* stats, int64_t st_ld, int st_off,
-                       void* workspace, size_t workspace_bytes, hipStream_t stream);
+                       void* workspace, size_t workspace_bytes, hipStream_t stream, const void* wimage = nullptr);
+size_t oan_unpool_wimage_bytes(int clusters);
+int oan_unpool_wimage(const float* weight, const float* bias, int clusters, void* wimage, hipStream_t stream);
 
 int64_t oaf_conv2_image_bytes(int N, int K);
+int oaf_conv2_wimage(const float* W, int N, int K, int64_t ldw, uint16_t* wimg, int64_t wimg_bytes, hipStream_t stream);
 
 inline int gemm_ntiles(int N){ return (N + GEMM_BN - 1) / GEMM_BN; }
 inline int gemm_mtiles(int M) { return (M + GEMM_BM - 1) / GEMM_BM; }
diff --git a/3d_multiview_reg_amd/csrc/knobs.hip b/3d_multiview_reg_amd/csrc/knobs.hip
--- a/3d_multiview_reg_amd/csrc/knobs.hip
+++ b/3d_multiview_reg_amd/csrc/knobs.hip
@@ -15,6 +15,21 @@
   return prev;
 }
 
+extern "C" int mvr_set_opt(int what, int value) {
+  using namespace mvr;
+  int* sw[OPT_COUNT] = {&g_conv1_fast, &g_oan_prepared, &g_fcgf_head};
+  if (what < 0 || what >= OPT_COUNT || value < 0 || value > 1) return MVR_EINVAL;
+  const int prev = *sw[what];
+  *sw[what] = value;
+  return prev;
+}
+
+extern "C" int mvr_get_opt(int what) {
+  using namespace mvr;
+  const int* sw[OPT_COUNT] = {&g_conv1_fast, &g_oan_prepared, &g_fcgf_head};
+  return what < 0 || what >= OPT_COUNT ? MVR_EINVAL : *sw[what];
+}
+
 extern "C" int mvr_debug_force(int what, int value) {
   using namespace mvr;
   if (what == FORCE_FEAT_NN_ONLINE) {
diff --git a/3d_multiview_reg_amd/csrc/knobs.hpp b/3d_multiview_reg_amd/csrc/knobs.hpp
--- a/3d_multiview_reg_amd/csrc/knobs.hpp
+++ b/3d_multiview_reg_amd/csrc/knobs.hpp
@@ -22,4 +22,14 @@
 };
 extern int g_force[FORCE_COUNT];
 
+enum OptSwitch : int {
+  OPT_CONV1_FAST = 0,
+  OPT_OAN_PREPARED = 1,
+  OPT_FCGF_HEAD = 2,
+  OPT_COUNT = 3
+};
+extern int g_conv1_fast;
+extern int g_oan_prepared;
+extern int g_fcgf_head;
+
 }
diff --git a/3d_multiview_reg_amd/csrc/oan_attn.hip b/3d_multiview_reg_amd/csrc/oan_attn.hip
--- a/3d_multiview_reg_amd/csrc/oan_attn.hip
+++ b/3d_multiview_reg_amd/csrc/oan_attn.hip
@@ -1158,10 +1158,11 @@
                             const float* x_down, int64_t xd_pstride, int64_t xd_ld, int P, int channels, int N,
                             int clusters, float* out, int64_t out_pstride, int64_t out_ld, int64_t out_cs,
                             float* stats, int64_t st_ld, int st_off, void* workspace, size_t workspace_bytes,
-                            hipStream_t stream) {
+                            hipStream_t stream, const void* wimage) {
   if (P < 0 || N <= 0 || channels != AC || clusters <= 0 || clusters > MAX_CLUSTERS) return MVR_EINVAL;
   if (P == 0) return MVR_OK;
   if (!x_up || !sc || !sh || !weight || !x_down || !out || !workspace) return MVR_EINVAL;
+  if (wimage && !al16(wimage)) return MVR_EINVAL;
   auto bad_layout = [&](int64_t ld, int64_t cs) {
     return cs != 32 ? (ld != 32 || (cs & 3) || cs < 32 * AC) : ld < round_up4(N);
   };
@@ -1182,6 +1183,11 @@
   a.X = x_up; a.xps = x_pstride; a.xld = x_ld; a.xcs = x_cs;
   a.sc = sc; a.sh = sh; a.sps = s_pstride;
   a.wimg = wimg; a.bias = bias; a.bs = bs; a.dimg = dimg;
+  const bool wready = wimage && !g_attn_h;
+  if (wready) {
+    a.wimg = reinterpret_cast<const char*>(wimage);
+    a.bs = reinterpret_cast<const float2*>(a.wimg + (size_t)nkb * WIMG);
+  }
   a.P = P; a.N = N; a.Kc = clusters; a.nkb = nkb; a.nqb = (N + AQ - 1) / AQ;
   a.out = out; a.ops = out_pstride; a.old = out_ld; a.ocs = out_cs;
   a.stats = reinterpret_cast<float2*>(stats); a.st_ld = st_ld; a.st_off = st_off;
@@ -1205,23 +1211,43 @@
       a.range = nullptr;
       a.guard = guard = range;
     }
-    hipLaunchKernelGGL(split_w_kernel<0>, gw, dim3(256), 0, stream, weight, bias, clusters, nkb, wimg, bs, nullptr,
-                       guard);
-    MVR_CHECK_LAUNCH();
+    if (!wready) {
+      hipLaunchKernelGGL(split_w_kernel<0>, gw, dim3(256), 0, stream, weight, bias, clusters, nkb, wimg, bs, nullptr,
+                         guard);
+      MVR_CHECK_LAUNCH();
+    }
     hipLaunchKernelGGL(split_xd_kernel, gx, dim3(256), 0, stream, x_down, xd_pstride, xd_ld, P, clusters, nkb, dimg,
                        guard);
     MVR_CHECK_LAUNCH();
     hipLaunchKernelGGL(oan_unpool4_kernel<0>, dim3(grid), dim3(U4T), 0, stream, a);
   } else {
-    hipLaunchKernelGGL(split_w_kernel<0>, gw, dim3(256), 0, stream, weight, bias, clusters, nkb, wimg, bs, nullptr,
-                       nullptr);
-    MVR_CHECK_LAUNCH();
+    if (!wready) {
+      hipLaunchKernelGGL(split_w_kernel<0>, gw, dim3(256), 0, stream, weight, bias, clusters, nkb, wimg, bs, nullptr,
+                         nullptr);
+      MVR_CHECK_LAUNCH();
+    }
     hipLaunchKernelGGL(split_xd_kernel, gx, dim3(256), 0, stream, x_down, xd_pstride, xd_ld, P, clusters, nkb, dimg,
                        nullptr);
     MVR_CHECK_LAUNCH();
     const int grid = ((P + 7) / 8) * 8 * a.nqb;
     hipLaunchKernelGGL(oan_unpool_kernel, dim3(grid), dim3(ATHREADS), 0, stream, a);
   }
+  MVR_CHECK_LAUNCH();
+  return MVR_OK;
+}
+
+size_t mvr::oan_unpool_wimage_bytes(int clusters) {
+  if (clusters <= 0 || clusters > MAX_CLUSTERS) return 0;
+  const size_t nkb = (size_t)(clusters + AKB - 1) / AKB;
+  return nkb * (WIMG + AKB * sizeof(float2));
+}
+
+int mvr::oan_unpool_wimage(const float* weight, const float* bias, int clusters, void* wimage, hipStream_t stream) {
+  if (!weight || !wimage || !al16(wimage) || clusters <= 0 || clusters > MAX_CLUSTERS) return MVR_EINVAL;
+  const int nkb = (clusters + AKB - 1) / AKB;
+  char* wimg = reinterpret_cast<char*>(wimage);
+  hipLaunchKernelGGL(split_w_kernel<0>, dim3((nkb * 512 + 255) / 256), dim3(256), 0, stream, weight, bias, clusters,
+                     nkb, wimg, reinterpret_cast<float2*>(wimg + (size_t)nkb * WIMG), nullptr, nullptr);
   MVR_CHECK_LAUNCH();
   return MVR_OK;
 }
diff --git a/3d_multiview_reg_amd/csrc/oanet.hip b/3d_multiview_reg_amd/csrc/oanet.hip
--- a/3d_multiview_reg_amd/csrc/oanet.hip
+++ b/3d_multiview_reg_amd/csrc/oanet.hip
@@ -387,6 +387,40 @@
   return pl;
 }
 
+}
+#ifndef OAN_PREPARED_DEFAULT
+#define OAN_PREPARED_DEFAULT 1
+#endif
+int g_oan_prepared = OAN_PREPARED_DEFAULT;
+namespace {
+
+struct Prep {
+  float *W1, *W8;
+  void* uw;
+  float* scK[MVR_OAN_MAX_HALF];
+  float* shK[MVR_OAN_MAX_HALF];
+  uint16_t* w2img[MVR_OAN_MAX_HALF];
+  int64_t w2img_bytes;
+  size_t bytes;
+};
+
+Prep prep_plan(int C, int Kc, int Cin, int H, void* base) {
+  Prep pp{};
+  Ws w{reinterpret_cast<char*>(base), 0, 0};
+  pp.W1 = w.take<float>((size_t)C * round4(Cin));
+  pp.W8 = w.take<float>((size_t)C * 8);
+  const size_t ub = C == 128 ? oan_unpool_wimage_bytes(Kc) : 0;
+  pp.uw = ub ? w.take<char>(ub) : nullptr;
+  pp.w2img_bytes = oaf_conv2_image_bytes(Kc, Kc);
+  for (int i = 0; i < H; ++i) {
+    pp.scK[i] = w.take<float>((size_t)round32(Kc));
+    pp.shK[i] = w.take<float>((size_t)round32(Kc));
+    pp.w2img[i] = w.take<uint16_t>((size_t)pp.w2img_bytes / 2);
+  }
+  pp.bytes = w.off + 256;
+  return pp;
+}
+
 struct Ctx {
   const Plan& pl;
   hipStream_t s;
@@ -396,6 +430,7 @@
   bool f16;
   int err = 0;
   int nflag = 0;
+  const Prep* prep = nullptr;
   int nfin = 0;
   int fcur = 0;
   float* sc() const { return fcur ? pl.sc2 : pl.sc; }
@@ -519,15 +554,20 @@
     return yf;
   }
 
-  bool oafilter(const mvr_oafilter_p& f, const Act& xd, const FoldReq* next = nullptr, bool x_folded = false) {
+  bool oafilter(const mvr_oafilter_p& f, const Act& xd, const FoldReq* next = nullptr, bool x_folded = false,
+                int idx = 0) {
     const int C = pl.C, Kc = pl.Kc;
     const int64_t Kp = pl.Kp;
     if (!x_folded) finalize_in(xd, 1e-3f, f.bn1);
     Act o1{pl.O1, (int64_t)C * Kp, Kp, C, Kc, pl.stcol, Kc, 0};
     conv(f.conv1, xd, true, o1, nullptr, train ? ST_COL : ST_NONE);
+    const float *scK = pl.scK, *shK = pl.shK;
     if (train) {
       hipLaunchKernelGGL(bn_col_train_kernel, dim3((Kc + 255) / 256, ngroups()), dim3(256), 0, s, pl.stcol, pl.P,
                          bn_group, gemm_mtiles(C), Kc, C, f.bn2, pl.scK, pl.shK, Kp);
+    } else if (prep) {
+      scK = prep->scK[idx];
+      shK = prep->shK[idx];
     } else {
       hipLaunchKernelGGL(bn_fold_eval_kernel, dim3((Kc + 255) / 256), dim3(256), 0, s, f.bn2, Kc, pl.scK, pl.shK);
     }
@@ -541,11 +581,12 @@
     g.C = o2.p; g.sCb = o2.ps; g.ldc = Kp;
     g.R = pl.O1; g.sRb = (int64_t)C * Kp; g.has_res = 1;
     g.bias = f.conv2.bias; g.bias_mode = BIAS_N;
-    g.pro = PRO_A_K; g.psc = pl.scK; g.psh = pl.shK; g.sPb = train ? Kp : 0;
+    g.pro = PRO_A_K; g.psc = scK; g.psh = shK; g.sPb = train ? Kp : 0;
     g.stats_mode = ST_ROW; g.stats = o2.st; g.st_ld = C; g.st_off = 0;
     g.prof_kind = PK_OAFILTER;
     g.flag = flag();
     g.wimg = pl.w2img; g.wimg_bytes = pl.w2img_bytes;
+    if (prep) { g.wimg = prep->w2img[idx]; g.wimg_bytes = prep->w2img_bytes; g.wimg_ready = 1; }
     chk(launch_gemm(g, s));
     finalize_in(o2, 1e-3f, f.bn3);
     return conv(f.conv3, o2, true, xd, &xd, ST_ROW, nullptr, false, next);
@@ -566,6 +607,39 @@
 
 extern "C" size_t mvr_oan_block_workspace_bytes(int channels, int clusters, int in_channels, int P, int N) {
   return plan(channels, clusters, in_channels, P, N, nullptr).bytes;
+}
+
+extern "C" size_t mvr_oan_block_prepare_bytes(int channels, int clusters, int in_channels, int half_layers) {
+  if (channels <= 0 || clusters <= 0 || in_channels <= 0 || half_layers <= 0 || half_layers > MVR_OAN_MAX_HALF) return 0;
+  return prep_plan(channels, clusters, in_channels, half_layers, nullptr).bytes;
+}
+
+extern "C" int mvr_oan_block_prepare(const mvr_oan_block_p* blk, void* prepared, size_t prepared_bytes, hipStream_t s) {
+  if (!blk || !prepared || (reinterpret_cast<uintptr_t>(prepared) & 15)) return MVR_EINVAL;
+  const int C = blk->channels, Kc = blk->clusters, H = blk->half_layers, Cin = blk->in_channels;
+  if (C <= 0 || Kc <= 0 || H <= 0 || H > MVR_OAN_MAX_HALF || Cin <= 0) return MVR_EINVAL;
+  const Prep pp = prep_plan(C, Kc, Cin, H, prepared);
+  if (prepared_bytes < pp.bytes) return MVR_EINVAL;
+  if (!blk->conv1.weight || !blk->up_conv.weight) return MVR_EINVAL;
+  const int n1 = (int)(C * round4(Cin)), n8 = C * 8;
+  hipLaunchKernelGGL(pad_cols_kernel, dim3((n1 + 255) / 256), dim3(256), 0, s, blk->conv1.weight, C, Cin,
+                     (int)round4(Cin), pp.W1);
+  if (Cin <= 8)
+    hipLaunchKernelGGL(pad_cols_kernel, dim3((n8 + 255) / 256), dim3(256), 0, s, blk->conv1.weight, C, Cin, 8, pp.W8);
+  MVR_CHECK_LAUNCH();
+  if (pp.uw) {
+    const int e = oan_unpool_wimage(blk->up_conv.weight, blk->up_conv.bias, Kc, pp.uw, s);
+    if (e) return e;
+  }
+  for (int i = 0; i < H; ++i) {
+    const mvr_oafilter_p& f = blk->l2[i];
+    if (!f.bn2.gamma || !f.bn2.beta || !f.bn2.mean || !f.bn2.var || !f.conv2.weight) return MVR_EINVAL;
+    hipLaunchKernelGGL(bn_fold_eval_kernel, dim3((Kc + 255) / 256), dim3(256), 0, s, f.bn2, Kc, pp.scK[i], pp.shK[i]);
+    MVR_CHECK_LAUNCH();
+    const int e = oaf_conv2_wimage(f.conv2.weight, Kc, Kc, Kc, pp.w2img[i], pp.w2img_bytes, s);
+    if (e) return e;
+  }
+  return MVR_OK;
 }
 
 extern "C" int mvr_oan_block_forward(const mvr_oan_block_p* blk, const float* input, int64_t in_pstride, int64_t ld,
@@ -574,6 +648,18 @@
                                      float* latent, float* res_row, float* score_row, int64_t row_pstride,
                                      int32_t* guard_pos, int32_t* status, int guard_group, void* workspace,
                                      size_t workspace_bytes, hipStream_t s) {
+  return mvr_oan_block_forward_prepared(blk, input, in_pstride, ld, xs, xs_pstride, xs_nstride, P, N, bn_train, logits,
+                                        scores, R, t, res, latent, res_row, score_row, row_pstride, guard_pos, status,
+                                        guard_group, workspace, workspace_bytes, nullptr, 0, s);
+}
+
+extern "C" int mvr_oan_block_forward_prepared(const mvr_oan_block_p* blk, const float* input, int64_t in_pstride,
+                                              int64_t ld, const float* xs, int64_t xs_pstride, int64_t xs_nstride,
+                                              int P, int N, int bn_train, float* logits, float* scores, float* R,
+                                              float* t, float* res, float* latent, float* res_row, float* score_row,
+                                              int64_t row_pstride, int32_t* guard_pos, int32_t* status,
+                                              int guard_group, void* workspace, size_t workspace_bytes,
+                                              const void* prepared, size_t prepared_bytes, hipStream_t s) {
   if (P < 0 || N < 0) return MVR_EINVAL;
   if (P == 0) return MVR_OK;
   if (!blk || !input || !xs || !logits || !scores || !R || !t || !res || !guard_pos || !workspace) return MVR_EINVAL;
@@ -584,7 +670,18 @@
   if (!blk->l1_2[0].shortcut.weight) return MVR_EINVAL;
   Plan pl = plan(C, Kc, Cin, P, N, workspace);
   if (workspace_bytes < pl.bytes) return MVR_EINVAL;
+  Prep pp{};
+  if (prepared) {
+    if (reinterpret_cast<uintptr_t>(prepared) & 15) return MVR_EINVAL;
+    pp = prep_plan(C, Kc, Cin, H, const_cast<void*>(prepared));
+    if (prepared_bytes < pp.bytes) return MVR_EINVAL;
+  }
   Ctx cx{pl, s, bn_train ? 1 : 0, bn_train > 1 ? std::min(bn_train, P) : P, g_gemm_h || g_pconv_h};
+  if (prepared && !bn_train && g_oan_prepared) {
+    cx.prep = &pp;
+    pl.W1 = pp.W1;
+    pl.W8 = pp.W8;
+  }
   if (cx.f16 && hipMemsetAsync(pl.flags, 0, sizeof(int) * FLAG_SLOTS, s) != hipSuccess) return MVR_ELAUNCH;
   if (OAN_FUSED_FIN && hipMemsetAsync(pl.fcnt, 0, sizeof(int) * FIN_SLOTS * P, s) != hipSuccess)
     return MVR_ELAUNCH;
@@ -594,10 +691,12 @@
 
   const float* w1 = nullptr;
   if (Cin % 4) {
-    const int n = (int)(C * pl.Cinp);
-    hipLaunchKernelGGL(pad_cols_kernel, dim3((n + 255) / 256), dim3(256), 0, s, blk->conv1.weight, C, Cin,
-                       (int)pl.Cinp, pl.W1);
-    cx.chk_launch();
+    if (!cx.prep) {
+      const int n = (int)(C * pl.Cinp);
+      hipLaunchKernelGGL(pad_cols_kernel, dim3((n + 255) / 256), dim3(256), 0, s, blk->conv1.weight, C, Cin,
+                         (int)pl.Cinp, pl.W1);
+      cx.chk_launch();
+    }
     w1 = pl.W1;
   }
   Act in{const_cast<float*>(input), in_pstride, ld, Cin, N, nullptr, 0, 0};
@@ -632,7 +731,8 @@
   bool yfold = false;
   if (fold1) {
     const int n8 = C * 8;
-    hipLaunchKernelGGL(pad_cols_kernel, dim3((n8 + 255) / 256), dim3(256), 0, s, blk->conv1.weight, C, Cin, 8, pl.W8);
+    if (!cx.prep)
+      hipLaunchKernelGGL(pad_cols_kernel, dim3((n8 + 255) / 256), dim3(256), 0, s, blk->conv1.weight, C, Cin, 8, pl.W8);
     hipLaunchKernelGGL(xin_stats_kernel, dim3((TN + 3) / 4, P), dim3(256), 0, s, input, in_pstride, ld, Cin, N, TN,
                        pl.W8, blk->conv1.bias, pl.stA);
     cx.chk_launch();
@@ -709,7 +809,7 @@
   bool xdfold = false;
   for (int i = 0; i < H; ++i) {
     const FoldReq fn{1e-3f, i + 1 < H ? blk->l2[i + 1].bn1 : mvr_bn_p{}};
-    xdfold = cx.oafilter(blk->l2[i], xd, i + 1 < H ? &fn : nullptr, xdfold);
+    xdfold = cx.oafilter(blk->l2[i], xd, i + 1 < H ? &fn : nullptr, xdfold, i);
     dbg_hash(pl.XD, P, C, Kc, (int64_t)C * Kp, Kp, s);
   }
 
@@ -717,7 +817,8 @@
   if (pl.fused) {
     cx.chk(oan_diff_unpool_cm(pl.X11, 2 * CN, x11top.ld, x11cs, pl.scU, pl.shU, C, blk->up_conv.weight,
                               blk->up_conv.bias, pl.XD, (int64_t)C * Kp, Kp, P, C, N, Kc, pl.X11 + C * x11top.ld, 2 * CN,
-                              x11top.ld, x11cs, reinterpret_cast<float*>(pl.st11), 2 * C, C, pl.uimg, pl.uimg_bytes, s));
+                              x11top.ld, x11cs, reinterpret_cast<float*>(pl.st11), 2 * C, C, pl.uimg, pl.uimg_bytes, s,
+                              cx.prep ? cx.prep->uw : nullptr));
   } else {
     Act e2{pl.E, (int64_t)Kc * Np, Np, Kc, N, pl.smx, N, 0};
     cx.conv(blk->up_conv, x11top, true, e2, nullptr, ST_COLSMX, nullptr, false, nullptr, pl.scU, pl.shU);
diff --git a/3d_multiview_reg_amd/csrc/sparse.hip b/3d_multiview_reg_amd/csrc/sparse.hip
--- a/3d_multiview_reg_amd/csrc/sparse.hip
+++ b/3d_multiview_reg_amd/csrc/sparse.hip
@@ -511,19 +511,33 @@
   float sc[32], sh[32];
 };
 
+__device__ int g_c1_fast_bricks;
+#ifndef CONV1_FAST_DEFAULT
+#define CONV1_FAST_DEFAULT 1
+#endif
+int g_conv1_fast = CONV1_FAST_DEFAULT;
+
+__device__ __forceinline__ bool bf16_exact(float v) {
+  const unsigned b = __float_as_uint(v), e = (b >> 23) & 0xff;
+  return (b & 0xffffu) == 0 && e != 0xff && (e != 0 || (b << 1) == 0);
+}
+
 __global__ __launch_bounds__(512) void spconv_c1_brick_kernel(BrickView bv, const float* __restrict__ feat,
                                                               const float* __restrict__ W, mvr_bn_p bn,
                                                               float bn_eps, int relu, float* __restrict__ out,
-                                                              int64_t ldout, uint16_t* __restrict__ outp) {
+                                                              int64_t ldout, uint16_t* __restrict__ outp, int fast) {
   using namespace bx;
   __shared__ __attribute__((aligned(16))) C1Smem sm;
   const int tid = threadIdx.x, lane = tid & 63, l32 = lane & 31, hh = lane >> 5;
   const int w = tid >> 6;
+  bool wfin = true;
   for (int e = tid; e < C1_NS * 64; e += blockDim.x) {
     const int s = e >> 6, ln = e & 63, k0 = 16 * s + 8 * (ln >> 5), c = ln & 31;
     float v[8];
 #pragma unroll
     for (int i = 0; i < 8; ++i) v[i] = k0 + i < C1_K ? W[(k0 + i) * 32 + c] : 0.f;
+#pragma unroll
+    for (int i = 0; i < 8; ++i) wfin = wfin && fabsf(v[i]) < __builtin_inff();
     Frag f;
     split8(v, f.h, f.m, f.l);
     sm.wf[s][0][ln] = f.h;
@@ -542,7 +556,8 @@
     sm.sc[tid] = sc;
     sm.sh[tid] = sh;
   }
-  __syncthreads();
+  const bool fastw = __syncthreads_and(wfin) && fast;
+  int nfast = 0;
   const float csc = sm.sc[l32], csh = sm.sh[l32];
   const int base0 = (l32 & 3) + C1_G * ((l32 >> 2) & 3) + C1_G * C1_G * (l32 >> 4);
   const int base1 = base0 + 2 * C1_G * C1_G;
@@ -576,6 +591,31 @@
     floatx16 acc0, acc1;
 #pragma unroll
     for (int r = 0; r < 16; ++r) acc0[r] = acc1[r] = 0.f;
+    bool exact = fastw;
+#pragma unroll
+    for (int i = 0; i < 16; ++i) exact = exact && bf16_exact(fv[i]);
+    if (__all(exact)) {
+      ++nfast;
+#pragma unroll 2
+      for (int s = 0; s < C1_NS; ++s) {
+        const s16x8 o = *reinterpret_cast<const s16x8*>(&sm.off[16 * s + 8 * hh]);
+        const bf16x8 wh = sm.wf[s][0][lane], wm = sm.wf[s][1][lane], wl = sm.wf[s][2][lane];
+        unsigned p0[4], p1[4];
+#pragma unroll
+        for (int i = 0; i < 4; ++i) {
+          p0[i] = (__float_as_uint(g[base0 + o[2 * i]]) >> 16) | (__float_as_uint(g[base0 + o[2 * i + 1]]) & 0xffff0000u);
+          p1[i] = (__float_as_uint(g[base1 + o[2 * i]]) >> 16) | (__float_as_uint(g[base1 + o[2 * i + 1]]) & 0xffff0000u);
+        }
+        const bf16x8 a0 = __builtin_bit_cast(bf16x8, u32x4{p0[0], p0[1], p0[2], p0[3]});
+        const bf16x8 a1 = __builtin_bit_cast(bf16x8, u32x4{p1[0], p1[1], p1[2], p1[3]});
+        acc0 = __builtin_amdgcn_mfma_f32_32x32x16_bf16(a0, wl, acc0, 0, 0, 0);
+        acc0 = __builtin_amdgcn_mfma_f32_32x32x16_bf16(a0, wm, acc0, 0, 0, 0);
+        acc0 = __builtin_amdgcn_mfma_f32_32x32x16_bf16(a0, wh, acc0, 0, 0, 0);
+        acc1 = __builtin_amdgcn_mfma_f32_32x32x16_bf16(a1, wl, acc1, 0, 0, 0);
+        acc1 = __builtin_amdgcn_mfma_f32_32x32x16_bf16(a1, wm, acc1, 0, 0, 0);
+        acc1 = __builtin_amdgcn_mfma_f32_32x32x16_bf16(a1, wh, acc1, 0, 0, 0);
+      }
+    } else {
 #pragma unroll 2
     for (int s = 0; s < C1_NS; ++s) {
       const s16x8 o = *reinterpret_cast<const s16x8*>(&sm.off[16 * s + 8 * hh]);
@@ -594,6 +634,7 @@
       split8(v1, a1.h, a1.m, a1.l);
       acc0 = mfma6(a0, wf, acc0);
       acc1 = mfma6(a1, wf, acc1);
+    }
     }
 #pragma unroll
     for (int q = 0; q < 16; ++q) {
@@ -612,6 +653,7 @@
       }
     }
   }
+  if (lane == 0 && nfast) atomicAdd(&g_c1_fast_bricks, nfast);
 }
 
 __global__ void l2norm_rows_kernel(float* x, int64_t M, int C, int64_t ld) {
@@ -979,7 +1021,7 @@
     ProfScope prof(PK_SPCONV, 2.0 * Mout * C1_K * Cout, (double)Mout * (16 + Cout * 4), s);
     const int grid = (int)std::min<int64_t>(256, (Mout + 63) / 64);
     hipLaunchKernelGGL(spconv_c1_brick_kernel, dim3(grid), dim3(512), 0, s, v, feat, W, bn, bn_eps, relu, out,
-                       ldout, out_planes);
+                       ldout, out_planes, g_conv1_fast);
     MVR_CHECK_LAUNCH();
     return MVR_OK;
   }
@@ -1001,6 +1043,18 @@
                              mvr_bn_p bn, float bn_eps, int relu, float* out, int64_t ldout, hipStream_t s) {
   return mvr_spconv_c1_x(out_coords, Mout, in_bricks, Min, in_bricks_bytes, feat, ksize, step, W, Cout, bn, bn_eps,
                          relu, out, ldout, nullptr, s);
+}
+
+extern "C" int mvr_conv1_fast_bricks(int reset) {
+  int v = 0;
+  if (hipDeviceSynchronize() != hipSuccess ||
+      hipMemcpyFromSymbol(&v, HIP_SYMBOL(g_c1_fast_bricks), sizeof(int)) != hipSuccess)
+    return -1;
+  if (reset) {
+    const int z = 0;
+    if (hipMemcpyToSymbol(HIP_SYMBOL(g_c1_fast_bricks), &z, sizeof(int)) != hipSuccess) return -1;
+  }
+  return v;
 }
 
 extern "C" int mvr_l2norm_rows(float* x, int64_t M, int C, int64_t ld, hipStream_t s) {
diff --git a/3d_multiview_reg_amd/lib/_native.py b/3d_multiview_reg_amd/lib/_native.py
--- a/3d_multiview_reg_amd/lib/_native.py
+++ b/3d_multiview_reg_amd/lib/_native.py
@@ -61,6 +61,10 @@
     "mvr_oan_block_workspace_bytes": (c_size, [c_int, c_int, c_int, c_int, c_int]),
     "mvr_set_math": (c_int, [c_int]),
     "mvr_debug_force": (c_int, [c_int, c_int]),
+    "mvr_set_opt": (c_int, [c_int, c_int]),
+    "mvr_get_opt": (c_int, [c_int]),
+    "mvr_fcgf_head": (c_int, [c_vp, c_i64, c_i64, c_vp, c_vp, c_vp, c_vp, c_i64, c_vp]),
+    "mvr_conv1_fast_bricks": (c_int, [c_int]),
     "mvr_attn_reruns": (c_int, [c_int]),
     "mvr_debug_stage_hash": (c_int, [c_vp, c_int]),
     "mvr_debug_stage_dump": (c_int, [c_int, c_vp, c_size]),
@@ -75,6 +79,11 @@
     "mvr_oan_block_forward": (c_int, [ctypes.POINTER(OanBlockP), c_vp, c_i64, c_i64, c_vp, c_i64, c_i64, c_int, c_int, c_int,
                                       c_vp, c_vp, c_vp, c_vp, c_vp, c_vp, c_vp, c_vp, c_i64, c_vp, c_vp, c_int, c_vp,
                                       c_size, c_vp]),
+    "mvr_oan_block_prepare_bytes": (c_size, [c_int, c_int, c_int, c_int]),
+    "mvr_oan_block_prepare": (c_int, [ctypes.POINTER(OanBlockP), c_vp, c_size, c_vp]),
+    "mvr_oan_block_forward_prepared": (c_int, [ctypes.POINTER(OanBlockP), c_vp, c_i64, c_i64, c_vp, c_i64, c_i64, c_int,
+                                               c_int, c_int, c_vp, c_vp, c_vp, c_vp, c_vp, c_vp, c_vp, c_vp, c_i64, c_vp,
+                                               c_vp, c_int, c_vp, c_size, c_vp, c_size, c_vp]),
     "mvr_feat_nn": (c_int, [c_vp, c_i64, c_vp, c_i64, c_vp, c_i64, c_vp, c_i64, c_vp, c_int, c_int, c_int, c_int,
                             c_float, c_int, c_vp, c_i64, c_i64, c_vp, c_vp]),
     "mvr_feat_nn_gumbel": (c_int, [c_vp, c_i64, c_vp, c_i64, c_vp, c_i64, c_vp, c_i64, c_vp, c_int, c_int, c_int,
@@ -281,6 +290,28 @@
         lib().mvr_debug_force(self.what, self.prev)
 
 
+OPT = {"conv1_fast": 0, "oan_prepared": 1, "fcgf_head": 2}
+
+
+def get_opt(what):
+    return lib().mvr_get_opt(OPT[what])
+
+
+class opt:
+
+    def __init__(self, what, value):
+        self.what, self.value = OPT[what], int(value)
+
+    def __enter__(self):
+        self.prev = lib().mvr_set_opt(self.what, self.value)
+        if self.prev < 0:
+            raise ValueError("mvr_set_opt(%d, %d) rejected" % (self.what, self.value))
+        return self
+
+    def __exit__(self, *a):
+        lib().mvr_set_opt(self.what, self.prev)
+
+
 _ws_cache = {}
 _flag_cache = {}
 
diff --git a/3d_multiview_reg_amd/lib/descriptor/fcgf.py b/3d_multiview_reg_amd/lib/descriptor/fcgf.py
--- a/3d_multiview_reg_amd/lib/descriptor/fcgf.py
+++ b/3d_multiview_reg_amd/lib/descriptor/fcgf.py
@@ -185,11 +185,16 @@
         up = _planes(M[0], T[2], dev)
         self._conv(cat2, w2, self.conv2_tr, km("up", 1), M[0], u, T[2], self.norm2_tr, xp=cat2p, outp=up)
         self._block(self.block2_tr, u, T[2], km("s1", 1), M[0], cat1, w1, up, cat1p)
+        cout = self.final.kernel.shape[2]
+        out = torch.empty(M[0], cout, device=dev)
+        if (self.normalize_feature and not PRESPLIT and N.get_opt("fcgf_head") == 1
+                and tuple(self.conv1_tr.kernel.shape) == (1, 96, 64) and tuple(self.final.kernel.shape) == (1, 64, 32)):
+            N.check(L.mvr_fcgf_head(N.ptr(cat1), w1, M[0], N.ptr(self.conv1_tr.wimage()), N.ptr(self.final.wimage()),
+                                    N.ptr(self.final.bias), N.ptr(out), cout, N.stream()), "mvr_fcgf_head")
+            return SparseTensor(out, coords_key=1, coords_manager=cm)
         h = torch.empty(M[0], T[1], device=dev)
         hp = _planes(M[0], T[1], dev)
         self._conv(cat1, w1, self.conv1_tr, None, M[0], h, T[1], relu=True, xp=cat1p, outp=hp)
-        cout = self.final.kernel.shape[2]
-        out = torch.empty(M[0], cout, device=dev)
         self._conv(h, T[1], self.final, None, M[0], out, cout, bias=self.final.bias, xp=hp)
         if self.normalize_feature:
             N.check(L.mvr_l2norm_rows(N.ptr(out), M[0], cout, cout, N.stream()), "mvr_l2norm_rows")
diff --git a/3d_multiview_reg_amd/lib/filtering/oanet.py b/3d_multiview_reg_amd/lib/filtering/oanet.py
--- a/3d_multiview_reg_amd/lib/filtering/oanet.py
+++ b/3d_multiview_reg_amd/lib/filtering/oanet.py
@@ -135,6 +135,27 @@
         p.up_bn, p.up_conv = self._bp(self.up1.conv[1]), self._cp(self.up1.conv[3])
         p.output = self._cp(self.output)
         return p
+
+    def _prepared_key(self):
+        ts = [self.conv1.weight, self.up1.conv[3].weight, self.up1.conv[3].bias]
+        for i in range(self.layer_num // 2):
+            bn, cv = self.l2[i].conv2[0], self.l2[i].conv2[2]
+            ts += [bn.weight, bn.bias, bn.running_mean, bn.running_var, cv.weight]
+        return tuple(None if t is None else (t.data_ptr(), t._version, str(t.device)) for t in ts)
+
+    def native_prepared(self, params):
+        key = self._prepared_key()
+        hit = getattr(self, "_prep_cache", None)
+        if hit is not None and hit[0] == key:
+            return hit[1]
+        L = N.lib()
+        nb = L.mvr_oan_block_prepare_bytes(self.channels, self.clusters, self.in_channels, self.layer_num // 2)
+        blob = torch.empty(max(int(nb), 1), dtype=torch.uint8, device=self.conv1.weight.device)
+        N.check(L.mvr_oan_block_prepare(ctypes.byref(params), N.ptr(blob), blob.numel(), N.stream()),
+                "mvr_oan_block_prepare")
+        torch.cuda.current_stream(blob.device).synchronize()
+        self._prep_cache = (key, blob)
+        return blob
 
 
 class OANet(nn.Module):
@@ -194,13 +215,14 @@
             ext = self.guard_sync is not None
             res_row = None if last else N.ptr(inp[:, Cxs])
             score_row = None if last else N.ptr(inp[:, Cxs + 1])
-            rc = L.mvr_oan_block_forward(
+            prep = None if self.training else blk.native_prepared(params)
+            rc = L.mvr_oan_block_forward_prepared(
                 ctypes.byref(params), N.ptr(inp), rows * ld, ld, N.ptr(xs), Npts * Cxs, Cxs, P, Npts,
                 (int(self.bn_group) if self.bn_group > 1 else 1) if self.training else 0,
                 N.ptr(logits), N.ptr(scores), N.ptr(R), N.ptr(t), N.ptr(res), N.ptr(latent) if last else None,
                 res_row, score_row, rows * ld, N.ptr(guard), N.ptr(status[bi]), -1 if ext else int(self.guard_group),
-                N.ptr(ws), ws.numel(), st)
-            N.check(rc, "mvr_oan_block_forward")
+                N.ptr(ws), ws.numel(), N.ptr(prep), 0 if prep is None else prep.numel(), st)
+            N.check(rc, "mvr_oan_block_forward_prepared")
             if ext:
                 gp = self.guard_sync(guard)
                 N.check(L.mvr_procrustes(N.ptr(xs), N.ptr(xs[..., 3:]), Npts * Cxs, Cxs, N.ptr(scores), Npts, N.ptr(gp),
diff --git a/include/mvreg.h b/include/mvreg.h
--- a/include/mvreg.h
+++ b/include/mvreg.h
@@ -38,6 +38,12 @@
 
 int mvr_set_math(int mode);
 int mvr_debug_force(int what, int value);
+#define MVR_OPT_CONV1_FAST 0
+#define MVR_OPT_OAN_PREPARED 1
+#define MVR_OPT_FCGF_HEAD 2
+int mvr_set_opt(int what, int value);
+int mvr_get_opt(int what);
+int mvr_conv1_fast_bricks(int reset);
 
 int mvr_gemm_f32(int M, int N, int K, int batch, const float* A, int64_t sAb, int64_t lda, const float* B,
                  int64_t sBb, int64_t ldb, int b_kcontig, float* C, int64_t sCb, int64_t ldc, const float* R,
@@ -87,6 +93,14 @@
                           float* score_row, int64_t row_pstride, int32_t* guard_pos, int32_t* status, int guard_group,
                           void* workspace,
                           size_t workspace_bytes, mvr_stream_t stream);
+size_t mvr_oan_block_prepare_bytes(int channels, int clusters, int in_channels, int half_layers);
+int mvr_oan_block_prepare(const mvr_oan_block_p* blk, void* prepared, size_t prepared_bytes, mvr_stream_t stream);
+int mvr_oan_block_forward_prepared(const mvr_oan_block_p* blk, const float* input, int64_t in_pstride, int64_t ld,
+                                   const float* xs, int64_t xs_pstride, int64_t xs_nstride, int P, int N, int bn_train,
+                                   float* logits, float* scores, float* R, float* t, float* res, float* latent,
+                                   float* res_row, float* score_row, int64_t row_pstride, int32_t* guard_pos,
+                                   int32_t* status, int guard_group, void* workspace, size_t workspace_bytes,
+                                   const void* prepared, size_t prepared_bytes, mvr_stream_t stream);
 
 int mvr_oan_diff_pool(const float* x, int64_t x_pstride, int64_t x_ld, const float* sc, const float* sh,
                       int64_t s_pstride, const float* weight, const float* bias, int P, int channels, int N,
@@ -254,6 +268,8 @@
                     size_t in_bricks_bytes, const float* feat, int ksize, int step, const float* W, int Cout,
                     mvr_bn_p bn, float bn_eps, int relu, float* out, int64_t ldout, uint16_t* out_planes,
                     mvr_stream_t stream);
+int mvr_fcgf_head(const float* x, int64_t ldx, int64_t M, const void* wimg1, const void* wimg2, const float* bias2,
+                  float* out, int64_t ldout, mvr_stream_t stream);
 int mvr_l2norm_rows(float* x, int64_t M, int C, int64_t ld, mvr_stream_t stream);
 
 int mvr_sample_rand_mt19937(uint32_t* key, int32_t* pos, const int64_t* counts, int B, int tgt, int64_t* out,
```
